# yvokeller/Show-Attend-and-Tell

Measured on AMD Instinct MI355X. Metric: train images/sec on COCO batch=128 at 1/2/4/8 MI355X, higher is better.
Workload: dtype bf16; 1 GPU; COCO-shaped resnet152 encoder (bf16 fwd) + attention/tf/ado decoder train step, V=10000, T=27; global_batch=128, per_gpu_batch=128, seq_len=27, parallelism=dp1, hip_graph=True, encoder_decoder_overlap=True

## Files before the change

include/sat_hip.h:

```cpp
#ifndef SAT_HIP_H_
#define SAT_HIP_H_

#include <stddef.h>
#include <stdint.h>

#ifdef __cplusplus
extern "C" {
#endif

#define SAT_ABI_VERSION 9

enum { SAT_F32 = 0, SAT_BF16 = 1 };
enum { SAT_ACT_NONE = 0, SAT_ACT_RELU = 1, SAT_ACT_TANH = 2, SAT_ACT_SIGMOID = 3 };
enum { SAT_OK = 0, SAT_ERR_INVALID = 9001 };

typedef struct {
  int N, H, W, C, KH, KW, stride, pad, OH, OW;
} SatConvGeom;

typedef struct {
  int conv_pipe;
  int conv_stream;
  int conv3x3_ws;
  int conv_slices;
  int skinny;
  int gemm_stages;
  int gemm_tile;
  int gemm_linear_order;
  int gemm_epilogue;
  int split_gemm;
  int split_k;
  int attn_bwd;
  int attn_bwd_chunks;
  int attn_pipe;
  int decoder_splits[4];
  int greedy_step;
  int embed_grad;
  uint64_t* stamps;
  int stamp_capacity;
} SatPolicy;

typedef struct {
  int M, N, K, dtype;
  const void* A; int64_t lda; int transA;
  const void* B; int64_t ldb; int transB;
  void* C; int64_t ldc; int c_dtype;
  float alpha, beta;
  const float* bias;
  const void* add1; int64_t ld_add1; int add1_dtype;
  int act;
  void* aux; int64_t ld_aux; int aux_dtype;
  const SatPolicy* policy;
  void* workspace; int64_t workspace_bytes;
} SatGemmArgs;

typedef struct {
  int B, L, D, E, V, T;
  int tf, ado, attention, bert, training;
  int dtype;
  int start_token;
  int has_dropout_mask;
  uint64_t seed;
  uint64_t* seed_ptr;
  int split_target;
  const SatPolicy* policy;
} SatDecoderDims;

typedef struct {
  int64_t embedding, init_w, init_b, hcat_w, hcat_b, attW_w, attW_b, v_w, v_b, wih, bih;
  int64_t fh_w, fh_b, fz_w, fz_b, fout_w, fout_b, do_w, do_b;
  int64_t total;
  int64_t wih_ctx_t, hcat_t;
} SatDecoderLayout;

int sat_abi_version(void);
const char* sat_error_string(int code);

int sat_gemm(const SatGemmArgs* args, void* stream);
size_t sat_gemm_workspace_bytes(void);
int sat_cast(const void* x, int x_dtype, void* y, int y_dtype, int64_t n, void* stream);

int sat_mean_rows_abi(const void* a, int B, int L, int D, int dtype, float* out_f32, void* out_t, void* stream);

int sat_nchw_to_nhwc(int N, int C, int H, int W, int Cp, int dtype, const float* x, void* y, void* stream);
int sat_nchw_to_s2d(int N, int C, int H, int W, int dtype, const float* x, void* y, void* stream);
int sat_conv2d_nhwc(const SatConvGeom* g, int Cout, int dtype, const void* x, const void* w,
                    const float* bias, const void* residual, int relu, void* y, const SatPolicy* policy,
                    void* stream);
int sat_mfma_frag_layout(int N, int K, const void* src, void* dst, void* stream);
int sat_bottleneck_fused_supported(int H, int W, int Cin, int Cmid, int dtype);
int sat_bottleneck_fused(int N, int H, int W, int Cin, int Cmid, int dtype, const void* x, const void* w1f,
                         const float* b1, const void* w2f, const float* b2, const void* w3f, const float* b3,
                         void* y, const SatPolicy* policy, void* stream);
int sat_conv3x3_frag_supported(int H, int W, int C, int dtype);
int sat_conv3x3_frag(int N, int H, int W, int C, int dtype, const void* x, const void* wf, const float* b, void* y,
                     const SatPolicy* policy, void* stream);
int sat_conv1x1_frag_supported(int H, int W, int Cin, int Cout, int dtype);
int sat_conv1x1_frag(int N, int H, int W, int Cin, int Cout, int dtype, const void* x, const void* wf,
                     const float* b, void* y, const SatPolicy* policy, void* stream);
int sat_conv1x1_chain_supported(int64_t M, int K, int N, int N2, int dtype, const SatPolicy* policy);
int sat_conv1x1_chain(int64_t M, int K, int N, int N2, int dtype, const void* x, const void* w, const float* bias,
                      const void* residual, void* y, const void* w1, const float* b1, void* x1,
                      const SatPolicy* policy, void* stream);
int sat_conv1x1_proj_supported(int64_t M, int K, int N, int Kp, int stride, int N2, int dtype, const SatPolicy* policy);
int sat_conv1x1_proj(int n, int H, int W, int stride, int K, int N, int Kp, int N2, int dtype, const void* x,
                     const void* w, const float* bias, const void* xin, const void* wp, const float* bp, void* y,
                     const void* w1, const float* b1, void* x1, const SatPolicy* policy, void* stream);
int sat_conv_stem_pool_supported(const SatConvGeom* g, int Cout, int dtype, int relu, int pool_k, int pool_stride,
                                 int pool_pad, const SatPolicy* policy);
int sat_conv_stem_pool(const SatConvGeom* g, int Cout, int dtype, const void* x, const void* w, const float* bias,
                       int relu, int pool_k, int pool_stride, int pool_pad, void* y, const SatPolicy* policy,
                       void* stream);
int sat_maxpool2d_nhwc(int N, int H, int W, int C, int k, int stride, int pad, int dtype,
                       const void* x, void* y, int OH, int OW, void* stream);

size_t sat_conv3x3_wgrad_workspace_bytes(int N, int H, int W, int Cin, int Cout, int dtype, const SatPolicy* policy);
int sat_conv3x3_wgrad(int N, int H, int W, int Cin, int Cout, int dtype, const void* x, const void* dz, float* dw,
                      int accumulate, void* workspace, size_t workspace_bytes, const SatPolicy* policy,
                      void* stream);

int sat_relu_mask(const void* y, int y_dtype, const void* g, int g_dtype, const void* add, int add_dtype, void* out,
                  int out_dtype, int64_t n, void* stream);
int sat_conv_fold(int Cout, int Cin, int KH, int KW, int dtype, const float* weight, const float* bias,
                  const float* bn_weight, const float* bn_bias, const float* bn_mean, const float* bn_var, float eps,
                  void* w_fold, float* b_fold, void* w_igrad, void* stream);
typedef struct {
  const float* weight; const float* bias;
  const float* bn_weight; const float* bn_mean; const float* bn_var; float eps;
  const void* w_fold; const void* w_igrad;
  float* weight_grad; float* bias_grad; float* bn_weight_grad; float* bn_bias_grad;
} SatConvTrain;
int sat_conv_fold_backward(int Cout, int Cin, int KH, int KW, const float* dw_fold, const float* db_fold,
                           const SatConvTrain* conv, int accumulate, void* stream);
size_t sat_bottleneck_backward_workspace_bytes(int N, int H, int W, int Cin, int Cmid, int dtype,
                                               const SatPolicy* policy);
int sat_bottleneck_backward(int N, int H, int W, int Cin, int Cmid, int dtype, const void* x, const void* a1,
                            const void* a2, const void* y, const SatConvTrain* c1, const SatConvTrain* c2,
                            const SatConvTrain* c3, const void* dy, void* dx, int accumulate, void* workspace,
                            size_t workspace_bytes, const SatPolicy* policy, void* stream);
size_t sat_conv3x3_relu_backward_workspace_bytes(int N, int H, int W, int Cin, int Cout, int dtype,
                                                 const SatPolicy* policy);
int sat_conv3x3_relu_backward(int N, int H, int W, int Cin, int Cout, int dtype, const void* x, const void* y,
                              const SatConvTrain* c, const void* dy, void* dx, int accumulate, void* workspace,
                              size_t workspace_bytes, const SatPolicy* policy, void* stream);

int sat_attention_forward(int B, int L, int D, int E, int dtype, const void* img_features,
                          const float* hidden, const float* U_w, const float* U_b,
                          const float* W_w, const void* W_w_lp, const float* W_b,
                          const float* v_w, const float* v_b, float* ws_scratch,
                          float* context, float* alpha, void* stream);


int sat_decoder_step_bench(const SatDecoderDims* dims, const SatDecoderLayout* layout, const float* params,
                           const void* params_lp, const void* img_features, void* workspace, size_t workspace_bytes,
                           float* alphas, const float* d_alphas, int reps, float* us_out, void* stream);
size_t sat_decoder_workspace_bytes(const SatDecoderDims* d);
enum { SAT_DECODER_INSTANCE_FIELDS = 8 };
int sat_decoder_instance(const SatDecoderDims* d, const SatDecoderLayout* lay, int* out, int n);
int sat_decoder_refresh_transposed(const SatDecoderDims* d, const SatDecoderLayout* lay, void* params_lp,
                                   void* stream);
int sat_decoder_forward(const SatDecoderDims* d, const SatDecoderLayout* lay, const float* params,
                        const void* params_lp, const void* img_features, const int64_t* captions,
                        const uint8_t* dropout_mask, void* workspace, size_t workspace_bytes,
                        void* preds, float* alphas, int32_t* tokens, void* stream);
int sat_decoder_forward_sampled(const SatDecoderDims* d, const SatDecoderLayout* lay, const float* params,
                                const void* params_lp, const void* img_features, const int64_t* captions,
                                const uint8_t* dropout_mask, float tf_prob, const float* tf_prob_dev,
                                const uint8_t* tf_mask, uint8_t* tf_mask_out, void* workspace,
                                size_t workspace_bytes, void* preds, float* alphas, int32_t* tokens, void* stream);
int sat_decoder_backward(const SatDecoderDims* d, const SatDecoderLayout* lay, const float* params,
                         const void* params_lp, const void* img_features, void* workspace,
                         size_t workspace_bytes, const void* preds, const float* alphas,
                         const void* d_preds, const float* d_alphas, float* grads, int accumulate,
                         int phase, void* stream);
int sat_decoder_backward_features(const SatDecoderDims* d, const SatDecoderLayout* lay, const float* params,
                                  const void* params_lp, const void* img_features, void* workspace,
                                  size_t workspace_bytes, const void* preds, const float* alphas,
                                  const void* d_preds, const float* d_alphas, float* grads, int accumulate,
                                  int phase, void* stream, void* d_features, void* fg_workspace,
                                  size_t fg_workspace_bytes);
size_t sat_decoder_feature_grad_workspace_bytes(const SatDecoderDims* d);
int sat_feature_grad_accumulate(int B, int L, int D, int T1, int dtype, const float* alpha, int64_t alpha_stride_b,
                                int64_t alpha_stride_t, const float* dctx, int64_t dctx_stride_b,
                                int64_t dctx_stride_t, const float* addend, int64_t addend_ld,
                                const float* mean_term, int64_t mean_ld, void* out, int64_t out_ld, void* stream);

size_t sat_decoder_beam_workspace_bytes(const SatDecoderDims* d, int beam_size);
int sat_decoder_beam_search(const SatDecoderDims* d, const SatDecoderLayout* lay, const float* params,
                            const void* params_lp, const void* img_features, int beam_size, int max_step,
                            void* workspace, size_t workspace_bytes, int32_t* out_ids, int* out_len,
                            float* out_alphas, int* out_alpha_rows, float* out_score, void* stream);

size_t sat_decoder_beam_batch_workspace_bytes(const SatDecoderDims* d, int n_images, int beam_size, int max_step);
int sat_decoder_beam_search_batch(const SatDecoderDims* d, const SatDecoderLayout* lay, const float* params,
                                  const void* params_lp, const void* img_features, int n_images, int beam_size,
                                  int max_step, void* workspace, size_t workspace_bytes, int32_t* out_ids,
                                  int* out_len, float* out_alphas, int* out_alpha_rows, float* out_score,
                                  void* stream);

size_t sat_caption_loss_workspace_bytes(int B, int T, int L);
int sat_caption_loss_forward(int B, int T, int V, int L, int dtype, const void* preds,
                             const float* alphas, const int64_t* captions, float alpha_c,
                             int pad_id, int skip0, int skip1, int skip2, void* workspace,
                             float* out, void* stream);
int sat_caption_loss_forward_loss_out(int B, int T, int V, int L, int dtype, const void* preds,
                                      const float* alphas, const int64_t* captions, float alpha_c,
                                      int pad_id, int skip0, int skip1, int skip2, void* workspace,
                                      float* out, float* loss_out, void* stream);
int sat_caption_loss_backward(int B, int T, int V, int L, int dtype, const void* preds,
                              const int64_t* captions, float alpha_c, void* workspace,
                              const float* grad_out, void* d_preds, float* d_alphas, void* stream);
int sat_caption_loss_backward_relu(int B, int T, int V, int L, int dtype, const void* preds,
                              const int64_t* captions, float alpha_c, void* workspace,
                              const float* grad_out, void* d_preds, float* d_alphas, void* stream);
int sat_caption_loss_backward_ld(int B, int T, int V, int L, int dtype, const void* preds,
                                 const int64_t* captions, float alpha_c, void* workspace,
                                 const float* grad_out, void* d_preds, int64_t ld_dpreds,
                                 float* d_alphas, int relu_mask, void* stream);

enum { SAT_IMG_NCHW = 0, SAT_IMG_NHWC = 1, SAT_IMG_S2D16 = 2 };
size_t sat_images_workspace_bytes(int B, int OH, int OW);
int sat_images_max_downscale(void);
int sat_images_to_input(const uint8_t* pixels, const int64_t* offsets, const int32_t* sizes, int B, int max_h,
                        int max_w, int OH, int OW, const float* mean, const float* std, int layout, int c_pad,
                        int dtype, void* out, void* workspace, size_t workspace_bytes, void* stream);

int sat_rows_gather(const void* table, int64_t n_rows, int64_t row_elems, int dtype, const int64_t* idx, int n,
                    void* out, int32_t* n_bad, void* stream);
int sat_rows_scatter(const void* src, int n, int64_t row_elems, int dtype, const int64_t* idx, void* table,
                     int64_t n_rows, int32_t* n_bad, void* stream);

int sat_adam_step(float* param, const float* grad, float* exp_avg, float* exp_avg_sq,
// ... 8 lines not shown
```

show-attend-and-tell_amd/_lib.py:

```python
import ctypes
import os

import torch

_HERE = os.path.dirname(os.path.abspath(__file__))
LIB_PATH = os.environ.get("SAT_HIP_LIB_TUNING") or os.path.join(_HERE, "libsat_hip.so")

SAT_F32, SAT_BF16 = 0, 1
IMG_NCHW, IMG_NHWC, IMG_S2D16 = 0, 1, 2
ACT_NONE, ACT_RELU, ACT_TANH, ACT_SIGMOID = 0, 1, 2, 3

c_int, c_int64, c_float, c_void_p, c_size_t, c_uint64 = (ctypes.c_int, ctypes.c_int64, ctypes.c_float,
                                                        ctypes.c_void_p, ctypes.c_size_t, ctypes.c_uint64)


class SatConvGeom(ctypes.Structure):
    _fields_ = [(n, c_int) for n in ("N", "H", "W", "C", "KH", "KW", "stride", "pad", "OH", "OW")]


ABI_VERSION = 9


class SatPolicy(ctypes.Structure):
    _fields_ = [(n, c_int) for n in ("conv_pipe", "conv_stream", "conv3x3_ws", "conv_slices", "skinny", "gemm_stages",
                                     "gemm_tile", "gemm_linear_order", "gemm_epilogue", "split_gemm", "split_k",
                                     "attn_bwd", "attn_bwd_chunks", "attn_pipe")] + \
               [("decoder_splits", c_int * 4), ("greedy_step", c_int), ("embed_grad", c_int), ("stamps", c_void_p),
                ("stamp_capacity", c_int)]

    def __init__(self, **kw):
        splits = kw.pop("decoder_splits", None)
        super().__init__(**kw)
        if splits is not None:
            self.decoder_splits[:] = list(splits)


class SatGemmArgs(ctypes.Structure):
    _fields_ = [("M", c_int), ("N", c_int), ("K", c_int), ("dtype", c_int),
                ("A", c_void_p), ("lda", c_int64), ("transA", c_int),
                ("B", c_void_p), ("ldb", c_int64), ("transB", c_int),
                ("C", c_void_p), ("ldc", c_int64), ("c_dtype", c_int),
                ("alpha", c_float), ("beta", c_float),
                ("bias", c_void_p),
                ("add1", c_void_p), ("ld_add1", c_int64), ("add1_dtype", c_int),
                ("act", c_int),
                ("aux", c_void_p), ("ld_aux", c_int64), ("aux_dtype", c_int),
                ("policy", ctypes.POINTER(SatPolicy)),
                ("workspace", c_void_p), ("workspace_bytes", c_int64)]


class SatDecoderDims(ctypes.Structure):
    _fields_ = [("B", c_int), ("L", c_int), ("D", c_int), ("E", c_int), ("V", c_int), ("T", c_int),
                ("tf", c_int), ("ado", c_int), ("attention", c_int), ("bert", c_int), ("training", c_int),
                ("dtype", c_int), ("start_token", c_int), ("has_dropout_mask", c_int), ("seed", c_uint64),
                ("seed_ptr", c_void_p), ("split_target", c_int), ("policy", ctypes.POINTER(SatPolicy))]


class SatConvTrain(ctypes.Structure):
    _fields_ = [("weight", c_void_p), ("bias", c_void_p), ("bn_weight", c_void_p), ("bn_mean", c_void_p),
                ("bn_var", c_void_p), ("eps", c_float), ("w_fold", c_void_p), ("w_igrad", c_void_p),
                ("weight_grad", c_void_p), ("bias_grad", c_void_p), ("bn_weight_grad", c_void_p),
                ("bn_bias_grad", c_void_p)]


LAYOUT_FIELDS = ("embedding", "init_w", "init_b", "hcat_w", "hcat_b", "attW_w", "attW_b", "v_w", "v_b", "wih",
                 "bih", "fh_w", "fh_b", "fz_w", "fz_b", "fout_w", "fout_b", "do_w", "do_b", "total", "wih_ctx_t",
                 "hcat_t")


class SatDecoderLayout(ctypes.Structure):
    _fields_ = [(n, c_int64) for n in LAYOUT_FIELDS]


_SIGNATURES = [
    ("sat_abi_version", c_int, []),
    ("sat_error_string", ctypes.c_char_p, [c_int]),
    ("sat_gemm", c_int, [ctypes.POINTER(SatGemmArgs), c_void_p]),
    ("sat_gemm_workspace_bytes", c_size_t, []),
    ("sat_cast", c_int, [c_void_p, c_int, c_void_p, c_int, c_int64, c_void_p]),
    ("sat_mean_rows_abi", c_int, [c_void_p, c_int, c_int, c_int, c_int, c_void_p, c_void_p, c_void_p]),
    ("sat_nchw_to_nhwc", c_int, [c_int, c_int, c_int, c_int, c_int, c_int, c_void_p, c_void_p, c_void_p]),
    ("sat_nchw_to_s2d", c_int, [c_int, c_int, c_int, c_int, c_int, c_void_p, c_void_p, c_void_p]),
    ("sat_conv2d_nhwc", c_int, [ctypes.POINTER(SatConvGeom), c_int, c_int, c_void_p, c_void_p, c_void_p, c_void_p,
                                c_int, c_void_p, ctypes.POINTER(SatPolicy), c_void_p]),
    ("sat_mfma_frag_layout", c_int, [c_int, c_int, c_void_p, c_void_p, c_void_p]),
    ("sat_bottleneck_fused_supported", c_int, [c_int, c_int, c_int, c_int, c_int]),
    ("sat_bottleneck_fused", c_int, [c_int, c_int, c_int, c_int, c_int, c_int, c_void_p, c_void_p, c_void_p,
                                     c_void_p, c_void_p, c_void_p, c_void_p, c_void_p, ctypes.POINTER(SatPolicy),
                                     c_void_p]),
    ("sat_conv3x3_frag_supported", c_int, [c_int, c_int, c_int, c_int]),
    ("sat_conv3x3_frag", c_int, [c_int, c_int, c_int, c_int, c_int, c_void_p, c_void_p, c_void_p, c_void_p,
                                 ctypes.POINTER(SatPolicy), c_void_p]),
    ("sat_conv1x1_frag_supported", c_int, [c_int, c_int, c_int, c_int, c_int]),
    ("sat_conv1x1_frag", c_int, [c_int, c_int, c_int, c_int, c_int, c_int, c_void_p, c_void_p, c_void_p, c_void_p,
                                 ctypes.POINTER(SatPolicy), c_void_p]),
    ("sat_conv1x1_chain_supported", c_int, [c_int64, c_int, c_int, c_int, c_int, ctypes.POINTER(SatPolicy)]),
    ("sat_conv1x1_chain", c_int, [c_int64, c_int, c_int, c_int, c_int, c_void_p, c_void_p, c_void_p, c_void_p, c_void_p,
                                  c_void_p, c_void_p, c_void_p, ctypes.POINTER(SatPolicy), c_void_p]),
    ("sat_conv1x1_proj_supported", c_int, [c_int64, c_int, c_int, c_int, c_int, c_int, c_int,
                                           ctypes.POINTER(SatPolicy)]),
    ("sat_conv1x1_proj", c_int, [c_int, c_int, c_int, c_int, c_int, c_int, c_int, c_int, c_int, c_void_p, c_void_p,
                                 c_void_p, c_void_p, c_void_p, c_void_p, c_void_p, c_void_p, c_void_p, c_void_p,
                                 ctypes.POINTER(SatPolicy), c_void_p]),
    ("sat_conv_stem_pool_supported", c_int, [ctypes.POINTER(SatConvGeom), c_int, c_int, c_int, c_int, c_int, c_int,
                                             ctypes.POINTER(SatPolicy)]),
    ("sat_conv_stem_pool", c_int, [ctypes.POINTER(SatConvGeom), c_int, c_int, c_void_p, c_void_p, c_void_p, c_int,
                                   c_int, c_int, c_int, c_void_p, ctypes.POINTER(SatPolicy), c_void_p]),
    ("sat_maxpool2d_nhwc", c_int, [c_int, c_int, c_int, c_int, c_int, c_int, c_int, c_int, c_void_p, c_void_p,
                                   c_int, c_int, c_void_p]),
    ("sat_conv3x3_wgrad_workspace_bytes", c_size_t, [c_int, c_int, c_int, c_int, c_int, c_int,
                                                     ctypes.POINTER(SatPolicy)]),
    ("sat_conv3x3_wgrad", c_int, [c_int, c_int, c_int, c_int, c_int, c_int, c_void_p, c_void_p, c_void_p, c_int,
                                  c_void_p, c_size_t, ctypes.POINTER(SatPolicy), c_void_p]),
    ("sat_relu_mask", c_int, [c_void_p, c_int, c_void_p, c_int, c_void_p, c_int, c_void_p, c_int, c_int64, c_void_p]),
    ("sat_conv_fold", c_int, [c_int, c_int, c_int, c_int, c_int, c_void_p, c_void_p, c_void_p, c_void_p, c_void_p,
                              c_void_p, c_float, c_void_p, c_void_p, c_void_p, c_void_p]),
    ("sat_conv_fold_backward", c_int, [c_int, c_int, c_int, c_int, c_void_p, c_void_p, ctypes.POINTER(SatConvTrain),
                                       c_int, c_void_p]),
    ("sat_bottleneck_backward_workspace_bytes", c_size_t, [c_int, c_int, c_int, c_int, c_int, c_int,
                                                           ctypes.POINTER(SatPolicy)]),
    ("sat_bottleneck_backward", c_int, [c_int, c_int, c_int, c_int, c_int, c_int, c_void_p, c_void_p, c_void_p,
                                        c_void_p, ctypes.POINTER(SatConvTrain), ctypes.POINTER(SatConvTrain),
                                        ctypes.POINTER(SatConvTrain), c_void_p, c_void_p, c_int, c_void_p, c_size_t,
                                        ctypes.POINTER(SatPolicy), c_void_p]),
    ("sat_conv3x3_relu_backward_workspace_bytes", c_size_t, [c_int, c_int, c_int, c_int, c_int, c_int,
                                                             ctypes.POINTER(SatPolicy)]),
    ("sat_conv3x3_relu_backward", c_int, [c_int, c_int, c_int, c_int, c_int, c_int, c_void_p, c_void_p,
                                          ctypes.POINTER(SatConvTrain), c_void_p, c_void_p, c_int, c_void_p, c_size_t,
                                          ctypes.POINTER(SatPolicy), c_void_p]),
    ("sat_attention_forward", c_int, [c_int, c_int, c_int, c_int, c_int, c_void_p, c_void_p, c_void_p, c_void_p,
                                      c_void_p, c_void_p, c_void_p, c_void_p, c_void_p, c_void_p, c_void_p,
                                      c_void_p, c_void_p]),
    ("sat_decoder_workspace_bytes", c_size_t, [ctypes.POINTER(SatDecoderDims)]),
    ("sat_decoder_instance", c_int, [ctypes.POINTER(SatDecoderDims), ctypes.POINTER(SatDecoderLayout),
                                     ctypes.POINTER(c_int), c_int]),
    ("sat_decoder_refresh_transposed", c_int, [ctypes.POINTER(SatDecoderDims), ctypes.POINTER(SatDecoderLayout),
                                               c_void_p, c_void_p]),
    ("sat_decoder_forward", c_int, [ctypes.POINTER(SatDecoderDims), ctypes.POINTER(SatDecoderLayout), c_void_p,
                                    c_void_p, c_void_p, c_void_p, c_void_p, c_void_p, c_size_t, c_void_p,
                                    c_void_p, c_void_p, c_void_p]),
    ("sat_decoder_forward_sampled", c_int, [ctypes.POINTER(SatDecoderDims), ctypes.POINTER(SatDecoderLayout),
                                            c_void_p, c_void_p, c_void_p, c_void_p, c_void_p, c_float, c_void_p,
                                            c_void_p, c_void_p, c_void_p, c_size_t, c_void_p, c_void_p, c_void_p,
                                            c_void_p]),
    ("sat_decoder_backward", c_int, [ctypes.POINTER(SatDecoderDims), ctypes.POINTER(SatDecoderLayout), c_void_p,
                                     c_void_p, c_void_p, c_void_p, c_size_t, c_void_p, c_void_p, c_void_p,
                                     c_void_p, c_void_p, c_int, c_int, c_void_p]),
    ("sat_decoder_backward_features", c_int, [ctypes.POINTER(SatDecoderDims), ctypes.POINTER(SatDecoderLayout),
                                              c_void_p, c_void_p, c_void_p, c_void_p, c_size_t, c_void_p, c_void_p,
                                              c_void_p, c_void_p, c_void_p, c_int, c_int, c_void_p, c_void_p,
                                              c_void_p, c_size_t]),
    ("sat_decoder_feature_grad_workspace_bytes", c_size_t, [ctypes.POINTER(SatDecoderDims)]),
    ("sat_feature_grad_accumulate", c_int, [c_int, c_int, c_int, c_int, c_int, c_void_p, c_int64, c_int64, c_void_p,
                                            c_int64, c_int64, c_void_p, c_int64, c_void_p, c_int64, c_void_p,
                                            c_int64, c_void_p]),
    ("sat_decoder_step_bench", c_int, [ctypes.POINTER(SatDecoderDims), ctypes.POINTER(SatDecoderLayout), c_void_p,
                                       c_void_p, c_void_p, c_void_p, c_size_t, c_void_p, c_void_p, c_int, c_void_p,
                                       c_void_p]),
    ("sat_decoder_beam_workspace_bytes", c_size_t, [ctypes.POINTER(SatDecoderDims), c_int]),
    ("sat_decoder_beam_search", c_int, [ctypes.POINTER(SatDecoderDims), ctypes.POINTER(SatDecoderLayout), c_void_p,
                                        c_void_p, c_void_p, c_int, c_int, c_void_p, c_size_t, c_void_p, c_void_p,
                                        c_void_p, c_void_p, c_void_p, c_void_p]),
    ("sat_decoder_beam_batch_workspace_bytes", c_size_t, [ctypes.POINTER(SatDecoderDims), c_int, c_int, c_int]),
    ("sat_decoder_beam_search_batch", c_int, [ctypes.POINTER(SatDecoderDims), ctypes.POINTER(SatDecoderLayout),
                                              c_void_p, c_void_p, c_void_p, c_int, c_int, c_int, c_void_p, c_size_t,
                                              c_void_p, c_void_p, c_void_p, c_void_p, c_void_p, c_void_p]),
    ("sat_caption_loss_workspace_bytes", c_size_t, [c_int, c_int, c_int]),
    ("sat_caption_loss_forward", c_int, [c_int, c_int, c_int, c_int, c_int, c_void_p, c_void_p, c_void_p, c_float,
                                         c_int, c_int, c_int, c_int, c_void_p, c_void_p, c_void_p]),
    ("sat_caption_loss_forward_loss_out", c_int, [c_int, c_int, c_int, c_int, c_int, c_void_p, c_void_p, c_void_p,
                                                  c_float, c_int, c_int, c_int, c_int, c_void_p, c_void_p, c_void_p,
                                                  c_void_p]),
    ("sat_caption_loss_backward", c_int, [c_int, c_int, c_int, c_int, c_int, c_void_p, c_void_p, c_float,
                                          c_void_p, c_void_p, c_void_p, c_void_p, c_void_p]),
    ("sat_caption_loss_backward_relu", c_int, [c_int, c_int, c_int, c_int, c_int, c_void_p, c_void_p, c_float,
                                          c_void_p, c_void_p, c_void_p, c_void_p, c_void_p]),
    ("sat_caption_loss_backward_ld", c_int, [c_int, c_int, c_int, c_int, c_int, c_void_p, c_void_p, c_float,
                                             c_void_p, c_void_p, c_void_p, c_int64, c_void_p, c_int, c_void_p]),
    ("sat_images_workspace_bytes", c_size_t, [c_int, c_int, c_int]),
    ("sat_images_max_downscale", c_int, []),
    ("sat_images_to_input", c_int, [c_void_p, c_void_p, c_void_p, c_int, c_int, c_int, c_int, c_int,
                                    ctypes.POINTER(c_float), ctypes.POINTER(c_float), c_int, c_int, c_int, c_void_p,
                                    c_void_p, c_size_t, c_void_p]),
    ("sat_rows_gather", c_int, [c_void_p, c_int64, c_int64, c_int, c_void_p, c_int, c_void_p, c_void_p, c_void_p]),
    ("sat_rows_scatter", c_int, [c_void_p, c_int, c_int64, c_int, c_void_p, c_void_p, c_int64, c_void_p, c_void_p]),
    ("sat_adam_step", c_int, [c_void_p, c_void_p, c_void_p, c_void_p, c_void_p, c_int64, c_float, c_float,
                              c_float, c_float, c_float, c_void_p]),
]
EXPORTED = [s[0] for s in _SIGNATURES]

_lib = None


def lib():
    global _lib
    if _lib is None:
        if not os.path.exists(LIB_PATH):
            raise RuntimeError(f"sat_amd: HIP library not found at {LIB_PATH}; build it with "
                               "`python -c 'import __graft_entry__ as g; g.build()'` (make -C "
                               "show-attend-and-tell_amd/csrc)")
        handle = ctypes.CDLL(LIB_PATH)
        for name, res, args in _SIGNATURES:
            fn = getattr(handle, name)
            fn.restype = res
            fn.argtypes = args
        version = handle.sat_abi_version()
        if version != ABI_VERSION:
            raise RuntimeError(f"sat_amd: {LIB_PATH} has C-ABI version {version}, this package binds version "
                               f"{ABI_VERSION}; rebuild it (make -C show-attend-and-tell_amd/csrc)")
        _lib = handle
    return _lib


def check(code, what):
    if code != 0:
        msg = lib().sat_error_string(code)
        raise RuntimeError(f"sat_amd: {what} failed with code {code}: {msg.decode() if msg else '?'}")


def dtype_code(dt):
    if dt == torch.float32:
        return SAT_F32
    if dt == torch.bfloat16:
        return SAT_BF16
    raise TypeError(f"sat_amd: unsupported dtype {dt} (float32 or bfloat16)")


def require_device(*tensors):
    for t in tensors:
        if t is not None and t.device.type != "cuda":
            raise RuntimeError("sat_amd: tensors must live on a HIP device (the product path has no CPU fallback)")
# ... 13 lines not shown
```

show-attend-and-tell_amd/csrc/decoder.hip:

```cpp
#include "sat_common.h"
#include "sat_internal.h"

namespace {

struct WS {
  float *mean_f, *hc0, *hc0pre, *xg, *gctx_const, *hg, *gctx, *uh_all, *gates_all, *c_in, *c_out, *h_out, *ctx_all,
      *gate_all, *fh, *fz;
  void *mean_t, *Ws, *emb_t, *h_in_t, *ctx_t, *gated_t, *hd_t, *comb_t;
  int32_t* tok;
  uint8_t* dmask;
  void *dpre_t, *dfh_t, *dfz_t, *dhg_t, *dWs_t, *dpre0_t;
  float *dcomb, *dhd, *dctx_head, *dhg, *dgated, *dh_rec, *dc, *dWs_acc, *dv_acc, *dbv_acc, *part, *demb, *dpre0,
      *colsum, *de_all;
  unsigned* ticket;
  float* gsplit;
  unsigned* gtickets;
  float* xt;
  float* fzp;
  float* am_val;
  int32_t* am_idx;
  void* emb_ws;
};
constexpr int kTicketBlocks = 16;

struct Splits { int h, c, g, dh, i; };
constexpr int kSplitTargetDefault = 192;

constexpr int kChainAtomicK = 1024;
inline int ragged_splits(int K, long want) {
  const int kt = sat_cdiv(K, 64);
  const int cap = want < 2 ? 2 : (want > 8 ? 8 : (int)want);
  const int kc = sat_cdiv(kt, cap);
  return sat_cdiv(kt, kc);
}
inline int pick_splits(int M, int N, int K, int dtype, bool kmajor_w, int target) {
  if (dtype != SAT_BF16) return 1;
  const long tiles = (long)sat_cdiv(M, 128) * sat_cdiv(N, kmajor_w ? 128 : 64);
  long want = (target + tiles - 1) / tiles;
  if (want > 32) want = 32;
  const int kt = K / 64;
  int best = 1;
  if (K % 64 == 0)
    for (int s = 1; s <= kt && s <= want; ++s)
      if (kt % s == 0) best = s;
  if (best == 1 && K >= kChainAtomicK) best = ragged_splits(K, want);
  return best;
}
inline int forced(int f, int K, int auto_s) {
  if (f == 1 && K >= kChainAtomicK) return auto_s;
  return (f > 0 && K % 64 == 0 && (K / 64) % f == 0) ? f : auto_s;
}
inline Splits splits_for(const SatDecoderDims& d, bool tr) {
  const int E = d.E, D = d.D, HG = 5 * E + D;
  const bool bf = d.dtype == SAT_BF16;
  const int tg = d.split_target > 0 ? d.split_target : kSplitTargetDefault;
  const int KH = d.attention ? HG : 4 * E;
  Splits s;
  s.h = pick_splits(d.B, KH, E, d.dtype, false, tg);
  s.c = pick_splits(d.B, 4 * E, D, d.dtype, false, tg);
  s.g = pick_splits(d.B, D, 4 * E, d.dtype, !tr, tg);
  s.dh = pick_splits(d.B, E, KH, d.dtype, !tr, tg);
  s.i = pick_splits(d.B, 2 * E, D, d.dtype, false, tg);
  if (bf) {
    int k;
    if ((k = sat_skinny_splits(d.B, KH, E))) s.h = k;
    if ((k = sat_skinny_splits(d.B, 4 * E, D))) s.c = D % 512 == 0 ? k / 2 : k;
    if ((k = sat_skinny_splits(d.B, 2 * E, D))) s.i = k;
    if (tr && (k = sat_skinny_splits(d.B, D, 4 * E)) && (4 * E) % 512 == 0) s.g = k / 2;
    if (tr && (k = sat_skinny_splits(d.B, E, KH)) && KH % 512 == 0) s.dh = k / 2;
    if (tr && s.dh > 1 && KH % 128 == 0 && KH >= 4096) {
      const int cols = E / 32, kt = KH / 128;
      for (int c = 16; c > s.dh; --c)
        if (kt % c == 0 && c * cols <= 256 && KH / c <= 1024) { s.dh = c; break; }
    }
  }
  if (bf) {
    const int* f = sat_policy().decoder_splits;
    s.h = forced(f[0], E, s.h);
    s.c = forced(f[1], D, s.c);
    s.g = forced(f[2], 4 * E, s.g);
    s.dh = forced(f[3], KH, s.dh);
  }
  return s;
}
inline bool use_transposed(const SatDecoderDims& d, const SatDecoderLayout& lay) {
  return d.dtype == SAT_BF16 && lay.wih_ctx_t >= 0 && lay.hcat_t >= 0 && sat_policy().skinny != 1;
}
inline bool greedy_fused(const SatDecoderDims& d) {
  return d.dtype == SAT_BF16 && !d.tf && sat_policy().greedy_step != 1 && sat_greedy_supported(d.B, d.E);
}
inline bool embed_sorted(const SatDecoderDims& d) {
  return !d.bert && sat_policy().embed_grad != 1 && (long)d.B * (d.T - 1) <= sat_embed_sorted_max_rows() &&
         d.V < (1 << 18) && d.E % 4 == 0;
}

struct Carver {
  char* base;
  size_t off = 0;
  template <typename P>
  void take(P*& p, size_t bytes) {
    off = (off + 255) & ~(size_t)255;
    p = base ? (P*)(base + off) : nullptr;
    off += bytes;
  }
};

inline int head_ld(const SatDecoderDims& d) { return d.dtype == SAT_BF16 && d.V % 8 ? (d.V + 7) / 8 * 8 : d.V; }

size_t carve(const SatDecoderDims& d, char* base, WS* w) {
  const size_t B = d.B, L = d.L, D = d.D, E = d.E, V = d.V, T1 = d.T - 1, R = B * T1;
  const size_t HG = 5 * E + D;
  const size_t ts = d.dtype == SAT_BF16 ? 2 : 4, f = 4;
  Splits sp = splits_for(d, false);
  {
    const Splits st = splits_for(d, true);
    sp.g = sp.g > st.g ? sp.g : st.g;
    sp.dh = sp.dh > st.dh ? sp.dh : st.dh;
  }
  Carver c{base};
  c.take(w->mean_f, B * D * f);  c.take(w->mean_t, B * D * ts);
  c.take(w->hc0, B * 2 * E * f);
  c.take(w->hc0pre, sp.i * B * 2 * E * f);
  c.take(w->Ws, B * L * E * ts);
  c.take(w->tok, R * 4);
  c.take(w->emb_t, R * E * ts);
  c.take(w->xg, R * 4 * E * f);
  c.take(w->gctx_const, B * 4 * E * f);
  c.take(w->hg, sp.h * B * HG * f);
  c.take(w->gctx, sp.c * B * 4 * E * f);
  c.take(w->uh_all, R * E * f);
  c.take(w->gates_all, R * 4 * E * f);
  c.take(w->c_in, R * E * f);   c.take(w->c_out, R * E * f);
  c.take(w->h_in_t, R * E * ts); c.take(w->h_out, R * E * f);
  c.take(w->ctx_all, R * D * f); c.take(w->ctx_t, R * D * ts);
  c.take(w->gate_all, R * D * f); c.take(w->gated_t, R * D * ts);
  c.take(w->dmask, R * E);
  c.take(w->hd_t, R * E * ts);
  c.take(w->fh, R * E * f); c.take(w->fz, R * E * f); c.take(w->comb_t, R * E * ts);
  c.take(w->dpre_t, R * head_ld(d) * ts);
  c.take(w->dcomb, R * E * f);
  c.take(w->dfh_t, R * E * ts); c.take(w->dfz_t, R * E * ts);
  c.take(w->dhd, R * E * f);
  c.take(w->dctx_head, R * D * f);
  c.take(w->dhg, R * HG * f); c.take(w->dhg_t, R * HG * ts);
  c.take(w->dgated, sp.g * B * D * f);
  c.take(w->dh_rec, sp.dh * B * E * f); c.take(w->dc, B * E * f);
  c.take(w->dWs_acc, B * L * E * f); c.take(w->dWs_t, B * L * E * ts);
  c.take(w->dv_acc, B * E * f); c.take(w->dbv_acc, B * f);
  c.take(w->de_all, R * L * f);
  c.take(w->part, sat_attention_part_floats(d.B, d.L, d.D, d.E, d.dtype, d.split_target) * f);
  c.take(w->ticket, B * 4);
  if (d.dtype == SAT_BF16) {
    c.take(w->gsplit, sat_split_gemm_ws_bytes() - kSatSplitTickets * 4);
    c.take(w->gtickets, (size_t)kTicketBlocks * kSatSplitTickets * 4);
  } else {
    w->gsplit = nullptr;
    w->gtickets = nullptr;
  }
  c.take(w->demb, R * E * f);
  c.take(w->dpre0, B * 2 * E * f); c.take(w->dpre0_t, B * 2 * E * ts);
  if (greedy_fused(d)) {
    c.take(w->xt, V * 4 * E * f);
    c.take(w->fzp, sp.c * B * E * f);
    c.take(w->am_val, (size_t)sat_greedy_head_blocks(d.B, d.V, d.E) * B * f);
    c.take(w->am_idx, (size_t)sat_greedy_head_blocks(d.B, d.V, d.E) * B * 4);
  } else {
    w->xt = w->fzp = w->am_val = nullptr;
    w->am_idx = nullptr;
  }
  if (embed_sorted(d)) c.take(w->emb_ws, sat_embed_sorted_ws_bytes((int)R, (int)E));
  else w->emb_ws = nullptr;
  size_t maxN = V > HG ? V : HG;
  if (D > maxN) maxN = D;
  const size_t ph1 = V + 2 * E, ph2 = 9 * E + D + 1;
  if (ph1 > maxN) maxN = ph1;
  if (ph2 > maxN) maxN = ph2;
  c.take(w->colsum, sat_colsum_scratch_floats((int)R, (int)maxN) * f);
  return c.off + 256;
}

struct FGWS {
  float *dctx, *addend, *mean_term;
};
size_t carve_fg(const SatDecoderDims& d, char* base, FGWS* w) {
  const size_t B = d.B, L = d.L, D = d.D, R = B * (d.T - 1), f = 4;
  Carver c{base};
  c.take(w->dctx, R * D * f);
  if (d.attention) c.take(w->addend, B * L * D * f);
  else w->addend = nullptr;
  c.take(w->mean_term, B * D * f);
  return c.off + 256;
}

__global__ void start_tokens_kernel(int32_t* tok, int B, int T1, int start) {
  int b = blockIdx.x * blockDim.x + threadIdx.x;
  if (b < B) tok[(long)b * T1] = start;
}

__global__ void tf_prefill_kernel(const int64_t* __restrict__ caps, int B, int T, int V, int start,
                                  const uint8_t* __restrict__ keep_in, float p, const float* __restrict__ p_dev,
                                  uint64_t seed, const uint64_t* __restrict__ seed_ptr, int32_t* __restrict__ pre,
                                  uint8_t* __restrict__ keep_out) {
  const int T1 = T - 1;
  const int i = blockIdx.x * blockDim.x + threadIdx.x;
  if (i >= B * T1) return;
  const int b = i / T1, t = i - b * T1;
  bool keep = true;
  int tok = start;
  if (t > 0) {
    const int64_t c = caps[(long)b * T + t];
    tok = (c < 0 || c >= V) ? 0 : (int)c;
    if (keep_in) {
      keep = keep_in[i] != 0;
    } else {
      if (seed_ptr) seed ^= *seed_ptr * 0xD1B54A32D192ED03ULL;
      keep = sat_tf_uniform(seed, b, t) < (p_dev ? *p_dev : p);
    }
  }
  pre[i] = keep ? tok : -1;
  if (keep_out) keep_out[i] = keep ? 1 : 0;
}

struct Sampled {
  const int64_t* captions;
  float p; const float* p_dev;
  const uint8_t* mask; uint8_t* mask_out;
};
inline int32_t* tok_pre(const WS& w) { return (int32_t*)w.demb; }

template <typename T>
__global__ void ado_combine_rows_kernel(const float* fh, const float* fz, const T* emb, int rows, int E, long ld,
                                        T* comb) {
  const long n = (long)rows * E;
  for (long i = blockIdx.x * (long)blockDim.x + threadIdx.x; i < n; i += (long)gridDim.x * blockDim.x) {
    const long r = i / E;
    const int e = (int)(i - r * E);
    const long o = r * ld + e;
    comb[o] = (T)(fh[o] + fz[o] + (float)emb[o]);
  }
}

int combine_rows(const float* fh, const float* fz, const void* emb, int rows, int E, long ld, int dtype, void* comb,
                 hipStream_t s) {
  long n = (long)rows * E;
  int g = (int)((n + 255) / 256);
  if (g > 4096) g = 4096;
  if (dtype == SAT_BF16)
    hipLaunchKernelGGL(ado_combine_rows_kernel<bf16>, dim3(g), dim3(256), 0, s, fh, fz, (const bf16*)emb, rows, E, ld, (bf16*)comb);
  else
    hipLaunchKernelGGL(ado_combine_rows_kernel<float>, dim3(g), dim3(256), 0, s, fh, fz, (const float*)emb, rows, E, ld, (float*)comb);
  return (int)hipGetLastError();
}

template <typename T>
__global__ void init_state_kernel(const float* pre, int splits, long stride, int B, int E, float* hc0, T* h_t,
                                  long h_ld, float* c_in, long c_ld) {
  const long n = (long)B * 2 * E;
  for (long i = blockIdx.x * (long)blockDim.x + threadIdx.x; i < n; i += (long)gridDim.x * blockDim.x) {
    const int b = (int)(i / (2 * E)), j = (int)(i - (long)b * 2 * E);
    const float v = tanhf(sum_parts(pre, i, splits, stride));
    hc0[i] = v;
    if (j < E) h_t[(long)b * h_ld + j] = (T)v;
    else c_in[(long)b * c_ld + j - E] = v;
  }
}

struct Ctx {
  SatDecoderDims d;
  SatDecoderLayout lay;
  const float* P;
  const void* LP;
  int ts;
  long T1, R, HG;
  bool tr;
  const void* W(int64_t off) const {
    return d.dtype == SAT_BF16 ? (const void*)((const bf16*)LP + off) : (const void*)(P + off);
  }
  const float* F(int64_t off) const { return P + off; }
  void* at(void* p, long elems) const { return (char*)p + elems * ts; }
  const void* at(const void* p, long elems) const { return (const char*)p + elems * ts; }
};

int linear(const Ctx& c, int rows, int N, int K, const void* x, long ldx, const void* w, long ldw, const float* bias,
           void* y, long ldy, int y_dtype, int act, hipStream_t s, const void* add1 = nullptr, long ld_add1 = 0,
           int add1_dtype = SAT_F32, void* aux = nullptr, long ld_aux = 0, int aux_dtype = SAT_F32,
           int splits = 0, long split_stride = 0) {
  SatGemm g;
  g.partial_splits = splits; g.split_stride = split_stride;
  g.M = rows; g.N = N; g.K = K; g.dtype = c.d.dtype;
  g.A = x; g.lda = ldx; g.B = w; g.ldb = ldw;
  g.C = y; g.ldc = ldy; g.c_dtype = y_dtype; g.bias = bias; g.act = act;
  g.add1 = add1; g.ld_add1 = ld_add1; g.add1_dtype = add1_dtype;
  g.aux = aux; g.ld_aux = ld_aux; g.aux_dtype = aux_dtype;
  return sat_gemm_launch(g, s);
}

int head_forward(const Ctx& c, const WS& w, int rows, int t, bool per_step, void* preds, const uint8_t* mask_in,
                 hipStream_t s) {
  const SatDecoderDims& d = c.d;
  const int E = d.E, D = d.D, V = d.V;
  const long rs = per_step ? c.T1 : 1;
  const long oE = per_step ? (long)t * E : 0, oD = per_step ? (long)t * D : 0, oV = per_step ? (long)t * V : 0;
  if (per_step)
    SAT_CHECK((hipError_t)sat_dropout_apply(w.h_out + oE, c.T1 * E, d.B, 1, E, d.training, d.has_dropout_mask,
                                            mask_in ? mask_in + oE : nullptr, w.dmask + oE, c.T1 * E, d.seed,
                                            d.seed_ptr, t,
                                            c.at(w.hd_t, oE), c.T1 * E, d.dtype, s));
  else
    SAT_CHECK((hipError_t)sat_dropout_apply(w.h_out, E, d.B, (int)c.T1, E, d.training, d.has_dropout_mask, mask_in,
                                            w.dmask, E, d.seed, d.seed_ptr, 0, w.hd_t, E, d.dtype, s));
  if (d.ado) {
    SAT_CHECK((hipError_t)linear(c, rows, E, E, c.at(w.hd_t, oE), rs * E, c.W(c.lay.fh_w), E, c.F(c.lay.fh_b),
                                 w.fh + oE, rs * E, SAT_F32, SAT_ACT_RELU, s));
    SAT_CHECK((hipError_t)linear(c, rows, E, D, c.at(w.ctx_t, oD), rs * D, c.W(c.lay.fz_w), D, c.F(c.lay.fz_b),
                                 w.fz + oE, rs * E, SAT_F32, SAT_ACT_RELU, s));
    SAT_CHECK((hipError_t)combine_rows(w.fh + oE, w.fz + oE, c.at(w.emb_t, oE), rows, E, rs * E, d.dtype,
                                       c.at(w.comb_t, oE), s));
    SAT_CHECK((hipError_t)linear(c, rows, V, E, c.at(w.comb_t, oE), rs * E, c.W(c.lay.fout_w), E,
                                 c.F(c.lay.fout_b), c.at(preds, oV), rs * V, d.dtype, SAT_ACT_RELU, s));
  } else {
    SAT_CHECK((hipError_t)linear(c, rows, V, E, c.at(w.hd_t, oE), rs * E, c.W(c.lay.do_w), E, c.F(c.lay.do_b),
                                 c.at(preds, oV), rs * V, d.dtype, SAT_ACT_NONE, s));
  }
  return 0;
}

struct StepIO {
  const void* feats;
  float* alphas;
  const float* d_alphas;
};

int fwd_hgemm(const Ctx& c, const WS& w, const Splits& sp, int t, hipStream_t s) {
  const SatDecoderDims& d = c.d;
  const int B = d.B, D = d.D, E = d.E;
  const long T1 = c.T1, HG = c.HG;
  const void* h_t = c.at(w.h_in_t, (long)t * E);
  if (d.attention)
    return linear(c, B, (int)HG, E, h_t, T1 * E, c.W(c.lay.hcat_w), E, c.F(c.lay.hcat_b), w.hg, HG, SAT_F32,
                  SAT_ACT_NONE, s, nullptr, 0, SAT_F32, nullptr, 0, SAT_F32, sp.h, (long)B * HG);
  return linear(c, B, 4 * E, E, h_t, T1 * E, c.W(c.lay.hcat_w + (long)(E + D) * E), E, c.F(c.lay.hcat_b + E + D),
                w.hg + E + D, HG, SAT_F32, SAT_ACT_NONE, s, nullptr, 0, SAT_F32, nullptr, 0, SAT_F32, sp.h,
                (long)B * HG);
}

int fwd_attn(const Ctx& c, const WS& w, const Splits& sp, const StepIO& io, int t, hipStream_t s) {
  const SatDecoderDims& d = c.d;
  const int B = d.B, L = d.L, D = d.D, E = d.E;
  const long T1 = c.T1, HG = c.HG;
  AttnFwdArgs a{};
  a.B = B; a.L = L; a.D = D; a.E = E; a.dtype = d.dtype;
  a.Ws = w.Ws; a.uh = w.hg; a.uh_ld = HG; a.v_w = c.F(c.lay.v_w); a.v_b = c.F(c.lay.v_b); a.a = io.feats;
  a.gate_pre = w.hg + E; a.gate_ld = HG;
  a.hg_splits = sp.h; a.hg_split_stride = (long)B * HG;
  a.alpha = io.alphas + (long)t * L; a.alpha_ld = T1 * L;
  a.ctx = w.ctx_all + (long)t * D; a.ctx_ld = T1 * D;
  a.ctx_t = c.at(w.ctx_t, (long)t * D); a.ctx_t_ld = T1 * D;
  a.gate = w.gate_all + (long)t * D; a.gate_out_ld = T1 * D;
  a.gated = c.at(w.gated_t, (long)t * D); a.gated_ld = T1 * D;
  a.uh_save = w.uh_all + (long)t * E; a.uh_save_ld = T1 * E;
  return sat_attention_fwd_launch(a, s);
}

int fwd_cgemm(const Ctx& c, const WS& w, const Splits& sp, int t, hipStream_t s) {
  const SatDecoderDims& d = c.d;
  const int B = d.B, D = d.D, E = d.E;
  return linear(c, B, 4 * E, D, c.at(w.gated_t, (long)t * D), c.T1 * D, c.W(c.lay.wih + E), E + D, nullptr, w.gctx,
                4 * E, SAT_F32, SAT_ACT_NONE, s, nullptr, 0, SAT_F32, nullptr, 0, SAT_F32, sp.c, (long)B * 4 * E);
}

LstmFwdArgs lstm_fwd_args(const Ctx& c, const WS& w, const Splits& sp, int t) {
  const SatDecoderDims& d = c.d;
  const int B = d.B, D = d.D, E = d.E;
  const long T1 = c.T1, HG = c.HG;
  const bool att = d.attention != 0;
  LstmFwdArgs l{};
  l.B = B; l.E = E; l.dtype = d.dtype;
  l.hpart = w.hg + E + D; l.hpart_ld = HG;
  l.xpart = w.xg + (long)t * 4 * E; l.xpart_ld = T1 * 4 * E;
  l.cpart = att ? w.gctx : w.gctx_const; l.cpart_ld = 4 * E;
  l.h_splits = sp.h; l.h_split_stride = (long)B * HG;
  l.c_splits = att ? sp.c : 1; l.c_split_stride = (long)B * 4 * E;
  l.c_prev = w.c_in + (long)t * E; l.c_prev_ld = T1 * E;
  l.gates = w.gates_all + (long)t * 4 * E; l.gates_ld = T1 * 4 * E;
  l.c_out = w.c_out + (long)t * E; l.c_out_ld = T1 * E;
  l.c_next_in = t + 1 < T1 ? w.c_in + (long)(t + 1) * E : nullptr; l.c_next_in_ld = T1 * E;
  l.h_out = w.h_out + (long)t * E; l.h_out_ld = T1 * E;
  l.h_next_in_t = t + 1 < T1 ? c.at(w.h_in_t, (long)(t + 1) * E) : nullptr; l.h_next_in_t_ld = T1 * E;
  return l;
}

int fwd_lstm(const Ctx& c, const WS& w, const Splits& sp, int t, hipStream_t s) {
  return sat_lstm_fwd_launch(lstm_fwd_args(c, w, sp, t), s);
}

LstmBwdArgs lstm_bwd_args(const Ctx& c, const WS& w, const Splits& sp, int t) {
  const SatDecoderDims& d = c.d;
  const int B = d.B, D = d.D, E = d.E;
  const long T1 = c.T1, HG = c.HG;
  LstmBwdArgs l{};
  l.B = B; l.E = E; l.dtype = d.dtype;
  l.gates = w.gates_all + (long)t * 4 * E; l.gates_ld = T1 * 4 * E;
  l.c_prev = w.c_in + (long)t * E; l.c_prev_ld = T1 * E;
  l.c_new = w.c_out + (long)t * E; l.c_new_ld = T1 * E;
  l.dh_rec = t == T1 - 1 ? nullptr : w.dh_rec; l.dh_rec_ld = E;
  l.dh_splits = sp.dh; l.dh_split_stride = (long)B * E;
  l.dh_head = w.dhd + (long)t * E; l.dh_head_ld = T1 * E;
  l.mask = d.training ? w.dmask + (long)t * E : nullptr; l.mask_ld = T1 * E;
  l.dc = w.dc; l.dc_zero = t == T1 - 1;
  l.d_gates = w.dhg + (long)t * HG + E + D; l.d_gates_ld = T1 * HG;
  l.d_gates_t = c.at(w.dhg_t, (long)t * HG + E + D); l.d_gates_t_ld = T1 * HG;
  return l;
}

int bwd_lstm(const Ctx& c, const WS& w, const Splits& sp, int t, hipStream_t s) {
  return sat_lstm_bwd_launch(lstm_bwd_args(c, w, sp, t), s);
}

struct SplitWS {
  float* slab;
  unsigned* tickets;
  int blk;
};
inline void use_split(SatGemm& g, const SplitWS* sw) {
  if (!sw || !sw->slab) return;
  g.split_ws = sw->slab;
  g.split_ws_bytes = (long)(sat_split_gemm_ws_bytes() - kSatSplitTickets * 4);
  g.split_tickets = sw->tickets + (long)sw->blk * kSatSplitTickets;
  g.tickets_zeroed = 1;
}

int dgrad_launch(const Ctx& c, int M, int N, int K, const void* X, long ldx, const void* Wt, long ldw, float* out,
                 long ldo, hipStream_t s, const float* add1 = nullptr, long ld_add1 = 0, int splits = 0,
                 long split_stride = 0, int a_tail = 0, const SplitWS* sw = nullptr) {
  SatGemm g;
  use_split(g, sw);
  g.a_tail = a_tail;
  g.partial_splits = splits; g.split_stride = split_stride;
  g.M = M; g.N = N; g.K = K; g.dtype = c.d.dtype;
  g.A = X; g.lda = ldx; g.B = Wt; g.ldb = ldw; g.transB = 1;
  g.C = out; g.ldc = ldo; g.c_dtype = SAT_F32;
  g.add1 = add1; g.ld_add1 = ld_add1; g.add1_dtype = SAT_F32;
  return sat_gemm_launch(g, s);
}

int bwd_ggemm(const Ctx& c, const WS& w, const Splits& sp, int t, hipStream_t s) {
  const SatDecoderDims& d = c.d;
  const int B = d.B, D = d.D, E = d.E;
  if (c.tr)
    return linear(c, B, D, 4 * E, c.at(w.dhg_t, (long)t * c.HG + E + D), c.T1 * c.HG, c.W(c.lay.wih_ctx_t), 4 * E,
                  nullptr, w.dgated, D, SAT_F32, SAT_ACT_NONE, s, nullptr, 0, SAT_F32, nullptr, 0, SAT_F32, sp.g,
                  (long)B * D);
  return dgrad_launch(c, B, D, 4 * E, c.at(w.dhg_t, (long)t * c.HG + E + D), c.T1 * c.HG, c.W(c.lay.wih + E), E + D,
                      w.dgated, D, s, nullptr, 0, sp.g, (long)B * D);
}

int bwd_attn(const Ctx& c, const WS& w, const Splits& sp, const StepIO& io, int t, hipStream_t s,
             float* dctx_all = nullptr) {
  const SatDecoderDims& d = c.d;
  const int B = d.B, L = d.L, D = d.D, E = d.E;
  const long T1 = c.T1, HG = c.HG;
  AttnBwdArgs a{};
  a.B = B; a.L = L; a.D = D; a.E = E; a.dtype = d.dtype;
  a.Ws = w.Ws; a.a = io.feats;
  a.uh = w.uh_all + (long)t * E; a.uh_ld = T1 * E;
  a.v_w = c.F(c.lay.v_w);
  a.alpha = io.alphas + (long)t * L; a.alpha_ld = T1 * L;
  a.d_alpha_ext = io.d_alphas + (long)t * L; a.d_alpha_ext_ld = T1 * L;
  a.d_gated = w.dgated; a.d_gated_ld = D;
  a.gate = w.gate_all + (long)t * D; a.gate_ld = T1 * D;
  a.ctx = w.ctx_all + (long)t * D; a.ctx_ld = T1 * D;
  a.d_ctx_ext = d.ado ? w.dctx_head + (long)t * D : nullptr; a.d_ctx_ext_ld = T1 * D;
  a.d_ctx_out = dctx_all ? dctx_all + (long)t * D : nullptr; a.d_ctx_out_ld = T1 * D;
  a.d_uh = w.dhg + (long)t * HG; a.d_uh_ld = T1 * HG; a.d_uh_t = c.at(w.dhg_t, (long)t * HG);
  a.d_gpre = w.dhg + (long)t * HG + E; a.d_gpre_ld = T1 * HG; a.d_gpre_t = c.at(w.dhg_t, (long)t * HG + E);
  a.de_out = w.de_all + (long)t * L; a.de_ld = T1 * L; a.dv_acc = w.dv_acc; a.dbv_acc = w.dbv_acc; a.part = w.part;
  a.ticket = w.ticket;
  a.dg_splits = sp.g; a.dg_split_stride = (long)B * D;
  a.wg_target = d.split_target;
  return sat_attention_bwd_launch(a, s);
}

int bwd_dhgemm(const Ctx& c, const WS& w, const Splits& sp, int t, hipStream_t s) {
  const SatDecoderDims& d = c.d;
  const int B = d.B, D = d.D, E = d.E;
  const long T1 = c.T1, HG = c.HG;
  if (c.tr) {
    const long k0 = d.attention ? 0 : E + D;
    return linear(c, B, E, (int)(HG - k0), c.at(w.dhg_t, (long)t * HG + k0), T1 * HG, c.W(c.lay.hcat_t + k0), HG,
                  nullptr, w.dh_rec, E, SAT_F32, SAT_ACT_NONE, s, nullptr, 0, SAT_F32, nullptr, 0, SAT_F32, sp.dh,
                  (long)B * E);
  }
  if (d.attention)
    return dgrad_launch(c, B, E, (int)HG, c.at(w.dhg_t, (long)t * HG), T1 * HG, c.W(c.lay.hcat_w), E, w.dh_rec, E, s,
                        nullptr, 0, sp.dh, (long)B * E);
  return dgrad_launch(c, B, E, 4 * E, c.at(w.dhg_t, (long)t * HG + E + D), T1 * HG,
                      c.W(c.lay.hcat_w + (long)(E + D) * E), E, w.dh_rec, E, s, nullptr, 0, sp.dh, (long)B * E);
}

constexpr int kStampGroups = 8;
inline uint64_t* step_slot(const SatDecoderDims& d, int g, int t) {
  const SatPolicy* p = d.policy;
  if (!p || !p->stamps || p->stamp_capacity <= 0) return nullptr;
  return p->stamps + ((long)g * (d.T - 1) + t) * 2L * (p->stamp_capacity + 1);
}
inline int stamp_cap(const SatDecoderDims& d) { return d.policy ? d.policy->stamp_capacity : 0; }

struct StepTimer {
  SatStampScope stamps;
  StepTimer(const SatDecoderDims& d, int g, int t) : stamps(step_slot(d, g, t), stamp_cap(d)) {}
};

int greedy_loop(const Ctx& c, const WS& w, const Splits& sp, const StepIO& io, void* preds, const uint8_t* mask_in,
                int32_t* tokens, hipStream_t s, const Sampled* sm = nullptr) {
  const SatDecoderDims& d = c.d;
  const SatDecoderLayout& lay = c.lay;
  const int B = d.B, D = d.D, E = d.E, V = d.V, T1 = d.T - 1;
  const bool att = d.attention != 0;
  SAT_CHECK((hipError_t)linear(c, V, 4 * E, E, c.W(lay.embedding), E, c.W(lay.wih), E + D, c.F(lay.bih), w.xt, 4 * E,
                               SAT_F32, SAT_ACT_NONE, s));
  SAT_CHECK((hipError_t)sat_embed_gather(w.xt, w.tok, B, 1, T1, 4 * E, SAT_F32, w.xg, (long)T1 * 4 * E, s));
  for (int t = 0; t < T1; ++t) {
    const long oE = (long)t * E, oD = (long)t * D;
    {
      StepTimer st(d, 0, t);
      SAT_CHECK((hipError_t)fwd_hgemm(c, w, sp, t, s));
    }
    if (att) {
      {
        StepTimer st(d, 1, t);
        SAT_CHECK((hipError_t)fwd_attn(c, w, sp, io, t, s));
      }
      StepTimer st(d, 2, t);
      SatGemm g1;
      g1.partial_splits = sp.c; g1.split_stride = (long)B * 4 * E;
      g1.M = B; g1.N = 4 * E; g1.K = D; g1.dtype = d.dtype;
      g1.A = c.at(w.gated_t, oD); g1.lda = c.T1 * D; g1.B = c.W(lay.wih + E); g1.ldb = E + D;
      g1.C = w.gctx; g1.ldc = 4 * E; g1.c_dtype = SAT_F32;
      SatGemm g2 = g1;
      g2.N = E; g2.A = c.at(w.ctx_t, oD); g2.B = c.W(lay.fz_w); g2.ldb = D;
      g2.C = w.fzp; g2.ldc = E; g2.split_stride = (long)B * E;
      int err = 0;
      if (!(d.ado && sat_skinny_dual_try(g1, g2, s, &err))) {
        SAT_CHECK((hipError_t)sat_gemm_launch(g1, s));
        if (d.ado) SAT_CHECK((hipError_t)sat_gemm_launch(g2, s));
      }
      SAT_CHECK((hipError_t)err);
    } else if (d.ado) {
      SAT_CHECK((hipError_t)linear(c, B, E, D, c.at(w.ctx_t, oD), c.T1 * D, c.W(lay.fz_w), D, nullptr, w.fzp, E,
                                   SAT_F32, SAT_ACT_NONE, s));
    }
    {
      StepTimer st(d, 3, t);
      LstmFwdArgs l = lstm_fwd_args(c, w, sp, t);
      l.hd_t = c.at(w.hd_t, oE); l.hd_ld = c.T1 * E;
      l.drop_training = d.training; l.drop_has_mask = d.has_dropout_mask; l.drop_t = t;
      l.mask_in = mask_in ? mask_in + oE : nullptr; l.mask_out = w.dmask + oE; l.mask_ld = c.T1 * E;
      l.seed = d.seed; l.seed_ptr = d.seed_ptr;
      if (t > 0) {
        l.am_val = w.am_val; l.am_idx = w.am_idx; l.am_ncb = sat_greedy_head_blocks(B, V, E); l.am_V = V;
        l.xt = w.xt; l.emb = c.F(lay.embedding); l.emb_t = c.at(w.emb_t, oE); l.emb_t_ld = c.T1 * E;
        l.tok_out = w.tok + t; l.tok_ld = T1;
        if (sm) l.tok_pre = tok_pre(w) + t;
      }
      SAT_CHECK((hipError_t)sat_lstm_fwd_launch(l, s));
    }
    HeadOutArgs ho{};
    ho.B = B; ho.V = V; ho.E = E;
    if (d.ado) {
      HeadMidArgs hm{};
      hm.B = B; hm.E = E;
      hm.hd = (const bf16*)c.at(w.hd_t, oE); hm.hd_ld = c.T1 * E;
      hm.fh_w = (const bf16*)c.W(lay.fh_w); hm.fh_b = c.F(lay.fh_b);
      hm.fzp = w.fzp; hm.fzp_ld = E; hm.fz_splits = att ? sp.c : 1; hm.fz_split_stride = (long)B * E;
      hm.fz_b = c.F(lay.fz_b);
      hm.emb = (const bf16*)c.at(w.emb_t, oE); hm.emb_ld = c.T1 * E;
      hm.fh = w.fh + oE; hm.fz = w.fz + oE; hm.f_ld = c.T1 * E;
      hm.comb = (bf16*)c.at(w.comb_t, oE); hm.comb_ld = c.T1 * E;
      SAT_CHECK((hipError_t)sat_greedy_head_mid(hm, s));
      ho.relu = 1;
      ho.x = hm.comb; ho.x_ld = hm.comb_ld;
      ho.w = (const bf16*)c.W(lay.fout_w); ho.bias = c.F(lay.fout_b);
    } else {
      ho.relu = 0;
      ho.x = (const bf16*)c.at(w.hd_t, oE); ho.x_ld = c.T1 * E;
      ho.w = (const bf16*)c.W(lay.do_w); ho.bias = c.F(lay.do_b);
    }
    ho.preds = (bf16*)c.at(preds, (long)t * V); ho.preds_ld = c.T1 * V;
    ho.pval = w.am_val; ho.pidx = w.am_idx;
    SAT_CHECK((hipError_t)sat_greedy_head_out(ho, s));
  }
  if (d.training && d.seed_ptr) SAT_CHECK((hipError_t)sat_bump_seed(d.seed_ptr, s));
  if (tokens) SAT_CHECK(hipMemcpyAsync(tokens, w.tok, c.R * sizeof(int32_t), hipMemcpyDeviceToDevice, s));
  return 0;
}

// ... 127 lines not shown
    hipLaunchKernelGGL(start_tokens_kernel, dim3(sat_cdiv(B, 256)), dim3(256), 0, s, w.tok, B, T1, d.start_token);
    SAT_LAUNCH_CHECK();
    if (sm) {
      hipLaunchKernelGGL(tf_prefill_kernel, dim3(sat_cdiv(B * T1, 256)), dim3(256), 0, s, sm->captions, B, d.T, d.V,
                         d.start_token, sm->mask, sm->p, sm->p_dev, d.seed, (const uint64_t*)d.seed_ptr, tok_pre(w),
                         sm->mask_out);
      SAT_LAUNCH_CHECK();
    }
    SAT_CHECK((hipError_t)sat_embed_gather(c.F(lay->embedding), w.tok, B, 1, T1, E, d.dtype, w.emb_t, (long)T1 * E, s));
  }
  SAT_CHECK((hipError_t)sat_mean_rows(img_features, B, L, D, d.dtype, w.mean_f, w.mean_t, s));
  SAT_CHECK((hipError_t)linear(c, B, 2 * E, D, w.mean_t, D, c.W(lay->init_w), D, c.F(lay->init_b), w.hc0pre, 2 * E,
                               SAT_F32, SAT_ACT_NONE, s, nullptr, 0, SAT_F32, nullptr, 0, SAT_F32, sp.i,
                               (long)B * 2 * E));
  {
    const long n = (long)B * 2 * E;
    const int g = (int)((n + 255) / 256 < 2048 ? (n + 255) / 256 : 2048);
    if (d.dtype == SAT_BF16)
      hipLaunchKernelGGL(init_state_kernel<bf16>, dim3(g), dim3(256), 0, s, (const float*)w.hc0pre, sp.i,
                         (long)B * 2 * E, B, E, w.hc0, (bf16*)w.h_in_t, (long)T1 * E, w.c_in, (long)T1 * E);
    else
      hipLaunchKernelGGL(init_state_kernel<float>, dim3(g), dim3(256), 0, s, (const float*)w.hc0pre, sp.i,
                         (long)B * 2 * E, B, E, w.hc0, (float*)w.h_in_t, (long)T1 * E, w.c_in, (long)T1 * E);
    SAT_LAUNCH_CHECK();
  }
  if (att) {
    SAT_CHECK((hipError_t)linear(c, B * L, E, D, img_features, D, c.W(lay->attW_w), D, c.F(lay->attW_b), w.Ws, E,
                                 d.dtype, SAT_ACT_NONE, s));
  } else {
    SAT_CHECK((hipError_t)linear(c, B, 4 * E, D, w.mean_t, D, c.W(lay->wih + E), E + D, nullptr, w.gctx_const, 4 * E,
                                 SAT_F32, SAT_ACT_NONE, s));
    SAT_CHECK((hipError_t)sat_broadcast_rows(w.mean_t, B, D, T1, d.dtype, w.gated_t, s));
    SAT_CHECK((hipError_t)sat_broadcast_rows(w.mean_t, B, D, T1, d.dtype, w.ctx_t, s));
    SAT_CHECK((hipError_t)sat_broadcast_rows(w.mean_f, B, D, T1, SAT_F32, w.ctx_all, s));
    SAT_CHECK((hipError_t)sat_fill_const(alphas, (long)B * T1 * L, 1.0f / (float)L, s));
  }
  if (d.tf)
    SAT_CHECK((hipError_t)linear(c, (int)c.R, 4 * E, E, w.emb_t, E, c.W(lay->wih), E + D, c.F(lay->bih), w.xg, 4 * E,
                                 SAT_F32, SAT_ACT_NONE, s));

  if (greedy_fused(d)) return greedy_loop(c, w, sp, io, preds, dropout_mask, tokens, s, sm);

  for (int t = 0; t < T1; ++t) {
    if (!d.tf)
      SAT_CHECK((hipError_t)linear(c, B, 4 * E, E, c.at(w.emb_t, (long)t * E), (long)T1 * E, c.W(lay->wih), E + D,
                                   c.F(lay->bih), w.xg + (long)t * 4 * E, (long)T1 * 4 * E, SAT_F32, SAT_ACT_NONE, s));
    {
      StepTimer st(d, 0, t);
      SAT_CHECK((hipError_t)fwd_hgemm(c, w, sp, t, s));
    }
    if (att) {
      {
        StepTimer st(d, 1, t);
        SAT_CHECK((hipError_t)fwd_attn(c, w, sp, io, t, s));
      }
      StepTimer st(d, 2, t);
      SAT_CHECK((hipError_t)fwd_cgemm(c, w, sp, t, s));
    }
    {
      StepTimer st(d, 3, t);
      SAT_CHECK((hipError_t)fwd_lstm(c, w, sp, t, s));
    }
    if (!d.tf) {
      SAT_CHECK((hipError_t)head_forward(c, w, B, t, true, preds, dropout_mask, s));
      if (t + 1 < T1 && sm)
        SAT_CHECK((hipError_t)sat_argmax_rows_select(c.at(preds, (long)t * d.V), d.dtype, (long)T1 * d.V, B, d.V,
                                                     w.tok + t + 1, T1, c.F(lay->embedding), E,
                                                     c.at(w.emb_t, (long)(t + 1) * E), (long)T1 * E,
                                                     tok_pre(w) + t + 1, T1, s));
      else if (t + 1 < T1)
        SAT_CHECK((hipError_t)sat_argmax_rows(c.at(preds, (long)t * d.V), d.dtype, (long)T1 * d.V, B, d.V,
                                              w.tok + t + 1, T1, c.F(lay->embedding), E,
                                              c.at(w.emb_t, (long)(t + 1) * E), (long)T1 * E, s));
    }
  }
  if (d.tf) SAT_CHECK((hipError_t)head_forward(c, w, (int)c.R, 0, false, preds, dropout_mask, s));
  if (d.training && d.seed_ptr) SAT_CHECK((hipError_t)sat_bump_seed(d.seed_ptr, s));
  if (tokens) SAT_CHECK(hipMemcpyAsync(tokens, w.tok, c.R * sizeof(int32_t), hipMemcpyDeviceToDevice, s));
  return 0;
}
}

extern "C" int sat_decoder_forward(const SatDecoderDims* dp, const SatDecoderLayout* lay, const float* params,
                                   const void* params_lp, const void* img_features, const int64_t* captions,
                                   const uint8_t* dropout_mask, void* workspace, size_t workspace_bytes, void* preds,
                                   float* alphas, int32_t* tokens, void* stream) {
  return decoder_forward(dp, lay, params, params_lp, img_features, captions, dropout_mask, workspace, workspace_bytes,
                         preds, alphas, tokens, stream, nullptr);
}

extern "C" int sat_decoder_forward_sampled(const SatDecoderDims* dp, const SatDecoderLayout* lay, const float* params,
                                           const void* params_lp, const void* img_features, const int64_t* captions,
                                           const uint8_t* dropout_mask, float tf_prob, const float* tf_prob_dev,
                                           const uint8_t* tf_mask, uint8_t* tf_mask_out, void* workspace,
                                           size_t workspace_bytes, void* preds, float* alphas, int32_t* tokens,
                                           void* stream) {
  SAT_REQUIRE(dp && dp->tf == 0);
  SAT_REQUIRE(tf_prob >= 0.f && tf_prob <= 1.f);
  const Sampled sm{captions, tf_prob, tf_prob_dev, tf_mask, tf_mask_out};
  return decoder_forward(dp, lay, params, params_lp, img_features, captions, dropout_mask, workspace, workspace_bytes,
                         preds, alphas, tokens, stream, &sm);
}

namespace {
int decoder_backward(const SatDecoderDims* dp, const SatDecoderLayout* lay, const float* params, const void* params_lp,
                     const void* img_features, void* workspace, size_t workspace_bytes, const void* preds,
                     const float* alphas, const void* d_preds, const float* d_alphas, float* grads, int accumulate,
                     int phase, void* stream, void* d_features, void* fg_workspace, size_t fg_workspace_bytes) {
  SAT_CHECK((hipError_t)check_dims(dp));
  SAT_REQUIRE(lay && params && img_features && workspace && preds && alphas && d_preds && d_alphas && grads);
  FGWS fg{};
  if (d_features && (phase & 2)) {
    SAT_REQUIRE(fg_workspace && carve_fg(*dp, nullptr, &fg) <= fg_workspace_bytes);
    SAT_REQUIRE(((uintptr_t)d_features & 15) == 0 && ((uintptr_t)fg_workspace & 15) == 0);
    carve_fg(*dp, (char*)fg_workspace, &fg);
  }
  SAT_REQUIRE((phase & 3) != 0 && phase >= 1 && phase <= 15);
  SAT_REQUIRE(dp->dtype == SAT_F32 || params_lp);
  SatPolicyScope scope(dp->policy);
  SatStampScope no_stamps(nullptr, 0);
  const SatDecoderDims& d = *dp;
  WS w;
  SAT_REQUIRE(carve(d, nullptr, &w) <= workspace_bytes);
  carve(d, (char*)workspace, &w);
  hipStream_t s = (hipStream_t)stream;
  Ctx c{d, *lay, params, params_lp, d.dtype == SAT_BF16 ? 2 : 4, d.T - 1, (long)d.B * (d.T - 1), 5L * d.E + d.D,
        use_transposed(d, *lay)};
  const int B = d.B, L = d.L, D = d.D, E = d.E, V = d.V, T1 = d.T - 1;
  const int R = (int)c.R;
  const int VP = head_ld(d);
  const long HG = c.HG;
  const bool att = d.attention != 0;
  const float beta = accumulate ? 1.f : 0.f;
  const Splits sp = splits_for(d, c.tr);
  auto G = [&](int64_t off) { return grads + off; };
  auto wg = [&](int M, int N, int K, const void* X, long ldx, const void* Y, long ldy, float* out, long ldo,
                int a_tail = 0) {
    SatGemm g;
    g.a_tail = a_tail;
    g.M = M; g.N = N; g.K = K; g.dtype = d.dtype;
    g.A = X; g.lda = ldx; g.transA = 1;
    g.B = Y; g.ldb = ldy; g.transB = 1;
    g.C = out; g.ldc = ldo; g.c_dtype = SAT_F32; g.beta = beta;
    return g;
  };
  const SplitWS sws[kTicketBlocks] = {
      {w.gsplit, w.gtickets, 0}, {w.gsplit, w.gtickets, 1}, {w.gsplit, w.gtickets, 2}, {w.gsplit, w.gtickets, 3},
      {w.gsplit, w.gtickets, 4}, {w.gsplit, w.gtickets, 5}, {w.gsplit, w.gtickets, 6}, {w.gsplit, w.gtickets, 7},
      {w.gsplit, w.gtickets, 8}, {w.gsplit, w.gtickets, 9}, {w.gsplit, w.gtickets, 10}, {w.gsplit, w.gtickets, 11},
      {w.gsplit, w.gtickets, 12}, {w.gsplit, w.gtickets, 13}, {w.gsplit, w.gtickets, 14}, {w.gsplit, w.gtickets, 15}};
  const SatZeroSeg tickets_ph1{(float*)w.gtickets, 1, 8L * kSatSplitTickets, 8L * kSatSplitTickets};
  const SatZeroSeg tickets_ph2{(float*)w.gtickets + 8L * kSatSplitTickets, 1, 8L * kSatSplitTickets,
                               8L * kSatSplitTickets};
  auto wgs = [&](int blk, int M, int N, int K, const void* X, long ldx, const void* Y, long ldy, float* out, long ldo,
                 int a_tail = 0) {
    SatGemm g = wg(M, N, K, X, ldx, Y, ldy, out, ldo, a_tail);
    use_split(g, &sws[blk]);
    return g;
  };
  auto prezero = [&](SatGemm* const* gs, int n, SatZeroSeg* seg, int& nseg) {
    for (int i = 0; i < n; ++i)
      if (!accumulate && !sat_split_gemm_takes(*gs[i]) && sat_gemm_splits_atomically(*gs[i])) {
        seg[nseg++] = SatZeroSeg{(float*)gs[i]->C, gs[i]->M, gs[i]->N, gs[i]->ldc};
        gs[i]->c_zeroed = 1;
      }
  };
  auto dgrad = [&](int blk, int M, int N, int K, const void* X, long ldx, const void* Wt, long ldw, float* out,
                   long ldo, const float* add1 = nullptr, long ld_add1 = 0) {
    return dgrad_launch(c, M, N, K, X, ldx, Wt, ldw, out, ldo, s, add1, ld_add1, 0, 0, 0, &sws[blk]);
  };
  auto colsum = [&](const void* X, int dt, long ld, int rows, int N, float* out, float* out2 = nullptr,
                    int cols_readable = 0) {
    return sat_colsum(X, dt, ld, rows, N, out, accumulate, out2, w.colsum, s, cols_readable);
  };

  if (phase & 1) {
    if (d.ado) {
      const void* dpre = d_preds;
      long ldp = V;
      if (phase & 8) {
        SAT_REQUIRE(phase & 4);
        ldp = VP;
      } else if (VP != V) {
        SAT_CHECK((hipError_t)sat_pad_rows(d_preds, (phase & 4) ? nullptr : preds, R, V, VP, d.dtype, w.dpre_t, s));
        dpre = w.dpre_t; ldp = VP;
      } else if (!(phase & 4)) {
        SAT_CHECK((hipError_t)sat_relu_mask_mul(d_preds, preds, (long)R * V, d.dtype, w.dpre_t, s));
        dpre = w.dpre_t;
      }
      SatGemm gfo = wgs(0, V, E, R, dpre, ldp, w.comb_t, E, G(lay->fout_w), E, VP != V);
      SatGemm gfh = wgs(2, E, E, R, w.dfh_t, E, w.hd_t, E, G(lay->fh_w), E);
      SatGemm gfz = wgs(3, E, D, R, w.dfz_t, E, w.ctx_t, D, G(lay->fz_w), D);
      {
        SatGemm* gs[3] = {&gfo, &gfh, &gfz};
        SatZeroSeg seg[4];
        int nseg = 0;
        if (w.gtickets) seg[nseg++] = tickets_ph1;
        prezero(gs, 3, seg, nseg);
        SAT_CHECK((hipError_t)sat_zero_segs(seg, nseg, s));
      }
      SAT_CHECK((hipError_t)sat_gemm_launch(gfo, s));
      SAT_CHECK((hipError_t)dgrad_launch(c, R, E, V, dpre, ldp, c.W(lay->fout_w), E, w.dcomb, E, s, nullptr, 0, 0, 0,
                                         VP != V, &sws[1]));
      SAT_CHECK((hipError_t)sat_ado_bwd_split(w.dcomb, w.fh, w.fz, (long)R * E, d.dtype, w.dfh_t, w.dfz_t, s));
      SAT_CHECK((hipError_t)sat_gemm_launch(gfh, s));
      SAT_CHECK((hipError_t)sat_gemm_launch(gfz, s));
      const SatColsumSeg cs[3] = {{dpre, d.dtype, ldp, R, V, G(lay->fout_b), accumulate, nullptr, ldp != V},
                                  {w.dfh_t, d.dtype, E, R, E, G(lay->fh_b), accumulate, nullptr},
                                  {w.dfz_t, d.dtype, E, R, E, G(lay->fz_b), accumulate, nullptr}};
      SAT_CHECK((hipError_t)sat_colsum_multi(cs, 3, w.colsum, s));
      SAT_CHECK((hipError_t)dgrad(4, R, E, E, w.dfh_t, E, c.W(lay->fh_w), E, w.dhd, E));
      if (att) SAT_CHECK((hipError_t)dgrad(5, R, D, E, w.dfz_t, E, c.W(lay->fz_w), D, w.dctx_head, D));
    } else {
      const void* dpre = d_preds;
      long ldp = (phase & 8) ? VP : V;
      if (VP != V && !(phase & 8)) {
        SAT_CHECK((hipError_t)sat_pad_rows(d_preds, nullptr, R, V, VP, d.dtype, w.dpre_t, s));
        dpre = w.dpre_t; ldp = VP;
      }
      SatGemm gdo = wgs(0, V, E, R, dpre, ldp, w.hd_t, E, G(lay->do_w), E, VP != V);
      {
        SatGemm* gs[1] = {&gdo};
        SatZeroSeg seg[2];
        int nseg = 0;
        if (w.gtickets) seg[nseg++] = tickets_ph1;
        prezero(gs, 1, seg, nseg);
        SAT_CHECK((hipError_t)sat_zero_segs(seg, nseg, s));
      }
      SAT_CHECK((hipError_t)sat_gemm_launch(gdo, s));
      SAT_CHECK((hipError_t)colsum(dpre, d.dtype, ldp, R, V, G(lay->do_b), nullptr, ldp != V));
      SAT_CHECK((hipError_t)dgrad_launch(c, R, E, V, dpre, ldp, c.W(lay->do_w), E, w.dhd, E, s, nullptr, 0, 0, 0,
                                         VP != V, &sws[1]));
    }
  }
  if (!(phase & 2)) return 0;

  const void* dg_t = c.at(w.dhg_t, E + D);
  SatGemm g_attw = wgs(8, E, D, B * L, w.dWs_t, E, img_features, D, G(lay->attW_w), D);
  SatGemm g_init = wgs(9, 2 * E, D, B, w.dpre0_t, 2 * E, w.mean_t, D, G(lay->init_w), D);
  SatGemm g_hcat = att ? wgs(10, (int)HG, E, R, w.dhg_t, HG, w.h_in_t, E, G(lay->hcat_w), E)
                       : wgs(10, 4 * E, E, R, dg_t, HG, w.h_in_t, E, G(lay->hcat_w + (long)(E + D) * E), E);
  SatGemm g_wihx = wgs(11, 4 * E, E, R, dg_t, HG, w.emb_t, E, G(lay->wih), E + D);
  SatGemm g_wihc = wgs(12, 4 * E, D, R, dg_t, HG, w.gated_t, D, G(lay->wih + E), E + D);
  {
    SatZeroSeg seg[12];
    int nz = 0;
    if (att) {
      seg[nz++] = SatZeroSeg{w.dv_acc, 1, (long)B * E, (long)B * E};
      seg[nz++] = SatZeroSeg{w.dbv_acc, 1, B, B};
      seg[nz++] = SatZeroSeg{(float*)w.ticket, 1, B, B};
    }
    if (!d.bert && !accumulate) seg[nz++] = SatZeroSeg{G(lay->embedding), 1, (long)V * E, (long)V * E};
    if (w.gtickets) seg[nz++] = tickets_ph2;
    SatGemm* gs[5] = {&g_hcat, &g_wihx, &g_wihc, &g_init, &g_attw};
    prezero(gs, att ? 5 : 4, seg, nz);
    SAT_CHECK((hipError_t)sat_zero_segs(seg, nz, s));
  }
  const StepIO io{img_features, const_cast<float*>(alphas), d_alphas};
  for (int t = T1 - 1; t >= 0; --t) {
    {
      StepTimer st(d, 4, t);
      SAT_CHECK((hipError_t)bwd_lstm(c, w, sp, t, s));
    }
    if (att) {
      {
        StepTimer st(d, 5, t);
        SAT_CHECK((hipError_t)bwd_ggemm(c, w, sp, t, s));
      }
      StepTimer st(d, 6, t);
      SAT_CHECK((hipError_t)bwd_attn(c, w, sp, io, t, s, fg.dctx));
    }
    StepTimer st(d, 7, t);
    SAT_CHECK((hipError_t)bwd_dhgemm(c, w, sp, t, s));
  }

  if (att) {
    SAT_CHECK((hipError_t)sat_attention_dws_launch(w.Ws, w.uh_all, w.de_all, c.F(lay->v_w), B, L, E, T1, d.dtype,
                                                   w.dWs_acc, w.dWs_t, s));
    SAT_CHECK((hipError_t)sat_gemm_launch(g_attw, s));
  }
  SAT_CHECK((hipError_t)sat_tanh_pair_bwd(w.dh_rec, sp.dh, (long)B * E, w.dc, w.hc0, B, E, w.dpre0, w.dpre0_t,
                                          d.dtype, s));
  SAT_CHECK((hipError_t)sat_gemm_launch(g_init, s));
  {
    SatColsumSeg cs[6];
    int n = 0;
    if (att) {
      cs[n++] = {w.dWs_acc, SAT_F32, E, B * L, E, G(lay->attW_b), accumulate, nullptr};
      cs[n++] = {w.dv_acc, SAT_F32, E, B, E, G(lay->v_w), accumulate, nullptr};
      cs[n++] = {w.dbv_acc, SAT_F32, 1, B, 1, G(lay->v_b), accumulate, nullptr};
      cs[n++] = {w.dhg, SAT_F32, HG, R, E + D, G(lay->hcat_b), accumulate, nullptr};
    }
    cs[n++] = {w.dpre0, SAT_F32, 2 * E, B, 2 * E, G(lay->init_b), accumulate, nullptr};
    cs[n++] = {w.dhg + E + D, SAT_F32, HG, R, 4 * E, G(lay->hcat_b + E + D), accumulate, G(lay->bih)};
    SAT_CHECK((hipError_t)sat_colsum_multi(cs, n, w.colsum, s));
  }

  SAT_CHECK((hipError_t)sat_gemm_launch(g_hcat, s));
  SAT_CHECK((hipError_t)sat_gemm_launch(g_wihx, s));
  SAT_CHECK((hipError_t)sat_gemm_launch(g_wihc, s));
  if (!d.bert) {
    SAT_CHECK((hipError_t)dgrad(13, R, E, 4 * E, dg_t, HG, c.W(lay->wih), E + D, w.demb, E, d.ado ? w.dcomb : nullptr,
                                E));
    if (w.emb_ws)
      SAT_CHECK((hipError_t)sat_embed_scatter_add_sorted(w.demb, w.tok, R, E, G(lay->embedding), accumulate, w.emb_ws,
                                                         s));
    else
      SAT_CHECK((hipError_t)sat_embed_scatter_add(w.demb, w.tok, R, E, G(lay->embedding), s));
  }
  if (!fg.dctx) return 0;

  SAT_CHECK((hipError_t)dgrad(15, B, D, 2 * E, w.dpre0_t, 2 * E, c.W(lay->init_w), D, fg.mean_term, D));
  if (att) {
    SAT_CHECK((hipError_t)dgrad(14, B * L, D, E, w.dWs_t, E, c.W(lay->attW_w), D, fg.addend, D));
  } else {
    if (d.ado) SAT_CHECK((hipError_t)dgrad(8, R, D, E, w.dfz_t, E, c.W(lay->fz_w), D, w.dctx_head, D));
    SAT_CHECK((hipError_t)dgrad(14, R, D, 4 * E, dg_t, HG, c.W(lay->wih + E), E + D, fg.dctx, D,
                                d.ado ? w.dctx_head : nullptr, D));
  }
  FeatureGradArgs fa{};
  fa.B = B; fa.L = L; fa.D = D; fa.T1 = T1; fa.dtype = d.dtype;
  fa.alpha = alphas; fa.alpha_bs = (long)T1 * L; fa.alpha_ts = L;
  fa.dctx = fg.dctx; fa.dctx_bs = (long)T1 * D; fa.dctx_ts = D;
  fa.addend = fg.addend; fa.addend_ld = D;
  fa.mean_term = fg.mean_term; fa.mean_ld = D;
  fa.out = d_features; fa.out_ld = D;
  return sat_feature_grad_launch(fa, s);
}
}

extern "C" int sat_decoder_backward(const SatDecoderDims* dp, const SatDecoderLayout* lay, const float* params,
                                    const void* params_lp, const void* img_features, void* workspace,
                                    size_t workspace_bytes, const void* preds, const float* alphas,
                                    const void* d_preds, const float* d_alphas, float* grads, int accumulate,
                                    int phase, void* stream) {
  return decoder_backward(dp, lay, params, params_lp, img_features, workspace, workspace_bytes, preds, alphas, d_preds,
                          d_alphas, grads, accumulate, phase, stream, nullptr, nullptr, 0);
}

extern "C" int sat_decoder_backward_features(const SatDecoderDims* dp, const SatDecoderLayout* lay, const float* params,
                                             const void* params_lp, const void* img_features, void* workspace,
                                             size_t workspace_bytes, const void* preds, const float* alphas,
                                             const void* d_preds, const float* d_alphas, float* grads, int accumulate,
                                             int phase, void* stream, void* d_features, void* fg_workspace,
                                             size_t fg_workspace_bytes) {
  return decoder_backward(dp, lay, params, params_lp, img_features, workspace, workspace_bytes, preds, alphas, d_preds,
                          d_alphas, grads, accumulate, phase, stream, d_features, fg_workspace, fg_workspace_bytes);
}

extern "C" size_t sat_decoder_feature_grad_workspace_bytes(const SatDecoderDims* d) {
  if (check_dims(d)) return 0;
  FGWS w;
  return carve_fg(*d, nullptr, &w);
}

extern "C" int sat_decoder_step_bench(const SatDecoderDims* dp, const SatDecoderLayout* lay, const float* params,
                                      const void* params_lp, const void* img_features, void* workspace,
                                      size_t workspace_bytes, float* alphas, const float* d_alphas, int reps,
                                      float* us_out, void* stream) {
  SAT_CHECK((hipError_t)check_dims(dp));
  SAT_REQUIRE(lay && params && img_features && workspace && alphas && d_alphas && us_out && reps > 0);
  SAT_REQUIRE(dp->dtype == SAT_F32 || params_lp);
  SatPolicyScope scope(dp->policy);
  SatStampScope no_stamps(nullptr, 0);
  const SatDecoderDims& d = *dp;
  WS w;
  SAT_REQUIRE(carve(d, nullptr, &w) <= workspace_bytes);
  carve(d, (char*)workspace, &w);
  hipStream_t s = (hipStream_t)stream;
  Ctx c{d, *lay, params, params_lp, d.dtype == SAT_BF16 ? 2 : 4, d.T - 1, (long)d.B * (d.T - 1), 5L * d.E + d.D,
        use_transposed(d, *lay)};
  const Splits sp = splits_for(d, c.tr);
  const StepIO io{img_features, alphas, d_alphas};
  const int t = (d.T - 1) / 2;
  hipEvent_t e0, e1;
  SAT_CHECK(hipEventCreate(&e0));
  SAT_CHECK(hipEventCreate(&e1));
  int rc = 0;
  for (int k = 0; k < 8 && rc == 0; ++k) {
    us_out[k] = 0.f;
    if (!d.attention && (k == 1 || k == 2 || k == 5 || k == 6)) continue;
    for (int r = -1; r < reps && rc == 0; ++r) {
      if (r == 0) rc = (int)hipEventRecord(e0, s);
      switch (k) {
        case 0: rc = fwd_hgemm(c, w, sp, t, s); break;
        case 1: rc = fwd_attn(c, w, sp, io, t, s); break;
        case 2: rc = fwd_cgemm(c, w, sp, t, s); break;
        case 3: rc = fwd_lstm(c, w, sp, t, s); break;
        case 4: rc = bwd_lstm(c, w, sp, t, s); break;
        case 5: rc = bwd_ggemm(c, w, sp, t, s); break;
        case 6: rc = bwd_attn(c, w, sp, io, t, s); break;
        default: rc = bwd_dhgemm(c, w, sp, t, s); break;
      }
    }
    if (rc == 0) rc = (int)hipEventRecord(e1, s);
    if (rc == 0) rc = (int)hipEventSynchronize(e1);
    float ms = 0.f;
    if (rc == 0) rc = (int)hipEventElapsedTime(&ms, e0, e1);
    us_out[k] = ms * 1000.f / reps;
  }
  (void)hipEventDestroy(e0);
  (void)hipEventDestroy(e1);
  return rc;
}
```

show-attend-and-tell_amd/csrc/gemm.hip:

```cpp
#include "sat_common.h"
#include "sat_internal.h"

#include <type_traits>

namespace {

template <typename T> struct Cfg;
template <> struct Cfg<float> { static constexpr int BK = 16, VEC = 4, PAD = 4; };
template <> struct Cfg<bf16> { static constexpr int BK = 32, VEC = 8, PAD = 8; };

struct KArgs {
  int M, N, K;
  const void* A; long lda;
  const void* B; long ldb;
  void* C; long ldc; int c_dtype;
  float alpha, beta;
  const float* bias;
  const void* add1; long ld_add1; int add1_dtype;
  int act;
  void* aux; long ld_aux; int aux_dtype;
  long sA, sB, sC, s_add1, s_aux;
  SatConvGeom cv;
  int vecA, vecB;
  int splitk, kchunk;
// ... 270 lines not shown
  char* Xb = a.aux ? (char*)a.aux + z * a.s_aux * (a.aux_dtype == SAT_BF16 ? 2 : 4) : nullptr;
  if (a.c_dtype == SAT_BF16) {
    if (a.aux_dtype == SAT_BF16) epi((bf16*)Cb, (bf16*)Xb);
    else epi((bf16*)Cb, (float*)Xb);
  } else {
    if (a.aux_dtype == SAT_BF16) epi((float*)Cb, (bf16*)Xb);
    else epi((float*)Cb, (float*)Xb);
  }
}

template <typename T, int BM, int BN, int AMODE, bool TB>
int launch_cfg(const KArgs& k, int batch, hipStream_t s) {
  dim3 grid(sat_cdiv(k.N, BN), sat_cdiv(k.M, BM), batch * k.splitk);
  hipLaunchKernelGGL((gemm_kernel<T, BM, BN, AMODE, TB>), grid, dim3(256), 0, s, k);
  return (int)hipGetLastError();
}

template <typename T, int AMODE, bool TB>
int launch_tiles(const KArgs& k, int batch, hipStream_t s) {
  long t128 = (long)sat_cdiv(k.M, 128) * sat_cdiv(k.N, 128) * batch * k.splitk;
  long t64x128 = (long)sat_cdiv(k.M, 64) * sat_cdiv(k.N, 128) * batch * k.splitk;
  if (k.splitk == 1 && t128 >= 240) return launch_cfg<T, 128, 128, AMODE, TB>(k, batch, s);
  if (k.splitk == 1 && t64x128 >= 240) return launch_cfg<T, 64, 128, AMODE, TB>(k, batch, s);
  return launch_cfg<T, 64, 64, AMODE, TB>(k, batch, s);
}

template <typename T>
int launch_t(const KArgs& k, int amode, int tb, int batch, hipStream_t s) {
  if (amode == 2) return launch_tiles<T, 2, false>(k, batch, s);
  if (amode == 1) return tb ? launch_tiles<T, 1, true>(k, batch, s) : launch_tiles<T, 1, false>(k, batch, s);
  return tb ? launch_tiles<T, 0, true>(k, batch, s) : launch_tiles<T, 0, false>(k, batch, s);
}


}

int sat_gemm_launch(const SatGemm& g, hipStream_t s) {
  if (g.M <= 0 || g.N <= 0 || g.batch <= 0) return 0;
  SAT_REQUIRE(g.K >= 0 && g.A && g.B && g.C);
  SAT_REQUIRE(g.dtype == SAT_F32 || g.dtype == SAT_BF16);
  {
    int err = 0;
    if (sat_skinny_try(g, s, &err)) return err;
    if (sat_conv3x3_ws_try(g, s, &err)) return err;
    if (sat_conv_stream_try(g, s, &err)) return err;
    if (sat_conv_pipe_try(g, s, &err)) return err;
    if (sat_split_gemm_try(g, s, &err)) return err;
    if (sat_fast_gemm_try(g, s, &err)) return err;
  }
  const int vec = g.dtype == SAT_BF16 ? 8 : 4;
  KArgs k{};
  k.M = g.M; k.N = g.N; k.K = g.K;
  k.A = g.A; k.lda = g.lda; k.B = g.B; k.ldb = g.ldb;
  k.C = g.C; k.ldc = g.ldc; k.c_dtype = g.c_dtype;
  k.alpha = g.alpha; k.beta = g.beta; k.bias = g.bias;
  k.add1 = g.add1; k.ld_add1 = g.ld_add1; k.add1_dtype = g.add1_dtype;
  k.act = g.act; k.aux = g.aux; k.ld_aux = g.ld_aux; k.aux_dtype = g.aux_dtype;
  k.sA = g.sA; k.sB = g.sB; k.sC = g.sC; k.s_add1 = g.s_add1; k.s_aux = g.s_aux;
  k.cv = g.conv;
  int amode = g.conv.C > 0 ? 2 : (g.transA ? 1 : 0);
  if (amode == 2) {
    SAT_REQUIRE(g.conv.C % vec == 0 && sat_al16(g.A));
    SAT_REQUIRE(g.K == g.conv.KH * g.conv.KW * g.conv.C);
    SAT_REQUIRE(g.M == g.conv.N * g.conv.OH * g.conv.OW);
    k.vecA = 1;
  } else {
    k.vecA = sat_al16(g.A) && (g.lda % vec == 0) && (g.batch == 1 || g.sA % vec == 0);
  }
  k.vecB = sat_al16(g.B) && (g.ldb % vec == 0) && (g.batch == 1 || g.sB % vec == 0);
  k.splitk = 1;
  k.kchunk = g.K > 0 ? g.K : 1;
  k.partial = 0; k.split_stride = 0;
  const int bk = g.dtype == SAT_BF16 ? 32 : 16;
  if (g.partial_splits > 1) {
    SAT_REQUIRE(g.act == SAT_ACT_NONE && g.c_dtype == SAT_F32 && g.aux == nullptr && g.beta == 0.f &&
                g.batch == 1 && amode != 2);
    k.partial = 1; k.split_stride = g.split_stride;
    k.splitk = g.partial_splits;
    k.kchunk = sat_cdiv(sat_cdiv(g.K > 0 ? g.K : 1, g.partial_splits), bk) * bk;
    if (g.dtype == SAT_BF16) return launch_t<bf16>(k, amode, g.transB, g.batch, s);
    return launch_t<float>(k, amode, g.transB, g.batch, s);
  }
  const long tiles64 = (long)sat_cdiv(g.M, 64) * sat_cdiv(g.N, 64) * g.batch;
  const bool can_split = g.act == SAT_ACT_NONE && g.c_dtype == SAT_F32 && g.aux == nullptr &&
                         (g.beta == 0.f || g.beta == 1.f) && amode != 2 && g.batch == 1;
  if (can_split && g.dtype == SAT_BF16 && tiles64 < 200 && g.K >= 8 * bk) {
    int sk = (int)((400 + tiles64 - 1) / tiles64);
    sk = sk > 16 ? 16 : sk;
    const int max_by_k = g.K / (4 * bk);
    if (sk > max_by_k) sk = max_by_k;
    if (sk > 1) {
      int chunk = sat_cdiv(g.K, sk);
      chunk = sat_cdiv(chunk, bk) * bk;
      k.kchunk = chunk;
      k.splitk = sat_cdiv(g.K, chunk);
      if (g.beta == 0.f) {
        SAT_CHECK((hipError_t)sat_zero_rows((float*)g.C, g.ldc, g.M, g.N, s));
      }
    }
  }
  if (g.dtype == SAT_BF16) return launch_t<bf16>(k, amode, g.transB, g.batch, s);
  return launch_t<float>(k, amode, g.transB, g.batch, s);
}

namespace {
thread_local const SatPolicy* t_policy = nullptr;
const SatPolicy k_default_policy{};
}

const SatPolicy& sat_policy() { return t_policy ? *t_policy : k_default_policy; }

int sat_cu_count() {
  static const int cus = [] {
    int dev = 0, n = 0;
    if (hipGetDevice(&dev) != hipSuccess || hipDeviceGetAttribute(&n, hipDeviceAttributeMultiprocessorCount, dev) != hipSuccess || n <= 0)
      return 0;
    return n;
  }();
  return cus;
}

namespace {
__device__ __attribute__((aligned(16))) bf16 g_zero_line[64];
}
const bf16* sat_zero_line() {
  static const bf16* const zero = [] {
    void* p = nullptr;
    return hipGetSymbolAddress(&p, HIP_SYMBOL(g_zero_line)) == hipSuccess ? (const bf16*)p : nullptr;
  }();
  return zero;
}

namespace {
thread_local SatStamps t_stamps{};
thread_local bool t_stamps_set = false;
}
SatStamps sat_launch_stamps() {
  if (t_stamps_set) return t_stamps;
  return SatStamps{sat_policy().stamps, sat_policy().stamp_capacity};
}
SatStampScope::SatStampScope(uint64_t* p, int cap) : prev(t_stamps), prev_set(t_stamps_set) {
  t_stamps = SatStamps{p, cap};
  t_stamps_set = true;
}
SatStampScope::~SatStampScope() {
  t_stamps = prev;
  t_stamps_set = prev_set;
}
SatPolicyScope::SatPolicyScope(const SatPolicy* p) : prev(t_policy) { t_policy = p; }
SatPolicyScope::~SatPolicyScope() { t_policy = prev; }

extern "C" size_t sat_gemm_workspace_bytes(void) { return sat_split_gemm_ws_bytes(); }

extern "C" int sat_gemm(const SatGemmArgs* a, void* stream) {
  SAT_REQUIRE(a != nullptr);
  SatPolicyScope scope(a->policy);
  SatGemm g;
  if (a->workspace && a->workspace_bytes >= (int64_t)sat_split_gemm_ws_bytes()) {
    g.split_ws = (float*)a->workspace;
    g.split_ws_bytes = (long)(sat_split_gemm_ws_bytes() - kSatSplitTickets * 4);
    g.split_tickets = (unsigned*)((char*)a->workspace + g.split_ws_bytes);
  }
  g.M = a->M; g.N = a->N; g.K = a->K; g.dtype = a->dtype;
  g.A = a->A; g.lda = a->lda; g.transA = a->transA;
  g.B = a->B; g.ldb = a->ldb; g.transB = a->transB;
  g.C = a->C; g.ldc = a->ldc; g.c_dtype = a->c_dtype;
  g.alpha = a->alpha; g.beta = a->beta; g.bias = a->bias;
  g.add1 = a->add1; g.ld_add1 = a->ld_add1; g.add1_dtype = a->add1_dtype;
  g.act = a->act; g.aux = a->aux; g.ld_aux = a->ld_aux; g.aux_dtype = a->aux_dtype;
  return sat_gemm_launch(g, (hipStream_t)stream);
}

extern "C" int sat_conv2d_nhwc(const SatConvGeom* cg, int Cout, int dtype, const void* x, const void* w,
                               const float* bias, const void* residual, int relu, void* y, const SatPolicy* policy,
                               void* stream) {
  SAT_REQUIRE(cg != nullptr && x && w && y && Cout > 0);
  SatPolicyScope scope(policy);
  SatGemm g;
  g.conv = *cg;
  g.M = cg->N * cg->OH * cg->OW;
  g.N = Cout;
  g.K = cg->KH * cg->KW * cg->C;
  g.dtype = dtype;
  g.A = x; g.lda = 0;
  g.B = w; g.ldb = g.K; g.transB = 0;
  g.C = y; g.ldc = Cout; g.c_dtype = dtype;
  g.bias = bias;
  g.add1 = residual; g.ld_add1 = Cout; g.add1_dtype = dtype;
  g.act = relu ? SAT_ACT_RELU : SAT_ACT_NONE;
  return sat_gemm_launch(g, (hipStream_t)stream);
}
```

show-attend-and-tell_amd/csrc/gemmsplit.hip:

```cpp
#include "sat_common.h"
#include "sat_internal.h"
#include "sat_lds_pipe.h"

#ifndef SAT_SPLIT_RELEASE
#define SAT_SPLIT_RELEASE 0
#endif
#ifndef SAT_SPLIT_ACQUIRE
#define SAT_SPLIT_ACQUIRE 0
#endif
#ifndef SAT_SPLIT_DEBUG
#define SAT_SPLIT_DEBUG 0
#endif
#if SAT_SPLIT_DEBUG
__device__ unsigned g_sdbg[1 << 20];
__device__ unsigned g_sdbg_n;
__device__ unsigned g_sdbg_cs[64 * 256];
static unsigned g_sdbg_launch = 0;
#endif

namespace {

constexpr int SBN = 128, SBK = 64, SNSTG = 3;
constexpr int kMaxSplits = 8;
constexpr int kSplitCUs = 256;

template <int BM>
struct SGeom {
  static constexpr int WGN = BM == 256 ? 2 : 4;
  static constexpr int WGM = 8 / WGN;
  static constexpr int WTM = BM / WGM, WTN = SBN / WGN;
  static constexpr int MI = WTM / 16, NJ = WTN / 16;
  static constexpr int STAGE_A = BM * SBK * 2, STAGE_B = SBN * SBK * 2, STAGE = STAGE_A + STAGE_B;
  static constexpr int AI = STAGE_A / 1024 / 8, BI = STAGE_B / 1024 / 8, INSTR = AI + BI;
  static constexpr int EPI_LD = SBN + 4;
  static constexpr int EPI_BYTES = BM * EPI_LD * 4;
  static constexpr int LDS = SNSTG * STAGE;
  static_assert(WTM == 64 && MI == 4, "wave tiles are 64 rows high");
  static_assert(EPI_BYTES + 16 <= LDS, "epilogue tile + ticket word must fit in the ring");
};

struct SArgs {
  int M, N, K;
  const bf16* A; long lda;
  const bf16* B; long ldb;
  float* C; long ldc;
  int beta1;
  const float* add1; long ld_add1;
  int splits, kchunk;
  int a_mlim;
  int tiles_m, tiles_n;
  unsigned a_bytes, b_bytes, c_bytes, slab_bytes;
  float* slab;
  unsigned* tickets;
  SatStamps st;
  unsigned dbg_launch;
};

__device__ __forceinline__ uint4 f4u(f32x4 v) {
  return make_uint4(__float_as_uint(v[0]), __float_as_uint(v[1]), __float_as_uint(v[2]), __float_as_uint(v[3]));
}

template <int BM, bool AT, bool BT>
__device__ __forceinline__ void split_gemm_body(const SArgs& a) {
  using G = SGeom<BM>;
  constexpr int MI = G::MI, NJ = G::NJ, AI = G::AI, BI = G::BI;
  __shared__ __attribute__((aligned(16))) char smem[G::LDS];
  const int tid = threadIdx.x, lane = tid & 63;
  const int w = __builtin_amdgcn_readfirstlane(tid >> 6);
  const int wm = w / G::WGN, wn = w % G::WGN;

  int lin = blockIdx.x;
  {
    const int nwg = gridDim.x, q = nwg / 8, r = nwg % 8, x = lin % 8;
    lin = (x < r ? x * (q + 1) : r * (q + 1) + (x - r) * q) + lin / 8;
  }
  const int nt = lin % a.tiles_n;
  const int rest = lin / a.tiles_n;
  const int mt = rest % a.tiles_m, split = rest / a.tiles_m;
  const int m0 = mt * BM, n0 = nt * SBN;
  const int M = a.M, N = a.N;
  const int kbeg = split * a.kchunk, kend = min(a.K, kbeg + a.kchunk);
  const int nk = kend > kbeg ? (kend - kbeg + SBK - 1) / SBK : 0;

  const __amdgpu_buffer_rsrc_t rA = __builtin_amdgcn_make_buffer_rsrc((void*)a.A, (short)0, (int)a.a_bytes, 0x00020000);
  const __amdgpu_buffer_rsrc_t rB = __builtin_amdgcn_make_buffer_rsrc((void*)a.B, (short)0, (int)a.b_bytes, 0x00020000);
  int a_off[AI], a_k[AI];
  bool a_ok[AI];
#pragma unroll
  for (int j = 0; j < AI; ++j) {
    if constexpr (AT) {
      const int q = (w * AI + j) * 4 + (lane >> 4);
      const int kr = q & 63, ch = (lane & 15) ^ sat_swz256(kr);
      const int m = m0 + (q >> 6) * 128 + 8 * ch;
      a_ok[j] = m + 8 <= a.a_mlim;
      a_off[j] = m;
      a_k[j] = kr;
    } else {
      const int r = (w * AI + j) * 8 + (lane >> 3);
      const int ch = (lane & 7) ^ ((r >> 1) & 7);
      a_ok[j] = m0 + r < M;
      a_off[j] = (int)((long)(m0 + r) * a.lda);
      a_k[j] = 8 * ch;
    }
  }
  int b_off[BI], b_k[BI];
  bool b_ok[BI];
#pragma unroll
  for (int j = 0; j < BI; ++j) {
    if constexpr (BT) {
      const int kr = (w * BI + j) * 4 + (lane >> 4), ch = (lane & 15) ^ sat_swz256(kr);
      const int n = n0 + 8 * ch;
      b_ok[j] = n + 8 <= N;
      b_off[j] = n;
      b_k[j] = kr;
    } else {
      const int r = (w * BI + j) * 8 + (lane >> 3);
      const int ch = (lane & 7) ^ ((r >> 1) & 7);
      b_ok[j] = n0 + r < N;
      b_off[j] = (int)((long)(n0 + r) * a.ldb);
      b_k[j] = 8 * ch;
    }
  }
  auto stage = [&](int buf, int k0) {
    char* sa = smem + buf * G::STAGE;
    char* sb = sa + G::STAGE_A;
#pragma unroll
    for (int j = 0; j < AI; ++j) {
      const int k = k0 + a_k[j];
      const bool ok = a_ok[j] && k < kend;
      const unsigned off = AT ? 2u * (unsigned)((long)k * a.lda + a_off[j]) : 2u * (unsigned)(a_off[j] + k);
      sat_bdma16(rA, sa + (w * AI + j) * 1024, ok ? off : kSatOOB);
    }
#pragma unroll
    for (int j = 0; j < BI; ++j) {
      const int k = k0 + b_k[j];
      const bool ok = b_ok[j] && k < kend;
      const unsigned off = BT ? 2u * (unsigned)((long)k * a.ldb + b_off[j]) : 2u * (unsigned)(b_off[j] + k);
      sat_bdma16(rB, sb + (w * BI + j) * 1024, ok ? off : kSatOOB);
    }
  };

  const int fr = lane & 15, fh = lane >> 4, sw = (fr >> 1) & 7;
  const int am = wm * G::WTM;
  auto frags = [&](int buf, int h, bf16x8 (&fa)[MI], bf16x8 (&fb)[NJ]) {
    const char* sa = smem + buf * G::STAGE;
    const char* sb = sa + G::STAGE_A;
#pragma unroll
    for (int i = 0; i < MI; ++i) {
      if constexpr (AT) fa[i] = sat_frag_kmajor(sa + (am >> 7) * (64 * 256), h * 32, (am & 127) + i * 16, lane);
      else fa[i] = *(const bf16x8*)(sa + (am + i * 16 + fr) * 128 + 16 * ((h * 4 + fh) ^ sw));
    }
#pragma unroll
    for (int j = 0; j < NJ; ++j) {
      if constexpr (BT) fb[j] = sat_frag_kmajor(sb, h * 32, wn * G::WTN + j * 16, lane);
      else fb[j] = *(const bf16x8*)(sb + (wn * G::WTN + j * 16 + fr) * 128 + 16 * ((h * 4 + fh) ^ sw));
    }
  };
  f32x4 acc[MI][NJ];
#pragma unroll
  for (int i = 0; i < MI; ++i)
#pragma unroll
    for (int j = 0; j < NJ; ++j) acc[i][j] = f32x4{0.f, 0.f, 0.f, 0.f};
  auto mfma = [&](const bf16x8 (&fa)[MI], const bf16x8 (&fb)[NJ]) {
#pragma unroll
    for (int i = 0; i < MI; ++i)
#pragma unroll
      for (int j = 0; j < NJ; ++j) acc[i][j] = __builtin_amdgcn_mfma_f32_16x16x32_bf16(fa[i], fb[j], acc[i][j], 0, 0, 0);
  };

  bf16x8 xa[MI], xb[NJ], ya[MI], yb[NJ];
  if (nk > 0) {
    stage(0, kbeg);
    if (nk > 1) {
      stage(1, kbeg + SBK);
      sat_vm_lds_barrier<G::INSTR>();
    } else {
      sat_vm_lds_barrier<0>();
    }
    frags(0, 0, xa, xb);
    int cur = 0;
    for (int t = 0; t < nk; ++t) {
      frags(cur, 1, ya, yb);
      __builtin_amdgcn_sched_barrier(0);
      const bool dma = t + 2 < nk;
      if (dma) stage(cur == 0 ? 2 : cur - 1, kbeg + (t + 2) * SBK);
      __builtin_amdgcn_sched_barrier(0);
      __builtin_amdgcn_s_setprio(1);
      mfma(xa, xb);
      __builtin_amdgcn_s_setprio(0);
      __builtin_amdgcn_sched_barrier(0);
      if (t + 1 < nk) {
        if (dma) sat_vm_lds_barrier<G::INSTR>();
        else sat_vm_lds_barrier<0>();
        cur = cur == 2 ? 0 : cur + 1;
        frags(cur, 0, xa, xb);
      }
      __builtin_amdgcn_sched_barrier(0);
      __builtin_amdgcn_s_setprio(1);
      mfma(ya, yb);
      __builtin_amdgcn_s_setprio(0);
      __builtin_amdgcn_sched_barrier(0);
    }
  }

  if (a.splits > 1) {
    const long tile = (long)mt * a.tiles_n + nt;
    const __amdgpu_buffer_rsrc_t rS = sat_out_rsrc(a.slab, a.slab_bytes);
    constexpr unsigned PART = (unsigned)BM * SBN * 4;
    const unsigned tbase = (unsigned)(tile * a.splits) * PART;
    auto slot = [&](int i, int j) { return (unsigned)((((w * MI + i) * NJ + j) * 64 + lane) * 16); };
#pragma unroll
    for (int i = 0; i < MI; ++i)
#pragma unroll
      for (int j = 0; j < NJ; ++j) sat_st16<16>(rS, tbase + (unsigned)split * PART + slot(i, j), f4u(acc[i][j]));
    asm volatile("s_waitcnt vmcnt(0)" ::: "memory");
    __syncthreads();
    volatile unsigned* flag = (volatile unsigned*)(smem + G::EPI_BYTES);
    if (tid == 0) {
      if constexpr (SAT_SPLIT_RELEASE) {
        __builtin_amdgcn_fence(__ATOMIC_RELEASE, "agent");
        asm volatile("s_waitcnt vmcnt(0)" ::: "memory");
      }
      const unsigned prev = __hip_atomic_fetch_add(a.tickets + tile, 1u, __ATOMIC_RELAXED, __HIP_MEMORY_SCOPE_AGENT);
#if SAT_SPLIT_DEBUG
      {
        const unsigned i = atomicAdd(&g_sdbg_n, 1u);
        if (i < (1u << 18)) {
          g_sdbg[4 * i] = a.dbg_launch; g_sdbg[4 * i + 1] = (unsigned)tile; g_sdbg[4 * i + 2] = (unsigned)split;
          g_sdbg[4 * i + 3] = prev;
        }
      }
#endif
      if constexpr (SAT_SPLIT_ACQUIRE) {
        if (prev == (unsigned)(a.splits - 1)) {
          __builtin_amdgcn_fence(__ATOMIC_ACQUIRE, "agent");
          asm volatile("s_waitcnt vmcnt(0)" ::: "memory");
        }
      }
      *flag = prev;
    }
    __syncthreads();
    if (*flag != (unsigned)(a.splits - 1)) return;
    f32x4 tot[MI][NJ], part[MI][NJ];
    for (int s = 0; s < a.splits; ++s) {
      if (s == split) {
#pragma unroll
        for (int i = 0; i < MI; ++i)
#pragma unroll
          for (int j = 0; j < NJ; ++j) part[i][j] = acc[i][j];
      } else {
#pragma unroll
        for (int i = 0; i < MI; ++i)
#pragma unroll
          for (int j = 0; j < NJ; ++j) {
            const sat_u32x4 u = __builtin_amdgcn_raw_buffer_load_b128(rS, (int)(tbase + (unsigned)s * PART + slot(i, j)), 0, 16);
            part[i][j] = f32x4{__uint_as_float(u[0]), __uint_as_float(u[1]), __uint_as_float(u[2]), __uint_as_float(u[3])};
          }
      }
#pragma unroll
      for (int i = 0; i < MI; ++i)
#pragma unroll
        for (int j = 0; j < NJ; ++j) tot[i][j] = s == 0 ? part[i][j] : tot[i][j] + part[i][j];
    }
#pragma unroll
    for (int i = 0; i < MI; ++i)
#pragma unroll
      for (int j = 0; j < NJ; ++j) acc[i][j] = tot[i][j];
  }

#if SAT_SPLIT_DEBUG
  {
    unsigned x = 0;
#pragma unroll
    for (int i = 0; i < MI; ++i)
#pragma unroll
      for (int j = 0; j < NJ; ++j)
#pragma unroll
        for (int r = 0; r < 4; ++r) x ^= __float_as_uint(acc[i][j][r]) * (unsigned)(1 + ((i * NJ + j) * 4 + r));
    atomicXor(&g_sdbg_cs[(a.dbg_launch % 64) * 256 + ((long)mt * a.tiles_n + nt) % 256], x);
  }
#endif
  sat_vm_lds_barrier<0>();
  float* ep = (float*)smem;
#pragma unroll
  for (int j = 0; j < NJ; ++j) {
    const int cl = wn * G::WTN + j * 16 + fr;
#pragma unroll
    for (int i = 0; i < MI; ++i)
#pragma unroll
      for (int r = 0; r < 4; ++r) ep[(am + i * 16 + fh * 4 + r) * G::EPI_LD + cl] = acc[i][j][r];
  }
  __syncthreads();
  const int cc = tid & 15, r0 = tid >> 4;
  const int col = n0 + cc * 8;
  if (col >= N) return;
  const __amdgpu_buffer_rsrc_t rC = sat_out_rsrc(a.C, a.c_bytes);
#pragma unroll
  for (int it = 0; it < BM / 32; ++it) {
    const int rl = r0 + it * 32, row = m0 + rl;
    if (row >= M) break;
    float4 x0 = *(const float4*)(ep + rl * G::EPI_LD + cc * 8);
    float4 x1 = *(const float4*)(ep + rl * G::EPI_LD + cc * 8 + 4);
    const unsigned off = (unsigned)(((long)row * a.ldc + col) * 4);
    if (a.add1) {
      const float* p = a.add1 + (long)row * a.ld_add1 + col;
      x0 = f4add(x0, *(const float4*)p);
      x1 = f4add(x1, *(const float4*)(p + 4));
    }
    if (a.beta1) {
      const float* p = a.C + (long)row * a.ldc + col;
      x0 = f4add(x0, *(const float4*)p);
      x1 = f4add(x1, *(const float4*)(p + 4));
    }
    sat_st16<0>(rC, off, make_uint4(__float_as_uint(x0.x), __float_as_uint(x0.y), __float_as_uint(x0.z), __float_as_uint(x0.w)));
    sat_st16<0>(rC, off + 16, make_uint4(__float_as_uint(x1.x), __float_as_uint(x1.y), __float_as_uint(x1.z), __float_as_uint(x1.w)));
  }
}

template <int BM, bool AT, bool BT>
__global__ __launch_bounds__(512) void split_gemm_kernel(SArgs a) {
  const SatStampT0 t0 = sat_stamp_begin(a.st);
  split_gemm_body<BM, AT, BT>(a);
  sat_stamp_end(a.st, t0);
}


struct SPlan {
  int bm = 0, splits = 1, kchunk = 0, tiles_m = 0, tiles_n = 0;
  double us = 0;
};

constexpr double kKtileUs[2] = {0.73, 1.10};
constexpr double kEpiUs = 1.0;
constexpr double kPartUs[2] = {0.94, 1.87};
SPlan plan_split(const SatGemm& g, bool have_ws) {
  const SatPolicy& pol = sat_policy();
  const int nk = sat_cdiv(g.K, SBK);
  SPlan best;
  best.us = 1e30;
  for (int b = 0; b < 2; ++b) {
    const int bm = b ? 256 : 128;
    if ((pol.split_gemm == 2 && bm != 128) || (pol.split_gemm == 3 && bm != 256)) continue;
    const int tm = sat_cdiv(g.M, bm), tn = sat_cdiv(g.N, SBN);
    const long tiles = (long)tm * tn;
    for (int s = 1; s <= kMaxSplits; ++s) {
      if (pol.split_k > 0 && s != pol.split_k) continue;
      if (s > 1 && (!have_ws || tiles * s > kSplitCUs || nk < 2 * s)) continue;
      const int kch = sat_cdiv(nk, s);
      const int splits = sat_cdiv(nk, kch);
      if (splits != s) continue;
      const double us = sat_cdiv(tiles * s, kSplitCUs) * (kch * kKtileUs[b] + kEpiUs) + (s - 1) * kPartUs[b];
      if (us < best.us - 1e-9) {
        best.bm = bm; best.splits = s; best.kchunk = kch * SBK; best.tiles_m = tm; best.tiles_n = tn; best.us = us;
      }
    }
  }
  return best;
}

bool split_eligible(const SatGemm& g) {
  const int mode = sat_policy().split_gemm;
  if (mode == 1) return false;
  if (g.dtype != SAT_BF16 || g.c_dtype != SAT_F32 || g.batch != 1 || g.aux || g.bias || g.conv.C > 0 ||
      g.act != SAT_ACT_NONE || g.partial_splits > 1 || g.alpha != 1.f || (g.beta != 0.f && g.beta != 1.f))
    return false;
  if (g.M <= 0 || g.N <= 0 || g.K <= 0) return false;
  if (!(g.transA || g.transB) && !((long)sat_cdiv(g.M, 128) * sat_cdiv(g.N, 128) < 160 && g.K >= 1024)) return false;
  const bool at = g.transA != 0, bt = g.transB != 0;
  if (g.lda % 8 || g.ldb % 8 || g.ldc % 4 || g.N % 8) return false;
  if (at ? (g.M % 8 && !g.a_tail) : (g.K % 8 && !(g.a_tail && bt))) return false;
  if (!bt && g.K % 8) return false;
  if (!sat_al16(g.A) || !sat_al16(g.B) || !sat_al16(g.C)) return false;
  if (g.add1 && (g.add1_dtype != SAT_F32 || !sat_al16(g.add1) || g.ld_add1 % 4)) return false;
  const long a_bytes = at ? 2L * ((long)(g.K - 1) * g.lda + (g.a_tail ? sat_cdiv(g.M, 8) * 8 : g.M))
                          : 2L * ((long)(g.M - 1) * g.lda + sat_cdiv(g.K, 8) * 8);
  const long b_bytes = bt ? 2L * ((long)(g.K - 1) * g.ldb + g.N) : 2L * ((long)(g.N - 1) * g.ldb + g.K);
  const long c_bytes = 4L * ((long)(g.M - 1) * g.ldc + g.N);
  if (a_bytes >= (1L << 31) || b_bytes >= (1L << 31) || c_bytes >= (1L << 31)) return false;
  if (mode == 0 && g.K < 512) return false;
  return true;
}

}

size_t sat_split_gemm_ws_bytes() {
  static_assert(kSatSplitTickets >= kSplitCUs, "a split launch has at most kSplitCUs tiles");
  return (size_t)kSplitCUs * 256 * SBN * 4 + kSatSplitTickets * 4;
}

static bool split_takes(const SatGemm& g) {
  if (!split_eligible(g)) return false;
  if (g.split_ws && g.split_tickets) return true;
  return plan_split(g, true).splits <= 1;
}

int sat_split_gemm_takes(const SatGemm& g) { return split_takes(g) ? 1 : 0; }

int sat_split_gemm_try(const SatGemm& g, hipStream_t s, int* err) {
  *err = 0;
  if (!split_takes(g)) return 0;
  const bool have_ws = g.split_ws && g.split_tickets;
  const SPlan p = plan_split(g, have_ws);
  if (p.bm == 0) return 0;
  const bool at = g.transA != 0, bt = g.transB != 0;
  SArgs a{};
  a.M = g.M; a.N = g.N; a.K = g.K;
  a.A = (const bf16*)g.A; a.lda = g.lda; a.B = (const bf16*)g.B; a.ldb = g.ldb;
  a.C = (float*)g.C; a.ldc = g.ldc;
  a.beta1 = g.beta != 0.f;
  a.add1 = (const float*)g.add1; a.ld_add1 = g.ld_add1;
  a.splits = p.splits; a.kchunk = p.kchunk;
  a.a_mlim = at && g.a_tail ? sat_cdiv(g.M, 8) * 8 : g.M;
  a.tiles_m = p.tiles_m; a.tiles_n = p.tiles_n;
  a.a_bytes = (unsigned)(at ? 2L * ((long)(g.K - 1) * g.lda + a.a_mlim)
                            : 2L * ((long)(g.M - 1) * g.lda + sat_cdiv(g.K, 8) * 8));
  a.b_bytes = (unsigned)(bt ? 2L * ((long)(g.K - 1) * g.ldb + g.N) : 2L * ((long)(g.N - 1) * g.ldb + g.K));
  a.c_bytes = (unsigned)(4L * ((long)(g.M - 1) * g.ldc + g.N));
  if (p.splits > 1) {
    const long slab = (long)p.tiles_m * p.tiles_n * p.splits * p.bm * SBN * 4;
    SAT_REQUIRE(slab <= g.split_ws_bytes && (long)p.tiles_m * p.tiles_n <= kSplitCUs);
    a.slab = g.split_ws; a.slab_bytes = (unsigned)slab;
    a.tickets = g.split_tickets;
    if (!g.tickets_zeroed)
      SAT_CHECK((hipError_t)sat_zero_rows((float*)g.split_tickets, (long)p.tiles_m * p.tiles_n, 1,
                                          (long)p.tiles_m * p.tiles_n, s));
  }
  a.st = sat_launch_stamps();
#if SAT_SPLIT_DEBUG
  a.dbg_launch = ++g_sdbg_launch;
#endif
  const dim3 grid((unsigned)((long)p.tiles_m * p.tiles_n * p.splits));
  if (p.bm == 256) {
    if (at && bt) hipLaunchKernelGGL((split_gemm_kernel<256, true, true>), grid, dim3(512), 0, s, a);
    else if (at) hipLaunchKernelGGL((split_gemm_kernel<256, true, false>), grid, dim3(512), 0, s, a);
    else if (bt) hipLaunchKernelGGL((split_gemm_kernel<256, false, true>), grid, dim3(512), 0, s, a);
    else hipLaunchKernelGGL((split_gemm_kernel<256, false, false>), grid, dim3(512), 0, s, a);
  } else {
    if (at && bt) hipLaunchKernelGGL((split_gemm_kernel<128, true, true>), grid, dim3(512), 0, s, a);
    else if (at) hipLaunchKernelGGL((split_gemm_kernel<128, true, false>), grid, dim3(512), 0, s, a);
    else if (bt) hipLaunchKernelGGL((split_gemm_kernel<128, false, true>), grid, dim3(512), 0, s, a);
    else hipLaunchKernelGGL((split_gemm_kernel<128, false, false>), grid, dim3(512), 0, s, a);
  }
  *err = (int)hipGetLastError();
  return 1;
}

#if SAT_SPLIT_DEBUG
extern "C" int sat_split_debug_read(unsigned* out, int n4, unsigned* count) {
  SAT_CHECK(hipDeviceSynchronize());
  SAT_CHECK(hipMemcpyFromSymbol(count, HIP_SYMBOL(g_sdbg_n), sizeof(unsigned)));
  const unsigned m = *count * 4 < (unsigned)n4 ? *count * 4 : (unsigned)n4;
  if (m) SAT_CHECK(hipMemcpyFromSymbol(out, HIP_SYMBOL(g_sdbg), m * sizeof(unsigned)));
  const unsigned z = 0;
  SAT_CHECK(hipMemcpyToSymbol(HIP_SYMBOL(g_sdbg_n), &z, sizeof(unsigned)));
  return 0;
}
extern "C" int sat_split_debug_checksums(unsigned* out) {
  SAT_CHECK(hipDeviceSynchronize());
  SAT_CHECK(hipMemcpyFromSymbol(out, HIP_SYMBOL(g_sdbg_cs), 64 * 256 * sizeof(unsigned)));
  static unsigned zeros[64 * 256] = {};
  SAT_CHECK(hipMemcpyToSymbol(HIP_SYMBOL(g_sdbg_cs), zeros, sizeof(zeros)));
  return 0;
}
#endif
```

show-attend-and-tell_amd/csrc/sat_common.h:

```cpp
#pragma once
#include <hip/hip_runtime.h>
#include <stdint.h>
#include <stddef.h>

#include "../../include/sat_hip.h"

typedef float f32x4 __attribute__((ext_vector_type(4)));
typedef __bf16 bf16x8 __attribute__((ext_vector_type(8)));
typedef __bf16 bf16;

#define SAT_CHECK(x)                                   \
  do {                                                 \
    hipError_t e__ = (x);                              \
    if (e__ != hipSuccess) return (int)e__;            \
  } while (0)
#define SAT_LAUNCH_CHECK() SAT_CHECK(hipGetLastError())
#define SAT_REQUIRE(cond)                              \
  do {                                                 \
    if (!(cond)) return SAT_ERR_INVALID;               \
  } while (0)

static inline int sat_cdiv(long a, long b) { return (int)((a + b - 1) / b); }
static inline bool sat_al16(const void* p) { return ((uintptr_t)p & 15) == 0; }

__attribute__((visibility("hidden"))) int sat_cu_count();
__attribute__((visibility("hidden"))) const bf16* sat_zero_line();

const SatPolicy& sat_policy();
struct SatPolicyScope {
  const SatPolicy* prev;
  explicit SatPolicyScope(const SatPolicy* p);
  ~SatPolicyScope();
  SatPolicyScope(const SatPolicyScope&) = delete;
  SatPolicyScope& operator=(const SatPolicyScope&) = delete;
};

struct SatStamps {
  uint64_t* p = nullptr;
  int cap = 0;
};
struct SatStampT0 {
  uint64_t t0;
  bool on;
};
__device__ __forceinline__ SatStampT0 sat_stamp_begin(const SatStamps& st) {
  if (!st.p || st.p[0] == 0) return SatStampT0{0, false};
  return SatStampT0{__builtin_amdgcn_s_memrealtime(), true};
}
__device__ __forceinline__ void sat_stamp_end(const SatStamps& st, SatStampT0 t) {
  if (!t.on) return;
  __syncthreads();
  const int w = blockIdx.x + gridDim.x * (blockIdx.y + gridDim.y * blockIdx.z);
  if (threadIdx.x == 0 && w < st.cap) {
    const uint64_t t1 = __builtin_amdgcn_s_memrealtime();
    *(ulonglong2*)(st.p + 2 + 2 * (long)w) = make_ulonglong2(t.t0, t1);
  }
}

SatStamps sat_launch_stamps();
struct SatStampScope {
  SatStamps prev;
  bool prev_set;
  SatStampScope(uint64_t* p, int cap);
  ~SatStampScope();
  SatStampScope(const SatStampScope&) = delete;
  SatStampScope& operator=(const SatStampScope&) = delete;
};
__device__ __forceinline__ float ld_as_f32(const void* p, long i, int dt) {
  return dt == SAT_BF16 ? (float)((const bf16*)p)[i] : ((const float*)p)[i];
}
__device__ __forceinline__ void st_from_f32(void* p, long i, int dt, float v) {
  if (dt == SAT_BF16) ((bf16*)p)[i] = (bf16)v;
  else ((float*)p)[i] = v;
}
template <typename T> __device__ __forceinline__ float to_f32(T v) { return (float)v; }
template <typename T> __device__ __forceinline__ T from_f32(float v) { return (T)v; }

__device__ __forceinline__ float sat_sigmoid(float x) { return 1.0f / (1.0f + __expf(-x)); }

__device__ __forceinline__ float apply_act(float v, int act) {
  switch (act) {
    case SAT_ACT_RELU: return v > 0.f ? v : 0.f;
    case SAT_ACT_TANH: return tanhf(v);
    case SAT_ACT_SIGMOID: return 1.0f / (1.0f + expf(-v));
    default: return v;
  }
}

#ifndef SAT_OUT_CPOL
#define SAT_OUT_CPOL 16
#endif
#ifndef SAT_OUT8_CPOL
#define SAT_OUT8_CPOL 0
#endif
typedef unsigned sat_u32x2 __attribute__((ext_vector_type(2)));
typedef unsigned sat_u32x4 __attribute__((ext_vector_type(4)));
__device__ __forceinline__ __amdgpu_buffer_rsrc_t sat_out_rsrc(const void* base, long bytes) {
  return __builtin_amdgcn_make_buffer_rsrc((void*)base, (short)0, (int)(bytes < 0x7fffffffL ? bytes : 0x7fffffffL),
                                           0x00020000);
}
constexpr unsigned kSatOOB = 0x80000000u;
__device__ __forceinline__ __amdgpu_buffer_rsrc_t sat_in_rsrc(const void* base, long bytes) { return sat_out_rsrc(base, bytes); }
__device__ __forceinline__ uint4 sat_ld16(__amdgpu_buffer_rsrc_t r, unsigned byte_off) {
  const sat_u32x4 v = __builtin_amdgcn_raw_buffer_load_b128(r, (int)byte_off, 0, 0);
  return make_uint4(v.x, v.y, v.z, v.w);
}
__device__ __forceinline__ float4 sat_ld16f(__amdgpu_buffer_rsrc_t r, unsigned byte_off) {
  const uint4 u = sat_ld16(r, byte_off);
  return make_float4(__uint_as_float(u.x), __uint_as_float(u.y), __uint_as_float(u.z), __uint_as_float(u.w));
}
__device__ __forceinline__ float sat_ld4f(__amdgpu_buffer_rsrc_t r, unsigned byte_off) {
  return __uint_as_float((unsigned)__builtin_amdgcn_raw_buffer_load_b32(r, (int)byte_off, 0, 0));
}
template <int CPOL = SAT_OUT_CPOL>
__device__ __forceinline__ void sat_st16(__amdgpu_buffer_rsrc_t r, unsigned byte_off, uint4 u) {
  __builtin_amdgcn_raw_buffer_store_b128(sat_u32x4{u.x, u.y, u.z, u.w}, r, (int)byte_off, 0, CPOL);
}
__device__ __forceinline__ void sat_st8(__amdgpu_buffer_rsrc_t r, unsigned byte_off, sat_u32x2 u) {
  __builtin_amdgcn_raw_buffer_store_b64(u, r, (int)byte_off, 0, SAT_OUT8_CPOL);
}

template <int CPOL = SAT_OUT_CPOL>
__device__ __forceinline__ void sat_st_pair16(__amdgpu_buffer_rsrc_t r, unsigned offA, unsigned offB, sat_u32x2 a, sat_u32x2 b,
                                          bool okA, bool okB) {
  const bool odd = (threadIdx.x >> 4) & 1;
  const sat_u32x2 send = odd ? a : b;
  const unsigned gx = (unsigned)__shfl_xor((int)send.x, 16, 64), gy = (unsigned)__shfl_xor((int)send.y, 16, 64);
  const uint4 u = odd ? make_uint4(gx, gy, b.x, b.y) : make_uint4(a.x, a.y, gx, gy);
  if (odd ? okB : okA) sat_st16<CPOL>(r, odd ? offB - 8 : offA, u);
}

__device__ __forceinline__ float wave_sum(float v) {
#pragma unroll
  for (int o = 32; o > 0; o >>= 1) v += __shfl_xor(v, o, 64);
  return v;
}
__device__ __forceinline__ float wave_max(float v) {
#pragma unroll
  for (int o = 32; o > 0; o >>= 1) v = fmaxf(v, __shfl_xor(v, o, 64));
  return v;
}

struct SatGemm {
  int M = 0, N = 0, K = 0;
  int dtype = SAT_F32;
  const void* A = nullptr; long lda = 0; int transA = 0;
  const void* B = nullptr; long ldb = 0; int transB = 0;
  void* C = nullptr; long ldc = 0; int c_dtype = SAT_F32;
  float alpha = 1.f, beta = 0.f;
  const float* bias = nullptr;
  const void* add1 = nullptr; long ld_add1 = 0; int add1_dtype = SAT_F32;
  int act = SAT_ACT_NONE;
  void* aux = nullptr; long ld_aux = 0; int aux_dtype = SAT_BF16;
  int batch = 1; long sA = 0, sB = 0, sC = 0, s_add1 = 0, s_aux = 0;
  SatConvGeom conv{};
  int partial_splits = 0; long split_stride = 0;
  int a_tail = 0;
  int c_zeroed = 0;
  float* split_ws = nullptr; long split_ws_bytes = 0;
  unsigned* split_tickets = nullptr;
  int tickets_zeroed = 0;
};

int sat_gemm_launch(const SatGemm& g, hipStream_t s);
int sat_fast_gemm_try(const SatGemm& g, hipStream_t s, int* err);
int sat_split_gemm_try(const SatGemm& g, hipStream_t s, int* err);
int sat_split_gemm_takes(const SatGemm& g);
size_t sat_split_gemm_ws_bytes();
constexpr size_t kSatSplitTickets = 256;
int sat_conv_pipe_try(const SatGemm& g, hipStream_t s, int* err);
int sat_conv_stream_try(const SatGemm& g, hipStream_t s, int* err);
int sat_skinny_try(const SatGemm& g, hipStream_t s, int* err);
int sat_skinny_splits(int M, int N, int K);
int sat_conv3x3_ws_try(const SatGemm& g, hipStream_t s, int* err);
```

show-attend-and-tell_amd/csrc/skinny.hip:

```cpp
#include "sat_common.h"
#include "sat_internal.h"
#include "sat_lds_pipe.h"

namespace {

constexpr int SK_COLS = 32;
constexpr int SK_RLD = SK_COLS + 4;
constexpr int SK_KW = 128;

struct SkArgs {
  int M, N, K, kc, kw;
  const bf16* A; long lda;
  const bf16* W; long ldw;
  float* C; long ldc; long split_stride;
  const float* bias;
  int nb1;
  const bf16* A2; long lda2;
  const bf16* W2; long ldw2;
  float* C2; long ldc2; long split_stride2;
  SatStamps st;
};

template <int MB, int NW>
__device__ __forceinline__ void skinny_tile(const bf16* __restrict__ A, long lda, int M, int row0,
// ... 216 lines not shown
    }
    if ((q & 7) == 0 && row < a.B) {
      a.pval[(long)bx * a.B + row] = best;
      a.pidx[(long)bx * a.B + row] = bi;
    }
  }
  sat_stamp_end(st, t0);
}

constexpr int HO_K = 512, HO_COLS = 64, HO_BLK = 64, HO_Q = 4, HO_QB = HO_K * 2 / HO_Q;
template <int MB>
__global__ __launch_bounds__(256) void head_out_lds_kernel(HeadOutArgs a, SatStamps st) {
  static_assert(MB % 2 == 0, "DMA instructions cover 4 rows: MB * 16 / 4 per quarter, a multiple of the 4 waves");
  constexpr int MR = MB * 16, INSTR = MR / 4 / 4;
  const SatStampT0 t0 = sat_stamp_begin(st);
  __shared__ __attribute__((aligned(16))) char sA0[MR * HO_QB];
  __shared__ __attribute__((aligned(16))) char sA1[MR * HO_QB];
  __shared__ __attribute__((aligned(16))) char sA2[MR * HO_QB];
  __shared__ __attribute__((aligned(16))) char sA3[MR * HO_QB];
  auto quarter = [&](int q) -> char* { return q == 0 ? sA0 : q == 1 ? sA1 : q == 2 ? sA2 : sA3; };
  __shared__ float s_bv[4][MR];
  __shared__ int s_bi[4][MR];
  const int lane = threadIdx.x & 63, fr = lane & 15, fh = lane >> 4;
  const int w = __builtin_amdgcn_readfirstlane(threadIdx.x >> 6);
  const int n0 = blockIdx.x * HO_COLS + w * 16;
  const bf16* wr = a.w + (long)min(n0 + fr, a.V - 1) * HO_K + 8 * fh;
  bf16x8 bw[HO_K / 32];
#pragma unroll
  for (int ks = 0; ks < HO_K / 32; ++ks) bw[ks] = *(const bf16x8*)(wr + ks * 32);
  float bias4[4];
#pragma unroll
  for (int r = 0; r < 4; ++r) bias4[r] = a.bias[min(n0 + 4 * fh + r, a.V - 1)];
  const __amdgpu_buffer_rsrc_t rX = __builtin_amdgcn_make_buffer_rsrc(
      (void*)a.x, (short)0, (int)(2L * ((long)(a.B - 1) * a.x_ld + HO_K)), 0x00020000);
#pragma unroll
  for (int q = 0; q < HO_Q; ++q)
#pragma unroll
    for (int j = 0; j < INSTR; ++j) {
      const int r0 = 4 * (w + 4 * j), row = r0 + (lane >> 4);
      const int off = (int)(2L * ((long)min(row, a.B - 1) * a.x_ld + q * (HO_K / HO_Q) + 8 * ((lane & 15) ^ (row & 15))));
      sat_bdma16(rX, quarter(q) + r0 * HO_QB, (unsigned)off);
    }
  f32x4 acc[MB];
#pragma unroll
  for (int i = 0; i < MB; ++i) acc[i] = f32x4{0.f, 0.f, 0.f, 0.f};
  bf16x8 af[2][MB];
  auto frag = [&](int ks, bf16x8 (&dst)[MB]) {
    const int q = ks / 4, c = 4 * (ks % 4) + fh;
#pragma unroll
    for (int i = 0; i < MB; ++i) dst[i] = *(const bf16x8*)(quarter(q) + (i * 16 + fr) * HO_QB + 16 * (c ^ fr));
  };
  sat_static_for<HO_K / 32>([&](auto KS) {
    constexpr int ks = decltype(KS)::value;
    if constexpr (ks == 0) {
      sat_vm_barrier<(HO_Q - 1) * INSTR>();
      frag(0, af[0]);
    }
    if constexpr (ks + 1 < HO_K / 32 && (ks + 1) % 4 != 0) frag(ks + 1, af[(ks + 1) & 1]);
    __builtin_amdgcn_sched_barrier(0);
#pragma unroll
    for (int i = 0; i < MB; ++i) acc[i] = __builtin_amdgcn_mfma_f32_16x16x32_bf16(bw[ks], af[ks & 1][i], acc[i], 0, 0, 0);
    __builtin_amdgcn_sched_barrier(0);
    if constexpr (ks + 1 < HO_K / 32 && (ks + 1) % 4 == 0) {
      sat_vm_barrier<(HO_Q - 1 - (ks + 1) / 4) * INSTR>();
      frag(ks + 1, af[(ks + 1) & 1]);
    }
  });
  const bool vec = (a.V & 3) == 0 && (((uintptr_t)a.preds | (uintptr_t)(a.preds_ld * 2)) & 7) == 0;
#pragma unroll
  for (int i = 0; i < MB; ++i) {
    const int row = i * 16 + fr, n = n0 + 4 * fh;
    float best = -INFINITY;
    int bi = 0x7fffffff;
    uint2 pu;
    bf16* pv = (bf16*)&pu;
#pragma unroll
    for (int r = 0; r < 4; ++r) {
      float x = acc[i][r] + bias4[r];
      if (a.relu) x = x > 0.f ? x : 0.f;
      pv[r] = (bf16)x;
      if (row < a.B && n + r < a.V) {
        const float xr = (float)pv[r];
        if (sat_argmax_better(xr, n + r, best, bi)) { best = xr; bi = n + r; }
      }
    }
    if (row < a.B) {
      bf16* dst = a.preds + (long)row * a.preds_ld + n;
      if (vec && n + 3 < a.V) {
        *(uint2*)dst = pu;
      } else {
#pragma unroll
        for (int r = 0; r < 4; ++r)
          if (n + r < a.V) dst[r] = pv[r];
      }
    }
#pragma unroll
    for (int o = 16; o < 64; o <<= 1) {
      const float ov = __shfl_xor(best, o, 64);
      const int oi = __shfl_xor(bi, o, 64);
      if (sat_argmax_better(ov, oi, best, bi)) { best = ov; bi = oi; }
    }
    if (fh == 0) { s_bv[w][row] = best; s_bi[w][row] = bi; }
  }
  __syncthreads();
  if ((int)threadIdx.x < min(MR, a.B)) {
    const int row = threadIdx.x;
    float best = s_bv[0][row];
    int bi = s_bi[0][row];
#pragma unroll
    for (int v = 1; v < 4; ++v)
      if (sat_argmax_better(s_bv[v][row], s_bi[v][row], best, bi)) { best = s_bv[v][row]; bi = s_bi[v][row]; }
    a.pval[(long)blockIdx.x * a.B + row] = best;
    a.pidx[(long)blockIdx.x * a.B + row] = bi;
  }
  sat_stamp_end(st, t0);
}

}

int sat_skinny_try(const SatGemm& g, hipStream_t st, int* err) {
  *err = 0;
  SkArgs a;
  int nw;
  if (!skinny_shape(g, sat_policy().skinny, &a, &nw) || !skinny_ptrs(g)) return 0;
  a.st = sat_launch_stamps();
  const dim3 grid(g.N / SK_COLS, g.partial_splits > 1 ? g.partial_splits : 1);
  if (g.M <= 32) launch_mb<2>(nw, grid, st, a);
  else if (g.M <= 64) launch_mb<4>(nw, grid, st, a);
  else launch_mb<8>(nw, grid, st, a);
  *err = (int)hipGetLastError();
  return 1;
}

int sat_skinny_dual_try(const SatGemm& g1, const SatGemm& g2, hipStream_t st, int* err) {
  *err = 0;
  SkArgs a, b;
  int nw1, nw2;
  const int mode = sat_policy().skinny;
  if (!skinny_shape(g1, mode, &a, &nw1) || !skinny_ptrs(g1) || !skinny_shape(g2, mode, &b, &nw2) || !skinny_ptrs(g2))
    return 0;
  if (g1.M != g2.M || g1.K != g2.K || a.kc != b.kc || a.kw != b.kw || nw1 != nw2 || g2.bias) return 0;
  const int S1 = g1.partial_splits > 1 ? g1.partial_splits : 1, S2 = g2.partial_splits > 1 ? g2.partial_splits : 1;
  if (S1 != S2) return 0;
  a.A2 = b.A; a.lda2 = b.lda; a.W2 = b.W; a.ldw2 = b.ldw; a.C2 = b.C; a.ldc2 = b.ldc; a.split_stride2 = b.split_stride;
  a.st = sat_launch_stamps();
  const dim3 grid(g1.N / SK_COLS + g2.N / SK_COLS, S1);
  if (g1.M <= 32) launch_mb<2>(nw1, grid, st, a);
  else if (g1.M <= 64) launch_mb<4>(nw1, grid, st, a);
  else launch_mb<8>(nw1, grid, st, a);
  *err = (int)hipGetLastError();
  return 1;
}

int sat_skinny_splits(int M, int N, int K) {
  if (sat_policy().skinny == 1 || M > 128 || N % SK_COLS || K % 256 || K < 1024) return 0;
  return K / 256;
}


int sat_greedy_supported(int B, int E) { return B >= 1 && B <= 128 && E % 64 == 0 && E >= 64 && E <= 1024; }

int sat_greedy_head_mid(const HeadMidArgs& a, hipStream_t s) {
  if (!sat_greedy_supported(a.B, a.E)) return (int)hipErrorInvalidValue;
  const dim3 grid(a.E / SK_COLS, sat_cdiv(a.B, 32));
  if (head_waves(a.E) == 4) hipLaunchKernelGGL(head_mid_kernel<4>, grid, dim3(256), 0, s, a, head_kw(a.E));
  else hipLaunchKernelGGL(head_mid_kernel<8>, grid, dim3(512), 0, s, a, head_kw(a.E));
  return (int)hipGetLastError();
}

static bool head_out_lds(int B, int E) { return E == HO_K && B <= 128; }
int sat_greedy_head_blocks(int B, int V, int E) { return sat_cdiv(V, head_out_lds(B, E) ? HO_BLK : SK_COLS); }

int sat_greedy_head_out(const HeadOutArgs& a, hipStream_t s) {
  if (!sat_greedy_supported(a.B, a.E) || a.V < 1) return (int)hipErrorInvalidValue;
  const SatStamps st = sat_launch_stamps();
  if (head_out_lds(a.B, a.E)) {
    if (((uintptr_t)a.x & 15) || (a.x_ld & 7) || ((uintptr_t)a.w & 15)) return (int)hipErrorInvalidValue;
    const dim3 grid(sat_cdiv(a.V, HO_COLS));
    if (a.B <= 32) hipLaunchKernelGGL(head_out_lds_kernel<2>, grid, dim3(256), 0, s, a, st);
    else if (a.B <= 64) hipLaunchKernelGGL(head_out_lds_kernel<4>, grid, dim3(256), 0, s, a, st);
    else hipLaunchKernelGGL(head_out_lds_kernel<8>, grid, dim3(256), 0, s, a, st);
    return (int)hipGetLastError();
  }
  const dim3 grid(sat_cdiv(a.V, SK_COLS));
  const int nw = head_waves(a.E), kw = head_kw(a.E);
#define SAT_HEAD_OUT(MB)                                                                                            \
  do {                                                                                                            \
    if (nw == 4) hipLaunchKernelGGL((head_out_kernel<MB, 4>), grid, dim3(256), 0, s, a, kw, st);                   \
    else hipLaunchKernelGGL((head_out_kernel<MB, 8>), grid, dim3(512), 0, s, a, kw, st);                           \
  } while (0)
  if (a.B <= 32) SAT_HEAD_OUT(2);
  else if (a.B <= 64) SAT_HEAD_OUT(4);
  else SAT_HEAD_OUT(8);
#undef SAT_HEAD_OUT
  return (int)hipGetLastError();
}
```

show-attend-and-tell_amd/ops.py:

```python
import ctypes

import torch

from . import _lib as L


def linear(x, weight, bias=None, act=L.ACT_NONE, out_dtype=None, weight_lp=None):
    L.require_device(x, weight)
    M, K = x.shape
    N = weight.shape[0]
    dt = L.dtype_code(x.dtype)
    if dt == L.SAT_F32:
        w = weight
    elif weight_lp is not None:
        w = weight_lp
    else:
        w = cast_(weight.contiguous(), torch.empty(weight.shape, device=weight.device, dtype=torch.bfloat16))
    out_dtype = out_dtype or torch.float32
    y = torch.empty(M, N, device=x.device, dtype=out_dtype)
    gemm(x, w, y, bias=bias, act=act)
    return y


_GEMM_WS = {}


def gemm_workspace(device, stream):
    if torch.cuda.is_current_stream_capturing():
        return torch.empty(int(L.lib().sat_gemm_workspace_bytes()), dtype=torch.uint8, device=device)
    key = (torch.device(device).index, stream.value or 0)
    ws = _GEMM_WS.get(key)
    if ws is None:
        ws = torch.empty(int(L.lib().sat_gemm_workspace_bytes()), dtype=torch.uint8, device=device)
        _GEMM_WS[key] = ws
    return ws


def _may_split(A, C, bias, aux, act, K):
    return (A.dtype == torch.bfloat16 and C.dtype == torch.float32 and bias is None and aux is None
            and act == L.ACT_NONE and K >= 512)


def gemm(A, B, C, *, transA=False, transB=False, alpha=1.0, beta=0.0, bias=None, add1=None, act=L.ACT_NONE,
         aux=None, policy=None, workspace=True):
    L.require_device(A, B, C)
    dt = L.dtype_code(A.dtype)
    if B.dtype != A.dtype:
        raise TypeError("sat_amd.gemm: A and B must share a dtype")
    M = A.shape[1] if transA else A.shape[0]
    K = A.shape[0] if transA else A.shape[1]
    N = B.shape[1] if transB else B.shape[0]
    Kb = B.shape[0] if transB else B.shape[1]
    if Kb != K or C.shape[0] != M or C.shape[1] != N:
        raise ValueError(f"sat_amd.gemm: shape mismatch A{tuple(A.shape)} B{tuple(B.shape)} C{tuple(C.shape)}")
    for t in (A, B, C, add1, aux):
        if t is not None and t.stride(-1) != 1:
            raise ValueError("sat_amd.gemm: operands must be row-major with unit inner stride")
    a = L.SatGemmArgs()
    a.M, a.N, a.K, a.dtype = M, N, K, dt
    a.A, a.lda, a.transA = A.data_ptr(), A.stride(0), int(transA)
    a.B, a.ldb, a.transB = B.data_ptr(), B.stride(0), int(transB)
    a.C, a.ldc, a.c_dtype = C.data_ptr(), C.stride(0), L.dtype_code(C.dtype)
    a.alpha, a.beta = alpha, beta
    a.bias = bias.data_ptr() if bias is not None else None
    if add1 is not None:
        a.add1, a.ld_add1, a.add1_dtype = add1.data_ptr(), add1.stride(0), L.dtype_code(add1.dtype)
    a.act = act
    if aux is not None:
        a.aux, a.ld_aux, a.aux_dtype = aux.data_ptr(), aux.stride(0), L.dtype_code(aux.dtype)
    a.policy = L.policy_ptr(policy)
    stream = L.stream_of(C)
    if workspace is True:
        workspace = (gemm_workspace(C.device, stream)
                     if policy is not None or _may_split(A, C, bias, aux, act, K) else None)
    if workspace is not None:
        a.workspace, a.workspace_bytes = workspace.data_ptr(), workspace.numel() * workspace.element_size()
    L.check(L.lib().sat_gemm(ctypes.byref(a), stream), "sat_gemm")
    return C


def cast_(src, dst):
    L.require_device(src, dst)
    assert src.numel() == dst.numel() and src.is_contiguous() and dst.is_contiguous()
    L.check(L.lib().sat_cast(L.ptr(src), L.dtype_code(src.dtype), L.ptr(dst), L.dtype_code(dst.dtype),
                             src.numel(), L.stream_of(dst)), "sat_cast")
    return dst


def nchw_to_nhwc(x, c_pad, dtype):
    L.require_device(x)
    x = x.contiguous() if not x.is_contiguous() else x
    if x.dtype != torch.float32:
        raise TypeError("images must be float32 (post-Normalize domain, train.py:27-32)")
    N, C, H, W = x.shape
    y = torch.empty(N, H, W, c_pad, device=x.device, dtype=dtype)
    L.check(L.lib().sat_nchw_to_nhwc(N, C, H, W, c_pad, L.dtype_code(dtype), L.ptr(x), L.ptr(y), L.stream_of(y)),
            "sat_nchw_to_nhwc")
    return y


def nchw_to_s2d(x, dtype):
    L.require_device(x)
    x = x.contiguous() if not x.is_contiguous() else x
    if x.dtype != torch.float32:
        raise TypeError("images must be float32 (post-Normalize domain, train.py:27-32)")
    N, C, H, W = x.shape
    y = torch.empty(N, H // 2, W // 2, 16, device=x.device, dtype=dtype)
    L.check(L.lib().sat_nchw_to_s2d(N, C, H, W, L.dtype_code(dtype), L.ptr(x), L.ptr(y), L.stream_of(y)),
            "sat_nchw_to_s2d")
    return y


IMAGE_MEAN = (0.485, 0.456, 0.406)
IMAGE_STD = (0.229, 0.224, 0.225)


def images_to_input(packed, layout=L.IMG_NCHW, dtype=torch.float32, c_pad=8, size=(224, 224),
                    mean=IMAGE_MEAN, std=IMAGE_STD):
    L.require_device(packed.pixels, packed.offsets, packed.sizes)
    lib = L.lib()
    B = packed.count
    OH, OW = size
    mx = lib.sat_images_max_downscale()
    if packed.max_h > mx * OH or packed.max_w > mx * OW:
        raise ValueError(f"images_to_input: {packed.max_h}x{packed.max_w} exceeds the {mx}x downscale limit "
                         f"to {OH}x{OW}")
    dev = packed.pixels.device
    if layout == L.IMG_NCHW:
        if dtype != torch.float32:
            raise TypeError("images_to_input: the NCHW layout is the reference's float32 tensor")
        out = torch.empty(B, 3, OH, OW, device=dev, dtype=torch.float32)
    elif layout == L.IMG_NHWC:
        out = torch.empty(B, OH, OW, c_pad, device=dev, dtype=dtype)
    elif layout == L.IMG_S2D16:
        out = torch.empty(B, OH // 2, OW // 2, 16, device=dev, dtype=dtype)
    else:
        raise ValueError(f"images_to_input: unknown layout {layout}")
    ws_bytes = lib.sat_images_workspace_bytes(B, OH, OW)
    ws = torch.empty(ws_bytes, device=dev, dtype=torch.uint8)
    m = (ctypes.c_float * 3)(*mean)
    sd = (ctypes.c_float * 3)(*std)
    L.check(lib.sat_images_to_input(L.ptr(packed.pixels), L.ptr(packed.offsets), L.ptr(packed.sizes), B,
                                    packed.max_h, packed.max_w, OH, OW, m, sd, layout, c_pad, L.dtype_code(dtype),
                                    L.ptr(out), L.ptr(ws), ws_bytes, L.stream_of(out)), "sat_images_to_input")
    return out


class ProjectedResidual:

    def __init__(self, x, f):
        self.x, self.f = x, f

    def out_hw(self):
        s = self.f[2]
        return (self.x.shape[1] - 1) // s + 1, (self.x.shape[2] - 1) // s + 1

    def materialize(self, policy=None):
        return conv2d_nhwc(self.x, *self.f, False, policy=policy)


def conv1x1_proj_supported(M, K, N, Kp, stride, N2, dtype, policy=None):
    return bool(L.lib().sat_conv1x1_proj_supported(M, K, N, Kp, stride, N2, L.dtype_code(dtype), L.policy_ptr(policy)))


def _proj_launch(x, c3, proj, c1_next, policy):
    w, b = c3[0], c3[1]
    wp, bp, stride, pad = proj.f
    B, H, W, K = x.shape
    N, Kp = w.shape[0], proj.x.shape[3]
    w1, b1 = (c1_next[0], c1_next[1]) if c1_next is not None else (None, None)
    N2 = w1.shape[0] if w1 is not None else 0
    ts = [x, w, b, proj.x, wp, bp, w1, b1]
    if pad != 0 or tuple(wp.shape) != (N, 1, 1, Kp) or tuple(w.shape[1:]) != (1, 1, K) or proj.out_hw() != (H, W) \
            or proj.x.shape[0] != B or any(t.dtype != x.dtype for t in (w, proj.x, wp) + ((w1,) if N2 else ())) \
            or any(t is not None and (not t.is_contiguous() or t.data_ptr() % 16) for t in ts) \
            or proj.x.numel() * proj.x.element_size() >= 1 << 31 \
            or not conv1x1_proj_supported(B * H * W, K, N, Kp, stride, N2, x.dtype, policy):
        return None
    L.require_device(*[t for t in ts if t is not None])
    y = torch.empty(B, H, W, N, device=x.device, dtype=x.dtype)
    x1 = torch.empty(B, H, W, N2, device=x.device, dtype=x.dtype) if N2 else None
    L.check(L.lib().sat_conv1x1_proj(B, proj.x.shape[1], proj.x.shape[2], stride, K, N, Kp, N2, L.dtype_code(x.dtype),
                                     L.ptr(x), L.ptr(w), L.ptr(b), L.ptr(proj.x), L.ptr(wp), L.ptr(bp), L.ptr(y),
                                     L.ptr(w1), L.ptr(b1), L.ptr(x1), L.policy_ptr(policy), L.stream_of(y)),
            "sat_conv1x1_proj")
    return y, x1


def conv2d_nhwc(x, w, bias, stride, pad, relu, residual=None, out=None, out_hw=None, policy=None):
    L.require_device(x, w)
    if isinstance(residual, ProjectedResidual):
        if relu and stride == 1 and pad == 0 and out is None and out_hw is None and w.shape[1] == w.shape[2] == 1:
            r = _proj_launch(x, (w, bias), residual, None, policy)
            if r is not None:
                return r[0]
        residual = residual.materialize(policy)
    N, H, W, C = x.shape
    Cout, KH, KW, Cw = w.shape
    assert Cw == C, (w.shape, x.shape)
    if out_hw is None:
        OH = (H + 2 * pad - KH) // stride + 1
        OW = (W + 2 * pad - KW) // stride + 1
    else:
        OH, OW = out_hw
    y = out if out is not None else torch.empty(N, OH, OW, Cout, device=x.device, dtype=x.dtype)
    g = L.SatConvGeom(N, H, W, C, KH, KW, stride, pad, OH, OW)
    if residual is not None:
        assert residual.shape == y.shape and residual.dtype == y.dtype
    L.check(L.lib().sat_conv2d_nhwc(ctypes.byref(g), Cout, L.dtype_code(x.dtype), L.ptr(x), L.ptr(w), L.ptr(bias),
                                    L.ptr(residual), int(relu), L.ptr(y), L.policy_ptr(policy), L.stream_of(y)),
            "sat_conv2d_nhwc")
    return y


def _stem_geom(x, w, stride, pad, out_hw):
    N, H, W, C = x.shape
    Cout, KH, KW, Cw = w.shape
    assert Cw == C, (w.shape, x.shape)
    if out_hw is None:
        out_hw = ((H + 2 * pad - KH) // stride + 1, (W + 2 * pad - KW) // stride + 1)
    return L.SatConvGeom(N, H, W, C, KH, KW, stride, pad, out_hw[0], out_hw[1])


def conv_stem_pool_supported(x, w, stride, pad, relu, pool, out_hw=None, policy=None):
    g = _stem_geom(x, w, stride, pad, out_hw)
    return bool(L.lib().sat_conv_stem_pool_supported(ctypes.byref(g), w.shape[0], L.dtype_code(x.dtype), int(relu),
                                                     pool[0], pool[1], pool[2], L.policy_ptr(policy)))


def conv_stem_pool(x, w, bias, stride, pad, relu, pool, out_hw=None, policy=None):
    L.require_device(x, w, bias)
# ... 180 lines not shown
```

Before: 22540 images/s.

## Batch independent decoder backward GEMMs into one grouped split-K kernel launch

Adds a grouped GEMM launcher that plans several independent products, covering tiles, split-K counts, slab offsets and tickets, and runs them as one kernel whose blocks are partitioned across products. The decoder backward now groups the fh/fz weight gradients with their dgrads, and separately the attention, init, hcat and wih weight gradients with the embedding dgrad, when rows ≥ 2560. The goal is to remove per-launch overhead and tail underutilisation from many small sequential GEMMs. In exchange it needs extra workspace slabs and group tickets, and products that cannot be grouped fall back to individual launches.

```diff
diff --git a/include/sat_hip.h b/include/sat_hip.h
--- a/include/sat_hip.h
+++ b/include/sat_hip.h
@@ -78,6 +78,24 @@
 
 int sat_gemm(const SatGemmArgs* args, void* stream);
 size_t sat_gemm_workspace_bytes(void);
+
+typedef struct {
+  int M, N, K;
+  int tile_rows, splits;
+} SatGemmGroupShape;
+typedef struct {
+  int tile_rows, splits, kchunk, tiles_m, tiles_n;
+  int first_block, blocks;
+  int64_t slab_offset, slab_bytes;
+  int ticket_offset, tickets;
+  int fallback;
+} SatGemmGroupPlan;
+int sat_gemm_group(const SatGemmArgs* args, int n, void* workspace, int64_t workspace_bytes, void* stream);
+size_t sat_gemm_group_workspace_bytes(void);
+int sat_gemm_group_plan(const SatGemmGroupShape* shapes, int n, int64_t slab_bytes, int tickets, SatGemmGroupPlan* plan);
+int sat_gemm_group_block(const SatGemmGroupPlan* plan, int n, int block, int* product, int* tile_m, int* tile_n,
+                         int* split);
+int64_t sat_gemm_group_launches(void);
 int sat_cast(const void* x, int x_dtype, void* y, int y_dtype, int64_t n, void* stream);
 
 int sat_mean_rows_abi(const void* a, int B, int L, int D, int dtype, float* out_f32, void* out_t, void* stream);
diff --git a/show-attend-and-tell_amd/_lib.py b/show-attend-and-tell_amd/_lib.py
--- a/show-attend-and-tell_amd/_lib.py
+++ b/show-attend-and-tell_amd/_lib.py
@@ -49,6 +49,16 @@
                 ("workspace", c_void_p), ("workspace_bytes", c_int64)]
 
 
+class SatGemmGroupShape(ctypes.Structure):
+    _fields_ = [(n, c_int) for n in ("M", "N", "K", "tile_rows", "splits")]
+
+
+class SatGemmGroupPlan(ctypes.Structure):
+    _fields_ = [(n, c_int) for n in ("tile_rows", "splits", "kchunk", "tiles_m", "tiles_n", "first_block", "blocks")] + \
+               [("slab_offset", c_int64), ("slab_bytes", c_int64), ("ticket_offset", c_int), ("tickets", c_int),
+                ("fallback", c_int)]
+
+
 class SatDecoderDims(ctypes.Structure):
     _fields_ = [("B", c_int), ("L", c_int), ("D", c_int), ("E", c_int), ("V", c_int), ("T", c_int),
                 ("tf", c_int), ("ado", c_int), ("attention", c_int), ("bert", c_int), ("training", c_int),
@@ -77,6 +87,13 @@
     ("sat_error_string", ctypes.c_char_p, [c_int]),
     ("sat_gemm", c_int, [ctypes.POINTER(SatGemmArgs), c_void_p]),
     ("sat_gemm_workspace_bytes", c_size_t, []),
+    ("sat_gemm_group", c_int, [ctypes.POINTER(SatGemmArgs), c_int, c_void_p, c_int64, c_void_p]),
+    ("sat_gemm_group_workspace_bytes", c_size_t, []),
+    ("sat_gemm_group_plan", c_int, [ctypes.POINTER(SatGemmGroupShape), c_int, c_int64, c_int,
+                                    ctypes.POINTER(SatGemmGroupPlan)]),
+    ("sat_gemm_group_block", c_int, [ctypes.POINTER(SatGemmGroupPlan), c_int, c_int, ctypes.POINTER(c_int),
+                                     ctypes.POINTER(c_int), ctypes.POINTER(c_int), ctypes.POINTER(c_int)]),
+    ("sat_gemm_group_launches", c_int64, []),
     ("sat_cast", c_int, [c_void_p, c_int, c_void_p, c_int, c_int64, c_void_p]),
     ("sat_mean_rows_abi", c_int, [c_void_p, c_int, c_int, c_int, c_int, c_void_p, c_void_p, c_void_p]),
     ("sat_nchw_to_nhwc", c_int, [c_int, c_int, c_int, c_int, c_int, c_int, c_void_p, c_void_p, c_void_p]),
diff --git a/show-attend-and-tell_amd/csrc/decoder.hip b/show-attend-and-tell_amd/csrc/decoder.hip
--- a/show-attend-and-tell_amd/csrc/decoder.hip
+++ b/show-attend-and-tell_amd/csrc/decoder.hip
@@ -15,6 +15,8 @@
   unsigned* ticket;
   float* gsplit;
   unsigned* gtickets;
+  float* ggroup;
+  size_t ggroup_bytes;
   float* xt;
   float* fzp;
   float* am_val;
@@ -22,6 +24,8 @@
   void* emb_ws;
 };
 constexpr int kTicketBlocks = 16;
+constexpr int kGroupMinRows = 2560;
+constexpr int kGroups = 2;
 
 struct Splits { int h, c, g, dh, i; };
 constexpr int kSplitTargetDefault = 192;
@@ -152,10 +156,18 @@
   c.take(w->ticket, B * 4);
   if (d.dtype == SAT_BF16) {
     c.take(w->gsplit, sat_split_gemm_ws_bytes() - kSatSplitTickets * 4);
-    c.take(w->gtickets, (size_t)kTicketBlocks * kSatSplitTickets * 4);
+    c.take(w->gtickets, ((size_t)kTicketBlocks * kSatSplitTickets + (size_t)kGroups * kSatGroupTickets) * 4);
+    auto sb = [](size_t M, size_t N, size_t K) { return sat_gemm_group_slab_bound((int)M, (int)N, (int)K); };
+    const size_t four = sb(E, E, R) + sb(E, D, R) + sb(R, E, E) + sb(R, D, E);
+    const size_t post = sb(E, D, B * L) + sb(2 * E, D, B) + sb(HG, E, R) + sb(4 * E, E, R) + sb(4 * E, D, R) +
+                        sb(R, E, 4 * E);
+    w->ggroup_bytes = R >= (size_t)kGroupMinRows ? (four > post ? four : post) : 0;
+    c.take(w->ggroup, w->ggroup_bytes);
   } else {
     w->gsplit = nullptr;
     w->gtickets = nullptr;
+    w->ggroup = nullptr;
+    w->ggroup_bytes = 0;
   }
   c.take(w->demb, R * E * f);
   c.take(w->dpre0, B * 2 * E * f); c.take(w->dpre0_t, B * 2 * E * ts);
@@ -430,9 +442,9 @@
   g.tickets_zeroed = 1;
 }
 
-int dgrad_launch(const Ctx& c, int M, int N, int K, const void* X, long ldx, const void* Wt, long ldw, float* out,
-                 long ldo, hipStream_t s, const float* add1 = nullptr, long ld_add1 = 0, int splits = 0,
-                 long split_stride = 0, int a_tail = 0, const SplitWS* sw = nullptr) {
+SatGemm dgrad_gemm(const Ctx& c, int M, int N, int K, const void* X, long ldx, const void* Wt, long ldw, float* out,
+                   long ldo, const float* add1 = nullptr, long ld_add1 = 0, int splits = 0, long split_stride = 0,
+                   int a_tail = 0, const SplitWS* sw = nullptr) {
   SatGemm g;
   use_split(g, sw);
   g.a_tail = a_tail;
@@ -441,7 +453,13 @@
   g.A = X; g.lda = ldx; g.B = Wt; g.ldb = ldw; g.transB = 1;
   g.C = out; g.ldc = ldo; g.c_dtype = SAT_F32;
   g.add1 = add1; g.ld_add1 = ld_add1; g.add1_dtype = SAT_F32;
-  return sat_gemm_launch(g, s);
+  return g;
+}
+int dgrad_launch(const Ctx& c, int M, int N, int K, const void* X, long ldx, const void* Wt, long ldw, float* out,
+                 long ldo, hipStream_t s, const float* add1 = nullptr, long ld_add1 = 0, int splits = 0,
+                 long split_stride = 0, int a_tail = 0, const SplitWS* sw = nullptr) {
+  return sat_gemm_launch(dgrad_gemm(c, M, N, K, X, ldx, Wt, ldw, out, ldo, add1, ld_add1, splits, split_stride, a_tail,
+                                    sw), s);
 }
 
 int bwd_ggemm(const Ctx& c, const WS& w, const Splits& sp, int t, hipStream_t s) {
@@ -875,6 +893,15 @@
   const SatZeroSeg tickets_ph1{(float*)w.gtickets, 1, 8L * kSatSplitTickets, 8L * kSatSplitTickets};
   const SatZeroSeg tickets_ph2{(float*)w.gtickets + 8L * kSatSplitTickets, 1, 8L * kSatSplitTickets,
                                8L * kSatSplitTickets};
+  unsigned* const group_tickets = w.gtickets ? w.gtickets + (long)kTicketBlocks * kSatSplitTickets : nullptr;
+  const SatZeroSeg gtickets_ph1{(float*)group_tickets, 1, kSatGroupTickets, kSatGroupTickets};
+  const SatZeroSeg gtickets_ph2{(float*)group_tickets + kSatGroupTickets, 1, kSatGroupTickets, kSatGroupTickets};
+  auto group = [&](int k, const SatGemm* gs, int n) {
+    return sat_gemm_group_launch(gs, nullptr, n, w.ggroup, (long)w.ggroup_bytes,
+                                 group_tickets ? group_tickets + (long)k * kSatGroupTickets : nullptr,
+                                 kSatGroupTickets, s, 1);
+  };
+  const bool grouping = w.ggroup_bytes > 0 && sat_policy().split_gemm != 4;
   auto wgs = [&](int blk, int M, int N, int K, const void* X, long ldx, const void* Y, long ldy, float* out, long ldo,
                  int a_tail = 0) {
     SatGemm g = wg(M, N, K, X, ldx, Y, ldy, out, ldo, a_tail);
@@ -891,6 +918,10 @@
   auto dgrad = [&](int blk, int M, int N, int K, const void* X, long ldx, const void* Wt, long ldw, float* out,
                    long ldo, const float* add1 = nullptr, long ld_add1 = 0) {
     return dgrad_launch(c, M, N, K, X, ldx, Wt, ldw, out, ldo, s, add1, ld_add1, 0, 0, 0, &sws[blk]);
+  };
+  auto dgg = [&](int blk, int M, int N, int K, const void* X, long ldx, const void* Wt, long ldw, float* out, long ldo,
+                 const float* add1 = nullptr, long ld_add1 = 0, int a_tail = 0) {
+    return dgrad_gemm(c, M, N, K, X, ldx, Wt, ldw, out, ldo, add1, ld_add1, 0, 0, a_tail, &sws[blk]);
   };
   auto colsum = [&](const void* X, int dt, long ld, int rows, int N, float* out, float* out2 = nullptr,
                     int cols_readable = 0) {
@@ -916,9 +947,10 @@
       SatGemm gfz = wgs(3, E, D, R, w.dfz_t, E, w.ctx_t, D, G(lay->fz_w), D);
       {
         SatGemm* gs[3] = {&gfo, &gfh, &gfz};
-        SatZeroSeg seg[4];
+        SatZeroSeg seg[5];
         int nseg = 0;
         if (w.gtickets) seg[nseg++] = tickets_ph1;
+        if (grouping) seg[nseg++] = gtickets_ph1;
         prezero(gs, 3, seg, nseg);
         SAT_CHECK((hipError_t)sat_zero_segs(seg, nseg, s));
       }
@@ -926,14 +958,21 @@
       SAT_CHECK((hipError_t)dgrad_launch(c, R, E, V, dpre, ldp, c.W(lay->fout_w), E, w.dcomb, E, s, nullptr, 0, 0, 0,
                                          VP != V, &sws[1]));
       SAT_CHECK((hipError_t)sat_ado_bwd_split(w.dcomb, w.fh, w.fz, (long)R * E, d.dtype, w.dfh_t, w.dfz_t, s));
-      SAT_CHECK((hipError_t)sat_gemm_launch(gfh, s));
-      SAT_CHECK((hipError_t)sat_gemm_launch(gfz, s));
       const SatColsumSeg cs[3] = {{dpre, d.dtype, ldp, R, V, G(lay->fout_b), accumulate, nullptr, ldp != V},
                                   {w.dfh_t, d.dtype, E, R, E, G(lay->fh_b), accumulate, nullptr},
                                   {w.dfz_t, d.dtype, E, R, E, G(lay->fz_b), accumulate, nullptr}};
-      SAT_CHECK((hipError_t)sat_colsum_multi(cs, 3, w.colsum, s));
-      SAT_CHECK((hipError_t)dgrad(4, R, E, E, w.dfh_t, E, c.W(lay->fh_w), E, w.dhd, E));
-      if (att) SAT_CHECK((hipError_t)dgrad(5, R, D, E, w.dfz_t, E, c.W(lay->fz_w), D, w.dctx_head, D));
+      if (grouping) {
+        const SatGemm four[4] = {gfh, gfz, dgg(4, R, E, E, w.dfh_t, E, c.W(lay->fh_w), E, w.dhd, E),
+                                 dgg(5, R, D, E, w.dfz_t, E, c.W(lay->fz_w), D, w.dctx_head, D)};
+        SAT_CHECK((hipError_t)group(0, four, att ? 4 : 3));
+        SAT_CHECK((hipError_t)sat_colsum_multi(cs, 3, w.colsum, s));
+      } else {
+        SAT_CHECK((hipError_t)sat_gemm_launch(gfh, s));
+        SAT_CHECK((hipError_t)sat_gemm_launch(gfz, s));
+        SAT_CHECK((hipError_t)sat_colsum_multi(cs, 3, w.colsum, s));
+        SAT_CHECK((hipError_t)dgrad(4, R, E, E, w.dfh_t, E, c.W(lay->fh_w), E, w.dhd, E));
+        if (att) SAT_CHECK((hipError_t)dgrad(5, R, D, E, w.dfz_t, E, c.W(lay->fz_w), D, w.dctx_head, D));
+      }
     } else {
       const void* dpre = d_preds;
       long ldp = (phase & 8) ? VP : V;
@@ -975,6 +1014,7 @@
     }
     if (!d.bert && !accumulate) seg[nz++] = SatZeroSeg{G(lay->embedding), 1, (long)V * E, (long)V * E};
     if (w.gtickets) seg[nz++] = tickets_ph2;
+    if (grouping) seg[nz++] = gtickets_ph2;
     SatGemm* gs[5] = {&g_hcat, &g_wihx, &g_wihc, &g_init, &g_attw};
     prezero(gs, att ? 5 : 4, seg, nz);
     SAT_CHECK((hipError_t)sat_zero_segs(seg, nz, s));
@@ -1000,11 +1040,11 @@
   if (att) {
     SAT_CHECK((hipError_t)sat_attention_dws_launch(w.Ws, w.uh_all, w.de_all, c.F(lay->v_w), B, L, E, T1, d.dtype,
                                                    w.dWs_acc, w.dWs_t, s));
-    SAT_CHECK((hipError_t)sat_gemm_launch(g_attw, s));
+    if (!grouping) SAT_CHECK((hipError_t)sat_gemm_launch(g_attw, s));
   }
   SAT_CHECK((hipError_t)sat_tanh_pair_bwd(w.dh_rec, sp.dh, (long)B * E, w.dc, w.hc0, B, E, w.dpre0, w.dpre0_t,
                                           d.dtype, s));
-  SAT_CHECK((hipError_t)sat_gemm_launch(g_init, s));
+  if (!grouping) SAT_CHECK((hipError_t)sat_gemm_launch(g_init, s));
   {
     SatColsumSeg cs[6];
     int n = 0;
@@ -1019,12 +1059,26 @@
     SAT_CHECK((hipError_t)sat_colsum_multi(cs, n, w.colsum, s));
   }
 
-  SAT_CHECK((hipError_t)sat_gemm_launch(g_hcat, s));
-  SAT_CHECK((hipError_t)sat_gemm_launch(g_wihx, s));
-  SAT_CHECK((hipError_t)sat_gemm_launch(g_wihc, s));
+  if (!grouping) {
+    SAT_CHECK((hipError_t)sat_gemm_launch(g_hcat, s));
+    SAT_CHECK((hipError_t)sat_gemm_launch(g_wihx, s));
+    SAT_CHECK((hipError_t)sat_gemm_launch(g_wihc, s));
+    if (!d.bert)
+      SAT_CHECK((hipError_t)dgrad(13, R, E, 4 * E, dg_t, HG, c.W(lay->wih), E + D, w.demb, E,
+                                  d.ado ? w.dcomb : nullptr, E));
+  } else {
+    SatGemm set[6];
+    int n = 0;
+    if (att) set[n++] = g_attw;
+    set[n++] = g_init;
+    set[n++] = g_hcat;
+    set[n++] = g_wihx;
+    set[n++] = g_wihc;
+    if (!d.bert)
+      set[n++] = dgg(13, R, E, 4 * E, dg_t, HG, c.W(lay->wih), E + D, w.demb, E, d.ado ? w.dcomb : nullptr, E);
+    SAT_CHECK((hipError_t)group(1, set, n));
+  }
   if (!d.bert) {
-    SAT_CHECK((hipError_t)dgrad(13, R, E, 4 * E, dg_t, HG, c.W(lay->wih), E + D, w.demb, E, d.ado ? w.dcomb : nullptr,
-                                E));
     if (w.emb_ws)
       SAT_CHECK((hipError_t)sat_embed_scatter_add_sorted(w.demb, w.tok, R, E, G(lay->embedding), accumulate, w.emb_ws,
                                                          s));
diff --git a/show-attend-and-tell_amd/csrc/gemm.hip b/show-attend-and-tell_amd/csrc/gemm.hip
--- a/show-attend-and-tell_amd/csrc/gemm.hip
+++ b/show-attend-and-tell_amd/csrc/gemm.hip
@@ -446,14 +446,12 @@
 
 extern "C" size_t sat_gemm_workspace_bytes(void) { return sat_split_gemm_ws_bytes(); }
 
-extern "C" int sat_gemm(const SatGemmArgs* a, void* stream) {
-  SAT_REQUIRE(a != nullptr);
-  SatPolicyScope scope(a->policy);
+static SatGemm gemm_from_args(const SatGemmArgs* a, void* workspace, int64_t workspace_bytes) {
   SatGemm g;
-  if (a->workspace && a->workspace_bytes >= (int64_t)sat_split_gemm_ws_bytes()) {
-    g.split_ws = (float*)a->workspace;
+  if (workspace && workspace_bytes >= (int64_t)sat_split_gemm_ws_bytes()) {
+    g.split_ws = (float*)workspace;
     g.split_ws_bytes = (long)(sat_split_gemm_ws_bytes() - kSatSplitTickets * 4);
-    g.split_tickets = (unsigned*)((char*)a->workspace + g.split_ws_bytes);
+    g.split_tickets = (unsigned*)((char*)workspace + g.split_ws_bytes);
   }
   g.M = a->M; g.N = a->N; g.K = a->K; g.dtype = a->dtype;
   g.A = a->A; g.lda = a->lda; g.transA = a->transA;
@@ -462,7 +460,30 @@
   g.alpha = a->alpha; g.beta = a->beta; g.bias = a->bias;
   g.add1 = a->add1; g.ld_add1 = a->ld_add1; g.add1_dtype = a->add1_dtype;
   g.act = a->act; g.aux = a->aux; g.ld_aux = a->ld_aux; g.aux_dtype = a->aux_dtype;
-  return sat_gemm_launch(g, (hipStream_t)stream);
+  return g;
+}
+
+extern "C" int sat_gemm(const SatGemmArgs* a, void* stream) {
+  SAT_REQUIRE(a != nullptr);
+  SatPolicyScope scope(a->policy);
+  return sat_gemm_launch(gemm_from_args(a, a->workspace, a->workspace_bytes), (hipStream_t)stream);
+}
+
+extern "C" int sat_gemm_group(const SatGemmArgs* args, int n, void* workspace, int64_t workspace_bytes, void* stream) {
+  SAT_REQUIRE(args && n >= 1 && n <= kSatGemmGroupMax);
+  SAT_REQUIRE(workspace && workspace_bytes >= (int64_t)sat_gemm_group_workspace_bytes());
+  static_assert(kSatGroupTickets >= (int)kSatSplitTickets, "a product on its own finds its tickets in the group's");
+  const long slab_bytes = (long)(sat_split_gemm_ws_bytes() - kSatSplitTickets * 4);
+  unsigned* tickets = (unsigned*)((char*)workspace + slab_bytes);
+  SatGemm gs[kSatGemmGroupMax];
+  const SatPolicy* pol[kSatGemmGroupMax];
+  for (int i = 0; i < n; ++i) {
+    gs[i] = gemm_from_args(&args[i], workspace, (int64_t)sat_split_gemm_ws_bytes());
+    pol[i] = args[i].policy;
+  }
+  SAT_CHECK((hipError_t)sat_zero_rows((float*)tickets, kSatGroupTickets, 1, kSatGroupTickets, (hipStream_t)stream));
+  return sat_gemm_group_launch(gs, pol, n, (float*)workspace, slab_bytes, tickets, kSatGroupTickets,
+                               (hipStream_t)stream);
 }
 
 extern "C" int sat_conv2d_nhwc(const SatConvGeom* cg, int Cout, int dtype, const void* x, const void* w,
diff --git a/show-attend-and-tell_amd/csrc/gemmsplit.hip b/show-attend-and-tell_amd/csrc/gemmsplit.hip
--- a/show-attend-and-tell_amd/csrc/gemmsplit.hip
+++ b/show-attend-and-tell_amd/csrc/gemmsplit.hip
@@ -1,3 +1,12 @@
+#include <algorithm>
+#include <atomic>
+#include <climits>
+#include <map>
+#include <mutex>
+#include <optional>
+#include <queue>
+#include <vector>
+
 #include "sat_common.h"
 #include "sat_internal.h"
 #include "sat_lds_pipe.h"
@@ -56,27 +65,30 @@
   unsigned dbg_launch;
 };
 
+__host__ __device__ __forceinline__ void split_block_work(int lin, int nwg, int tiles_m, int tiles_n, int* mt, int* nt,
+                                                          int* split) {
+  const int q = nwg / 8, r = nwg % 8, x = lin % 8;
+  lin = (x < r ? x * (q + 1) : r * (q + 1) + (x - r) * q) + lin / 8;
+  *nt = lin % tiles_n;
+  const int rest = lin / tiles_n;
+  *mt = rest % tiles_m;
+  *split = rest / tiles_m;
+}
+
 __device__ __forceinline__ uint4 f4u(f32x4 v) {
   return make_uint4(__float_as_uint(v[0]), __float_as_uint(v[1]), __float_as_uint(v[2]), __float_as_uint(v[3]));
 }
 
 template <int BM, bool AT, bool BT>
-__device__ __forceinline__ void split_gemm_body(const SArgs& a) {
+__device__ __forceinline__ void split_gemm_body(const SArgs& a, char* smem, int lin, const int nwg) {
   using G = SGeom<BM>;
   constexpr int MI = G::MI, NJ = G::NJ, AI = G::AI, BI = G::BI;
-  __shared__ __attribute__((aligned(16))) char smem[G::LDS];
   const int tid = threadIdx.x, lane = tid & 63;
   const int w = __builtin_amdgcn_readfirstlane(tid >> 6);
   const int wm = w / G::WGN, wn = w % G::WGN;
 
-  int lin = blockIdx.x;
-  {
-    const int nwg = gridDim.x, q = nwg / 8, r = nwg % 8, x = lin % 8;
-    lin = (x < r ? x * (q + 1) : r * (q + 1) + (x - r) * q) + lin / 8;
-  }
-  const int nt = lin % a.tiles_n;
-  const int rest = lin / a.tiles_n;
-  const int mt = rest % a.tiles_m, split = rest / a.tiles_m;
+  int mt, nt, split;
+  split_block_work(lin, nwg, a.tiles_m, a.tiles_n, &mt, &nt, &split);
   const int m0 = mt * BM, n0 = nt * SBN;
   const int M = a.M, N = a.N;
   const int kbeg = split * a.kchunk, kend = min(a.K, kbeg + a.kchunk);
@@ -319,9 +331,41 @@
 
 template <int BM, bool AT, bool BT>
 __global__ __launch_bounds__(512) void split_gemm_kernel(SArgs a) {
+  __shared__ __attribute__((aligned(16))) char smem[SGeom<BM>::LDS];
   const SatStampT0 t0 = sat_stamp_begin(a.st);
-  split_gemm_body<BM, AT, BT>(a);
+  split_gemm_body<BM, AT, BT>(a, smem, blockIdx.x, gridDim.x);
   sat_stamp_end(a.st, t0);
+}
+
+struct SGroupArgs {
+  SArgs p[kSatGemmGroupMax];
+  int first[kSatGemmGroupMax];
+  int blocks[kSatGemmGroupMax];
+  int form[kSatGemmGroupMax];
+  SatStamps st;
+};
+
+__global__ __launch_bounds__(512) void split_gemm_group_kernel(SGroupArgs g) {
+  __shared__ __attribute__((aligned(16))) char smem[SGeom<256>::LDS];
+  static_assert(SGeom<256>::LDS >= SGeom<128>::LDS && SGeom<128>::LDS > 80 * 1024, "either ring keeps a CU to itself");
+  const SatStampT0 t0 = sat_stamp_begin(g.st);
+  const int bi = blockIdx.x;
+  int idx = 0;
+#pragma unroll
+  for (int i = 1; i < kSatGemmGroupMax; ++i) idx += bi >= g.first[i] ? 1 : 0;
+  const SArgs& a = g.p[idx];
+  const int lin = bi - g.first[idx], nwg = g.blocks[idx];
+  switch (g.form[idx]) {
+    case 0: split_gemm_body<128, false, false>(a, smem, lin, nwg); break;
+    case 1: split_gemm_body<128, false, true>(a, smem, lin, nwg); break;
+    case 2: split_gemm_body<128, true, false>(a, smem, lin, nwg); break;
+    case 3: split_gemm_body<128, true, true>(a, smem, lin, nwg); break;
+    case 4: split_gemm_body<256, false, false>(a, smem, lin, nwg); break;
+    case 5: split_gemm_body<256, false, true>(a, smem, lin, nwg); break;
+    case 6: split_gemm_body<256, true, false>(a, smem, lin, nwg); break;
+    default: split_gemm_body<256, true, true>(a, smem, lin, nwg); break;
+  }
+  sat_stamp_end(g.st, t0);
 }
 
 
@@ -377,8 +421,160 @@
   const long b_bytes = bt ? 2L * ((long)(g.K - 1) * g.ldb + g.N) : 2L * ((long)(g.N - 1) * g.ldb + g.K);
   const long c_bytes = 4L * ((long)(g.M - 1) * g.ldc + g.N);
   if (a_bytes >= (1L << 31) || b_bytes >= (1L << 31) || c_bytes >= (1L << 31)) return false;
-  if (mode == 0 && g.K < 512) return false;
+  if ((mode == 0 || mode == 4) && g.K < 512) return false;
   return true;
+}
+
+struct GShape {
+  int M, N, K, bm, splits;
+};
+struct GItem {
+  int bm = 0, splits = 1, kchunk = 0, tiles_m = 0, tiles_n = 0, first = 0, blocks = 0;
+  long slab_off = 0, slab_bytes = 0;
+  int ticket_off = 0, tickets = 0, fallback = 0;
+};
+struct GOpt {
+  int b = 0, s = 1, kch = 0, nk = 0, tm = 0, tn = 0, tickets = 0;
+  long slab = 0;
+  long tiles() const { return (long)tm * tn; }
+  double item_us(int j) const {
+    const int kt = kch < nk - j * kch ? kch : nk - j * kch;
+    return kt * kKtileUs[b] + kEpiUs + (s > 1 && j == s - 1 ? (s - 1) * kPartUs[b] : 0.0);
+  }
+};
+
+bool group_option(const GShape& sh, int b, int s, GOpt* o) {
+  const int nk = sat_cdiv(sh.K, SBK), bm = b ? 256 : 128;
+  if (s < 1 || s > kMaxSplits || (s > 1 && nk < 2 * s)) return false;
+  const int kch = sat_cdiv(nk, s);
+  if (sat_cdiv(nk, kch) != s) return false;
+  if (s > 1 && nk - (s - 1) * kch < 2) return false;
+  o->b = b; o->s = s; o->kch = kch; o->nk = nk;
+  o->tm = sat_cdiv(sh.M, bm); o->tn = sat_cdiv(sh.N, SBN);
+  o->slab = s > 1 ? o->tiles() * s * bm * SBN * 4 : 0;
+  o->tickets = s > 1 ? (int)o->tiles() : 0;
+  return o->tiles() * s < (1L << 24);
+}
+
+void group_order(const GOpt* o, const int* in, int n, int* order) {
+  int m = 0;
+  for (int i = 0; i < n; ++i)
+    if (in[i]) order[m++] = i;
+  std::stable_sort(order, order + m,
+                   [&](int x, int y) { return o[x].kch * kKtileUs[o[x].b] > o[y].kch * kKtileUs[o[y].b]; });
+}
+
+double group_model_us(const GOpt* o, const int* in, int n) {
+  int order[kSatGemmGroupMax], m = 0;
+  for (int i = 0; i < n; ++i) m += in[i] ? 1 : 0;
+  group_order(o, in, n, order);
+  std::priority_queue<double, std::vector<double>, std::greater<double>> cu;
+  for (int i = 0; i < kSplitCUs; ++i) cu.push(0.0);
+  double end = 0;
+  for (int x = 0; x < m; ++x) {
+    const GOpt& p = o[order[x]];
+    for (int j = 0; j < p.s; ++j) {
+      const double us = p.item_us(j);
+      for (long t = 0; t < p.tiles(); ++t) {
+        const double e = cu.top() + us;
+        cu.pop();
+        cu.push(e);
+        end = e > end ? e : end;
+      }
+    }
+  }
+  return end;
+}
+
+void plan_group(const GShape* sh, int n, long slab_cap, long ticket_cap, GItem* out) {
+  GOpt cur[kSatGemmGroupMax];
+  int in[kSatGemmGroupMax];
+  long slab = 0, tickets = 0;
+  for (int i = 0; i < n; ++i) {
+    out[i] = GItem{};
+    in[i] = 1;
+    if (sh[i].splits > 0) {
+      if (!group_option(sh[i], sh[i].bm == 256, sh[i].splits, &cur[i]) || slab + cur[i].slab > slab_cap ||
+          tickets + cur[i].tickets > ticket_cap) {
+        in[i] = 0;
+        continue;
+      }
+      slab += cur[i].slab;
+      tickets += cur[i].tickets;
+    } else if (!group_option(sh[i], sh[i].bm == 256, 1, &cur[i])) {
+      in[i] = 0;
+    }
+  }
+  double best = group_model_us(cur, in, n);
+  for (int sweep = 0; sweep < 4; ++sweep) {
+    bool changed = false;
+    for (int i = 0; i < n; ++i) {
+      if (!in[i] || (sh[i].splits > 0 && sh[i].bm > 0)) continue;
+      const GOpt keep = cur[i];
+      GOpt pick = keep;
+      for (int b = 0; b < 2; ++b) {
+        if (sh[i].bm > 0 && (sh[i].bm == 256) != (b == 1)) continue;
+        for (int s = 1; s <= kMaxSplits; ++s) {
+          if (sh[i].splits > 0 && s != sh[i].splits) continue;
+          GOpt o;
+          if (!group_option(sh[i], b, s, &o)) continue;
+          if (slab - keep.slab + o.slab > slab_cap || tickets - keep.tickets + o.tickets > ticket_cap) continue;
+          cur[i] = o;
+          const double us = group_model_us(cur, in, n);
+          if (us < best - 1e-9) {
+            best = us;
+            pick = o;
+          }
+        }
+      }
+      cur[i] = pick;
+      if (pick.b != keep.b || pick.s != keep.s) {
+        slab += pick.slab - keep.slab;
+        tickets += pick.tickets - keep.tickets;
+        changed = true;
+      }
+    }
+    if (!changed) break;
+  }
+  int order[kSatGemmGroupMax], m = 0;
+  for (int i = 0; i < n; ++i) m += in[i] ? 1 : 0;
+  group_order(cur, in, n, order);
+  int first = 0;
+  for (int x = 0; x < m; ++x) {
+    GItem& it = out[order[x]];
+    const GOpt& p = cur[order[x]];
+    it.bm = p.b ? 256 : 128; it.splits = p.s; it.kchunk = p.kch * SBK; it.tiles_m = p.tm; it.tiles_n = p.tn;
+    it.first = first;
+    it.blocks = (int)(p.tiles() * p.s);
+    first += it.blocks;
+  }
+  long so = 0;
+  int to = 0;
+  for (int i = 0; i < n; ++i) {
+    if (!in[i]) {
+      out[i].fallback = 1;
+      continue;
+    }
+    out[i].slab_off = so; out[i].slab_bytes = cur[i].slab;
+    out[i].ticket_off = to; out[i].tickets = cur[i].tickets;
+    so += cur[i].slab;
+    to += cur[i].tickets;
+  }
+}
+
+void plan_group_cached(const GShape* sh, int n, long slab_cap, long ticket_cap, GItem* out) {
+  static std::mutex mu;
+  static std::map<std::vector<long>, std::vector<GItem>> cache;
+  std::vector<long> key{n, slab_cap, ticket_cap};
+  for (int i = 0; i < n; ++i) key.insert(key.end(), {sh[i].M, sh[i].N, sh[i].K, sh[i].bm, sh[i].splits});
+  std::lock_guard<std::mutex> lock(mu);
+  auto it = cache.find(key);
+  if (it == cache.end()) {
+    std::vector<GItem> v(n);
+    plan_group(sh, n, slab_cap, ticket_cap, v.data());
+    it = cache.emplace(key, v).first;
+  }
+  for (int i = 0; i < n; ++i) out[i] = it->second[i];
 }
 
 }
@@ -395,6 +591,24 @@
 }
 
 int sat_split_gemm_takes(const SatGemm& g) { return split_takes(g) ? 1 : 0; }
+
+static SArgs split_args(const SatGemm& g, int splits, int kchunk, int tiles_m, int tiles_n) {
+  const bool at = g.transA != 0, bt = g.transB != 0;
+  SArgs a{};
+  a.M = g.M; a.N = g.N; a.K = g.K;
+  a.A = (const bf16*)g.A; a.lda = g.lda; a.B = (const bf16*)g.B; a.ldb = g.ldb;
+  a.C = (float*)g.C; a.ldc = g.ldc;
+  a.beta1 = g.beta != 0.f;
+  a.add1 = (const float*)g.add1; a.ld_add1 = g.ld_add1;
+  a.splits = splits; a.kchunk = kchunk;
+  a.a_mlim = at && g.a_tail ? sat_cdiv(g.M, 8) * 8 : g.M;
+  a.tiles_m = tiles_m; a.tiles_n = tiles_n;
+  a.a_bytes = (unsigned)(at ? 2L * ((long)(g.K - 1) * g.lda + a.a_mlim)
+                            : 2L * ((long)(g.M - 1) * g.lda + sat_cdiv(g.K, 8) * 8));
+  a.b_bytes = (unsigned)(bt ? 2L * ((long)(g.K - 1) * g.ldb + g.N) : 2L * ((long)(g.N - 1) * g.ldb + g.K));
+  a.c_bytes = (unsigned)(4L * ((long)(g.M - 1) * g.ldc + g.N));
+  return a;
+}
 
 int sat_split_gemm_try(const SatGemm& g, hipStream_t s, int* err) {
   *err = 0;
@@ -403,19 +617,7 @@
   const SPlan p = plan_split(g, have_ws);
   if (p.bm == 0) return 0;
   const bool at = g.transA != 0, bt = g.transB != 0;
-  SArgs a{};
-  a.M = g.M; a.N = g.N; a.K = g.K;
-  a.A = (const bf16*)g.A; a.lda = g.lda; a.B = (const bf16*)g.B; a.ldb = g.ldb;
-  a.C = (float*)g.C; a.ldc = g.ldc;
-  a.beta1 = g.beta != 0.f;
-  a.add1 = (const float*)g.add1; a.ld_add1 = g.ld_add1;
-  a.splits = p.splits; a.kchunk = p.kchunk;
-  a.a_mlim = at && g.a_tail ? sat_cdiv(g.M, 8) * 8 : g.M;
-  a.tiles_m = p.tiles_m; a.tiles_n = p.tiles_n;
-  a.a_bytes = (unsigned)(at ? 2L * ((long)(g.K - 1) * g.lda + a.a_mlim)
-                            : 2L * ((long)(g.M - 1) * g.lda + sat_cdiv(g.K, 8) * 8));
-  a.b_bytes = (unsigned)(bt ? 2L * ((long)(g.K - 1) * g.ldb + g.N) : 2L * ((long)(g.N - 1) * g.ldb + g.K));
-  a.c_bytes = (unsigned)(4L * ((long)(g.M - 1) * g.ldc + g.N));
+  SArgs a = split_args(g, p.splits, p.kchunk, p.tiles_m, p.tiles_n);
   if (p.splits > 1) {
     const long slab = (long)p.tiles_m * p.tiles_n * p.splits * p.bm * SBN * 4;
     SAT_REQUIRE(slab <= g.split_ws_bytes && (long)p.tiles_m * p.tiles_n <= kSplitCUs);
@@ -445,6 +647,124 @@
   return 1;
 }
 
+static std::atomic<int64_t> g_group_launches{0};
+
+int sat_gemm_group_launch(const SatGemm* gs, const SatPolicy* const* pol, int n, float* slab, long slab_bytes,
+                          unsigned* tickets, int n_tickets, hipStream_t s, int keep_splits) {
+  SAT_REQUIRE(gs && n >= 0 && n <= kSatGemmGroupMax);
+  GShape sh[kSatGemmGroupMax];
+  int idx[kSatGemmGroupMax], m = 0;
+  for (int i = 0; i < n; ++i) {
+    std::optional<SatPolicyScope> scope;
+    if (pol) scope.emplace(pol[i]);
+    const SatPolicy& p = sat_policy();
+    if (!slab || !tickets || p.split_gemm == 4 || gs[i].M <= 0 || gs[i].N <= 0 || sat_skinny_takes(gs[i]) ||
+        !split_eligible(gs[i]))
+      continue;
+    sh[m] = GShape{gs[i].M, gs[i].N, gs[i].K, p.split_gemm == 2 ? 128 : p.split_gemm == 3 ? 256 : 0,
+                   p.split_k > 0 ? p.split_k : 0};
+    if (keep_splits) {
+      const SPlan single = plan_split(gs[i], gs[i].split_ws && gs[i].split_tickets);
+      if (single.bm == 0) continue;
+      sh[m].splits = single.splits;
+    }
+    idx[m++] = i;
+  }
+  GItem plan[kSatGemmGroupMax];
+  bool grouped[kSatGemmGroupMax] = {};
+  if (m >= 2) plan_group_cached(sh, m, slab_bytes, n_tickets, plan);
+  int members = 0;
+  for (int x = 0; m >= 2 && x < m; ++x) members += plan[x].fallback ? 0 : 1;
+  if (members >= 2) {
+    SGroupArgs ga{};
+    int total = 0;
+    for (int x = 0, k = 0; x < m; ++x) {
+      const GItem& it = plan[x];
+      if (it.fallback) continue;
+      const SatGemm& g = gs[idx[x]];
+      grouped[idx[x]] = true;
+      SArgs& a = ga.p[k];
+      a = split_args(g, it.splits, it.kchunk, it.tiles_m, it.tiles_n);
+      if (it.splits > 1) {
+        SAT_REQUIRE(it.slab_off + it.slab_bytes <= slab_bytes && it.ticket_off + it.tickets <= n_tickets);
+        a.slab = slab + it.slab_off / 4; a.slab_bytes = (unsigned)it.slab_bytes;
+        a.tickets = tickets + it.ticket_off;
+      }
+#if SAT_SPLIT_DEBUG
+      a.dbg_launch = ++g_sdbg_launch;
+#endif
+      ga.first[k] = it.first; ga.blocks[k] = it.blocks;
+      ga.form[k] = (it.bm == 256 ? 4 : 0) | (g.transA ? 2 : 0) | (g.transB ? 1 : 0);
+      total += it.blocks;
+      ++k;
+    }
+    for (int x = 1; x < members; ++x)
+      for (int y = x; y > 0 && ga.first[y] < ga.first[y - 1]; --y) {
+        std::swap(ga.p[y], ga.p[y - 1]);
+        std::swap(ga.first[y], ga.first[y - 1]);
+        std::swap(ga.blocks[y], ga.blocks[y - 1]);
+        std::swap(ga.form[y], ga.form[y - 1]);
+      }
+    for (int k = members; k < kSatGemmGroupMax; ++k) ga.first[k] = INT_MAX;
+    ga.st = sat_launch_stamps();
+    hipLaunchKernelGGL(split_gemm_group_kernel, dim3((unsigned)total), dim3(512), 0, s, ga);
+    SAT_CHECK(hipGetLastError());
+    g_group_launches.fetch_add(1, std::memory_order_relaxed);
+  }
+  for (int i = 0; i < n; ++i) {
+    if (grouped[i]) continue;
+    std::optional<SatPolicyScope> scope;
+    if (pol) scope.emplace(pol[i]);
+    SAT_CHECK((hipError_t)sat_gemm_launch(gs[i], s));
+  }
+  return 0;
+}
+
+extern "C" int sat_gemm_group_plan(const SatGemmGroupShape* shapes, int n, int64_t slab_bytes, int tickets,
+                                   SatGemmGroupPlan* plan) {
+  SAT_REQUIRE(shapes && plan && n >= 1 && n <= kSatGemmGroupMax && slab_bytes >= 0 && tickets >= 0);
+  GShape sh[kSatGemmGroupMax];
+  for (int i = 0; i < n; ++i) {
+    SAT_REQUIRE(shapes[i].M > 0 && shapes[i].N > 0 && shapes[i].K > 0 && shapes[i].splits >= 0 &&
+                (shapes[i].tile_rows == 0 || shapes[i].tile_rows == 128 || shapes[i].tile_rows == 256));
+    sh[i] = GShape{shapes[i].M, shapes[i].N, shapes[i].K, shapes[i].tile_rows, shapes[i].splits};
+  }
+  GItem it[kSatGemmGroupMax];
+  plan_group(sh, n, slab_bytes, tickets, it);
+  for (int i = 0; i < n; ++i)
+    plan[i] = SatGemmGroupPlan{it[i].bm, it[i].splits, it[i].kchunk, it[i].tiles_m, it[i].tiles_n, it[i].first,
+                               it[i].blocks, it[i].slab_off, it[i].slab_bytes, it[i].ticket_off, it[i].tickets,
+                               it[i].fallback};
+  return 0;
+}
+
+extern "C" int sat_gemm_group_block(const SatGemmGroupPlan* plan, int n, int block, int* product, int* tile_m,
+                                    int* tile_n, int* split) {
+  SAT_REQUIRE(plan && product && tile_m && tile_n && split && n >= 1 && n <= kSatGemmGroupMax);
+  *product = -1;
+  for (int i = 0; i < n; ++i)
+    if (!plan[i].fallback && block >= plan[i].first_block && block < plan[i].first_block + plan[i].blocks) {
+      *product = i;
+      split_block_work(block - plan[i].first_block, plan[i].blocks, plan[i].tiles_m, plan[i].tiles_n, tile_m, tile_n,
+                       split);
+    }
+  return 0;
+}
+
+size_t sat_gemm_group_slab_bound(int M, int N, int K) {
+  const long tiles = (long)sat_cdiv(M, 256) * sat_cdiv(N, SBN);
+  if (tiles < 1) return 0;
+  long s = kSplitCUs / tiles < kMaxSplits ? kSplitCUs / tiles : kMaxSplits;
+  if (s > sat_cdiv(K, SBK) / 2) s = sat_cdiv(K, SBK) / 2;
+  return s > 1 ? (size_t)(tiles * s) * 256 * SBN * 4 : 0;
+}
+
+extern "C" int64_t sat_gemm_group_launches(void) { return g_group_launches.load(std::memory_order_relaxed); }
+
+extern "C" size_t sat_gemm_group_workspace_bytes(void) {
+  return sat_split_gemm_ws_bytes() - kSatSplitTickets * 4 + (size_t)kSatGroupTickets * 4;
+}
+
 #if SAT_SPLIT_DEBUG
 extern "C" int sat_split_debug_read(unsigned* out, int n4, unsigned* count) {
   SAT_CHECK(hipDeviceSynchronize());
diff --git a/show-attend-and-tell_amd/csrc/sat_common.h b/show-attend-and-tell_amd/csrc/sat_common.h
--- a/show-attend-and-tell_amd/csrc/sat_common.h
+++ b/show-attend-and-tell_amd/csrc/sat_common.h
@@ -168,8 +168,14 @@
 int sat_split_gemm_takes(const SatGemm& g);
 size_t sat_split_gemm_ws_bytes();
 constexpr size_t kSatSplitTickets = 256;
+constexpr int kSatGemmGroupMax = 8;
+constexpr int kSatGroupTickets = 1024;
+int sat_gemm_group_launch(const SatGemm* gs, const SatPolicy* const* pol, int n, float* slab, long slab_bytes,
+                          unsigned* tickets, int n_tickets, hipStream_t s, int keep_splits = 0);
+size_t sat_gemm_group_slab_bound(int M, int N, int K);
 int sat_conv_pipe_try(const SatGemm& g, hipStream_t s, int* err);
 int sat_conv_stream_try(const SatGemm& g, hipStream_t s, int* err);
 int sat_skinny_try(const SatGemm& g, hipStream_t s, int* err);
+int sat_skinny_takes(const SatGemm& g);
 int sat_skinny_splits(int M, int N, int K);
 int sat_conv3x3_ws_try(const SatGemm& g, hipStream_t s, int* err);
diff --git a/show-attend-and-tell_amd/csrc/skinny.hip b/show-attend-and-tell_amd/csrc/skinny.hip
--- a/show-attend-and-tell_amd/csrc/skinny.hip
+++ b/show-attend-and-tell_amd/csrc/skinny.hip
@@ -392,6 +392,12 @@
   return 1;
 }
 
+int sat_skinny_takes(const SatGemm& g) {
+  SkArgs a;
+  int nw;
+  return skinny_shape(g, sat_policy().skinny, &a, &nw) && skinny_ptrs(g) ? 1 : 0;
+}
+
 int sat_skinny_splits(int M, int N, int K) {
   if (sat_policy().skinny == 1 || M > 128 || N % SK_COLS || K % 256 || K < 1024) return 0;
   return K / 256;
diff --git a/show-attend-and-tell_amd/ops.py b/show-attend-and-tell_amd/ops.py
--- a/show-attend-and-tell_amd/ops.py
+++ b/show-attend-and-tell_amd/ops.py
@@ -43,6 +43,19 @@
 
 def gemm(A, B, C, *, transA=False, transB=False, alpha=1.0, beta=0.0, bias=None, add1=None, act=L.ACT_NONE,
          aux=None, policy=None, workspace=True):
+    a = _gemm_args(A, B, C, transA, transB, alpha, beta, bias, add1, act, aux, policy)
+    stream = L.stream_of(C)
+    if workspace is True:
+        workspace = (gemm_workspace(C.device, stream)
+                     if policy is not None or _may_split(A, C, bias, aux, act, a.K) else None)
+    if workspace is not None:
+        a.workspace, a.workspace_bytes = workspace.data_ptr(), workspace.numel() * workspace.element_size()
+    L.check(L.lib().sat_gemm(ctypes.byref(a), stream), "sat_gemm")
+    return C
+
+
+def _gemm_args(A, B, C, transA=False, transB=False, alpha=1.0, beta=0.0, bias=None, add1=None, act=L.ACT_NONE,
+               aux=None, policy=None):
     L.require_device(A, B, C)
     dt = L.dtype_code(A.dtype)
     if B.dtype != A.dtype:
@@ -69,14 +82,36 @@
     if aux is not None:
         a.aux, a.ld_aux, a.aux_dtype = aux.data_ptr(), aux.stride(0), L.dtype_code(aux.dtype)
     a.policy = L.policy_ptr(policy)
-    stream = L.stream_of(C)
-    if workspace is True:
-        workspace = (gemm_workspace(C.device, stream)
-                     if policy is not None or _may_split(A, C, bias, aux, act, K) else None)
-    if workspace is not None:
-        a.workspace, a.workspace_bytes = workspace.data_ptr(), workspace.numel() * workspace.element_size()
-    L.check(L.lib().sat_gemm(ctypes.byref(a), stream), "sat_gemm")
-    return C
+    return a
+
+
+def gemm_group(products, workspace):
+    args = (L.SatGemmArgs * len(products))()
+    keep = []
+    for i, p in enumerate(products):
+        a = _gemm_args(**p)
+        keep.append(a)
+        ctypes.memmove(ctypes.byref(args[i]), ctypes.byref(a), ctypes.sizeof(a))
+    L.check(L.lib().sat_gemm_group(args, len(products), workspace.data_ptr(),
+                                   workspace.numel() * workspace.element_size(), L.stream_of(products[0]["C"])),
+            "sat_gemm_group")
+
+
+def gemm_group_plan(shapes, slab_bytes, tickets):
+    sh = (L.SatGemmGroupShape * len(shapes))()
+    for i, t in enumerate(shapes):
+        t = tuple(t) + (0, 0)
+        sh[i].M, sh[i].N, sh[i].K, sh[i].tile_rows, sh[i].splits = t[:5]
+    plan = (L.SatGemmGroupPlan * len(shapes))()
+    L.check(L.lib().sat_gemm_group_plan(sh, len(shapes), slab_bytes, tickets, plan), "sat_gemm_group_plan")
+    return plan
+
+
+def gemm_group_block(plan, block):
+    out = [ctypes.c_int() for _ in range(4)]
+    L.check(L.lib().sat_gemm_group_block(plan, len(plan), block, *[ctypes.byref(o) for o in out]),
+            "sat_gemm_group_block")
+    return tuple(o.value for o in out)
 
 
 def cast_(src, dst):
```

After: 22790 images/s (median of 6 runs). 1.01x the previous value.
